# chaitjo/efficient-gnns

Measured on NVIDIA H100. Metric: edges aggregated/s (fwd+bwd), 3-layer GCN student + logit-KD, ARXIV-shape, higher is better.
Workload: dtype f32

## Files before the change

efficient-gnns_b200/csrc/dense_rows.cu:

```cuda
#include "common.cuh"
#include "philox.cuh"

namespace b200gnn {

constexpr int ROWS_THREADS = 256;

struct RowMap {
  int nvec, rows_per_iter, cv, rg;
  bool active;
};
__device__ __forceinline__ RowMap make_row_map(int K) {
  RowMap m;
  m.nvec = K >> 2;
  m.rows_per_iter = ROWS_THREADS / m.nvec;
  m.rg = threadIdx.x / m.nvec;
  m.cv = threadIdx.x - m.rg * m.nvec;
  m.active = m.rg < m.rows_per_iter;
  return m;
}

__device__ __forceinline__ float4 ld4(const float* p) { return *reinterpret_cast<const float4*>(p); }
__device__ __forceinline__ float4 ld4s(const float* p) { return __ldcs(reinterpret_cast<const float4*>(p)); }
__device__ __forceinline__ void st4(float* p, const float4& v) { *reinterpret_cast<float4*>(p) = v; }

__device__ __forceinline__ void reduce_store_2xK(const RowMap& m, int K, float4 a, float4 b, float* smem ,
                                                 float* out) {
  for (int i = threadIdx.x; i < 2 * K; i += ROWS_THREADS) smem[i] = 0.f;
  __syncthreads();
  for (int g = 0; g < m.rows_per_iter; ++g) {
    if (m.active && m.rg == g) {
      float* s = smem + 4 * m.cv;
      float* q = smem + K + 4 * m.cv;
      s[0] += a.x; s[1] += a.y; s[2] += a.z; s[3] += a.w;
      q[0] += b.x; q[1] += b.y; q[2] += b.z; q[3] += b.w;
    }
    __syncthreads();
  }
  for (int i = threadIdx.x; i < 2 * K; i += ROWS_THREADS) out[i] = smem[i];
}

__global__ void __launch_bounds__(ROWS_THREADS) col_stats4_kernel(const float* __restrict__ Y, int64_t n_rows, int K,
                                                                  float* __restrict__ partial, int slots) {
  extern __shared__ float smem[];
  const RowMap m = make_row_map(K);
  const int64_t per = (n_rows + slots - 1) / slots;
  const int64_t r0 = (int64_t)blockIdx.x * per, r1 = min(n_rows, r0 + per);
  float4 s = make_float4(0, 0, 0, 0), q = s;
  if (m.active)
    for (int64_t r = r0 + m.rg; r < r1; r += m.rows_per_iter) {
      const float4 y = ld4(Y + (size_t)r * K + 4 * m.cv);
      vstat(s, q, y);
    }
  reduce_store_2xK(m, K, s, q, smem, partial + (size_t)blockIdx.x * 2 * K);
}

constexpr int FIN_COLS = 4, FIN_GROUPS = 64;
__device__ __forceinline__ bool finalize_reduce(const float* __restrict__ partial, int slots, int K, bool second,
                                                double& s_out, double& q_out, int& k_out) {
  __shared__ double sh[2][FIN_GROUPS][FIN_COLS];
  const int c = threadIdx.x % FIN_COLS, g = threadIdx.x / FIN_COLS;
  const int k = blockIdx.x * FIN_COLS + c;
  double s = 0.0, q = 0.0;
  if (k < K)
    for (int j = g; j < slots; j += FIN_GROUPS) {
      s += (double)partial[(size_t)j * 2 * K + k];
      if (second) q += (double)partial[(size_t)j * 2 * K + K + k];
    }
  sh[0][g][c] = s; sh[1][g][c] = q;
  __syncthreads();
  if (g == 0 && k < K) {
    s = 0.0; q = 0.0;
    for (int j = 0; j < FIN_GROUPS; ++j) { s += sh[0][j][c]; q += sh[1][j][c]; }
    s_out = s; q_out = q; k_out = k;
    return true;
  }
  return false;
}

__global__ void __launch_bounds__(256) bn_finalize_kernel(const float* __restrict__ partial, int slots, int K,
                                                          int64_t n, const float* __restrict__ gamma,
                                                          const float* __restrict__ beta, float eps, float momentum,
                                                          float* running_mean, float* running_var, float* mean_out,
                                                          float* invstd_out, float* scale_out, float* shift_out) {
  double s, q; int k;
  if (finalize_reduce(partial, slots, K, true, s, q, k)) {
    const double mean = s / (double)n;
    double var = q / (double)n - mean * mean;
    if (var < 0.0) var = 0.0;
    const float invstd = (float)(1.0 / sqrt(var + (double)eps));
    const float sc = gamma[k] * invstd;
    mean_out[k] = (float)mean;
    invstd_out[k] = invstd;
    scale_out[k] = sc;
    shift_out[k] = beta[k] - (float)mean * sc;
    if (running_mean) {
      const double unbiased = n > 1 ? var * (double)n / (double)(n - 1) : var;
      running_mean[k] = (1.f - momentum) * running_mean[k] + momentum * (float)mean;
      running_var[k] = (1.f - momentum) * running_var[k] + momentum * (float)unbiased;
    }
  }
}

__device__ __forceinline__ float4 affine_relu4(float4 y, const float* __restrict__ scale, const float* __restrict__ shift,
                                               int cv, int relu) {
  if (scale) {
    const float4 sc = ld4(scale + 4 * cv), sh = ld4(shift + 4 * cv);
    y.x = fmaf(y.x, sc.x, sh.x); y.y = fmaf(y.y, sc.y, sh.y);
    y.z = fmaf(y.z, sc.z, sh.z); y.w = fmaf(y.w, sc.w, sh.w);
  }
  if (relu) { y.x = fmaxf(y.x, 0.f); y.y = fmaxf(y.y, 0.f); y.z = fmaxf(y.z, 0.f); y.w = fmaxf(y.w, 0.f); }
  return y;
}

template <bool P16>
__global__ void __launch_bounds__(256) affine_relu_dropout_kernel(const float* __restrict__ Y, float* __restrict__ out,
                                                                  int64_t n_vec, int nvec_row,
                                                                  const float* __restrict__ scale,
                                                                  const float* __restrict__ shift, int relu, float p,
                                                                  uint32_t thr16, uint64_t seed, uint64_t offset,
                                                                  const int32_t* __restrict__ step_dev,
// ... 249 lines not shown
    int K, float inv_keep, float* __restrict__ dY, float* __restrict__ colsum_partial, int slots) {
  extern __shared__ float smem[];
  const RowMap m = make_row_map(K);
  const int64_t per = (n_rows + slots - 1) / slots;
  const int64_t r0 = (int64_t)blockIdx.x * per, r1 = min(n_rows, r0 + per);
  float4 s = make_float4(0, 0, 0, 0), q = s;
  if (m.active) {
    const float4 mu = ld4(mean + 4 * m.cv), is = ld4(invstd + 4 * m.cv);
    const float4 c1 = ld4(coef + 4 * m.cv), c2 = ld4(coef + K + 4 * m.cv), c3 = ld4(coef + 2 * K + 4 * m.cv);
    for (int64_t r = r0 + m.rg; r < r1; r += m.rows_per_iter) {
      const size_t o = (size_t)r * K + 4 * m.cv;
      float4 g = ld4s(dOut + o);
      const float4 y = ld4s(Y + o);
      if (!DZ) {
        const float4 x = ld4s(Xout + o);
        g.x = x.x > 0.f ? g.x * inv_keep : 0.f; g.y = x.y > 0.f ? g.y * inv_keep : 0.f;
        g.z = x.z > 0.f ? g.z * inv_keep : 0.f; g.w = x.w > 0.f ? g.w * inv_keep : 0.f;
      }
      float4 d;
      d.x = c1.x * (g.x - c2.x - (y.x - mu.x) * is.x * c3.x);
      d.y = c1.y * (g.y - c2.y - (y.y - mu.y) * is.y * c3.y);
      d.z = c1.z * (g.z - c2.z - (y.z - mu.z) * is.z * c3.z);
      d.w = c1.w * (g.w - c2.w - (y.w - mu.w) * is.w * c3.w);
      st4(dY + o, d);
      s.x += d.x; s.y += d.y; s.z += d.z; s.w += d.w;
    }
  }
  if (colsum_partial) reduce_store_2xK(m, K, s, q, smem, colsum_partial + (size_t)blockIdx.x * 2 * K);
}

__global__ void __launch_bounds__(256) partial_reduce_kernel(const float* __restrict__ partial, int slots, int K2,
                                                             float* __restrict__ out) {
  __shared__ double sh[FIN_GROUPS][FIN_COLS];
  const int c = threadIdx.x % FIN_COLS, g = threadIdx.x / FIN_COLS;
  const int k = blockIdx.x * FIN_COLS + c;
  double s = 0.0;
  if (k < K2)
    for (int j = g; j < slots; j += FIN_GROUPS) s += (double)partial[(size_t)j * K2 + k];
  sh[g][c] = s;
  __syncthreads();
  if (g == 0 && k < K2) {
    s = 0.0;
    for (int j = 0; j < FIN_GROUPS; ++j) s += sh[j][c];
    out[k] = (float)s;
  }
}

__global__ void __launch_bounds__(256) colsum_finalize_kernel(const float* __restrict__ partial, int slots, int K,
                                                              float* __restrict__ out) {
  double s, q; int k;
  if (finalize_reduce(partial, slots, K, false, s, q, k)) out[k] = (float)s;
}

__global__ void __launch_bounds__(256) adam_kernel(float* __restrict__ p, const float* __restrict__ g,
                                                   float* __restrict__ m, float* __restrict__ v, int64_t n, float lr,
                                                   float b1, float b2, float eps, const int32_t* __restrict__ step) {
  const float t = (float)(*step + 1);
  const float bc1 = 1.f - powf(b1, t), bc2 = 1.f - powf(b2, t);
  const float step_size = lr / bc1, inv_sqrt_bc2 = rsqrtf(bc2);
  for (int64_t i = (int64_t)blockIdx.x * blockDim.x + threadIdx.x; i < n; i += (int64_t)gridDim.x * blockDim.x)
    adam_update(p[i], m[i], v[i], g[i], b1, b2, eps, step_size, inv_sqrt_bc2);
}
__global__ void adam_tick_kernel(int32_t* step) { *step += 1; }

__global__ void __launch_bounds__(256) rmsprop_kernel(float* __restrict__ p, const float* __restrict__ g, float* __restrict__ sq,
                                                      int64_t n, double lr, int warmup, float alpha, float one_minus_alpha,
                                                      float eps, float wd, const int32_t* __restrict__ step) {
  const int e = *step + 1;
  const float neg_lr = -(float)(warmup > 0 ? lr * (double)(e < warmup ? e : warmup) / (double)warmup : lr);
  for (int64_t i = (int64_t)blockIdx.x * blockDim.x + threadIdx.x; i < n; i += (int64_t)gridDim.x * blockDim.x) {
    const float pi = p[i];
    float gi = g[i];
    if (wd != 0.f) gi = __fadd_rn(gi, __fmul_rn(wd, pi));
    const float s = __fadd_rn(__fmul_rn(sq[i], alpha), __fmul_rn(__fmul_rn(one_minus_alpha, gi), gi));
    sq[i] = s;
    p[i] = __fadd_rn(pi, __fdiv_rn(__fmul_rn(neg_lr, gi), __fadd_rn(__fsqrt_rn(s), eps)));
  }
}

static inline int grid_for(int64_t n_items, int per_cta, int cap = 132 * 8) {
  int64_t g = (n_items + per_cta - 1) / per_cta;
  if (g > cap) g = cap;
  if (g < 1) g = 1;
  return (int)g;
}

}

using namespace b200gnn;

static bool rows_ok(int64_t n_rows, int64_t K) { return n_rows >= 0 && K > 0 && K % 4 == 0 && K <= 1024; }

extern "C" int64_t b200gnn_rows_slots(int64_t n_rows) {
  int64_t s = (n_rows + 255) / 256;
  if (s > 132 * 4) s = 132 * 4;
  return s < 1 ? 1 : s;
}

extern "C" int b200gnn_col_stats_f32(const float* Y, int64_t n_rows, int64_t K, float* partial, int64_t slots,
                                     void* stream) {
  if (!rows_ok(n_rows, K) || !Y || !partial || slots < 1 || !aligned_to(Y, 16)) return B200GNN_ERR_BAD_ARG;
  col_stats4_kernel<<<(int)slots, ROWS_THREADS, 2 * K * sizeof(float), (cudaStream_t)stream>>>(Y, n_rows, (int)K, partial,
                                                                                             (int)slots);
  return check_launch();
}

extern "C" int b200gnn_bn_finalize_f32(const float* partial, int64_t slots, int64_t K, int64_t n_rows,
                                       const float* gamma, const float* beta, float eps, float momentum,
                                       float* running_mean, float* running_var, float* mean_out, float* invstd_out,
                                       float* scale_out, float* shift_out, void* stream) {
  if (!partial || slots < 1 || K <= 0 || n_rows <= 0 || !gamma || !beta || !mean_out || !invstd_out || !scale_out ||
      !shift_out || ((running_mean == nullptr) != (running_var == nullptr)))
    return B200GNN_ERR_BAD_ARG;
  bn_finalize_kernel<<<(int)((K + FIN_COLS - 1) / FIN_COLS), 256, 0, (cudaStream_t)stream>>>(
// ... 182 lines not shown
  const size_t smem = 2 * K * sizeof(float);
  int rc;
  bn_bwd_finalize_kernel<<<(int)((K + FIN_COLS - 1) / FIN_COLS), 256, 0, st>>>(sums, (int)sum_slots, (int)K, n_norm, gamma,
                                                                              invstd, dgamma, dbeta, coef);
  if ((rc = check_launch())) return rc;
  if (Xout)
    bn_act_bwd_apply_kernel<false><<<(int)slots, ROWS_THREADS, smem, st>>>(dOut, Xout, Y, mean, invstd, coef, n_rows, (int)K,
                                                                          inv_keep, dY, dbias ? partial : nullptr, (int)slots);
  else
    bn_act_bwd_apply_kernel<true><<<(int)slots, ROWS_THREADS, smem, st>>>(dOut, nullptr, Y, mean, invstd, coef, n_rows, (int)K,
                                                                         inv_keep, dY, dbias ? partial : nullptr, (int)slots);
  if ((rc = check_launch())) return rc;
  if (dbias) {
    colsum_finalize_kernel<<<(int)((K + FIN_COLS - 1) / FIN_COLS), 256, 0, st>>>(partial, (int)slots, (int)K, dbias);
    if ((rc = check_launch())) return rc;
  }
  return B200GNN_OK;
}

extern "C" int b200gnn_bn_act_bwd_f32(const float* dOut, const float* Xout, const float* Y, const float* mean,
                                      const float* invstd, const float* gamma, int64_t n_rows, int64_t K, float p,
                                      float* dY, float* dgamma, float* dbeta, float* dbias, float* partial,
                                      int64_t slots, float* coef, void* stream) {
  int rc = b200gnn_bn_act_bwd_reduce_f32(dOut, Xout, Y, mean, invstd, n_rows, K, p, partial, slots, stream);
  if (rc) return rc;
  return b200gnn_bn_act_bwd_apply_f32(dOut, Xout, Y, mean, invstd, gamma, partial, slots, n_rows, n_rows, K, p, dY,
                                      dgamma, dbeta, dbias, partial, slots, coef, stream);
}

extern "C" int b200gnn_partial_reduce_f32(const float* partial, int64_t slots, int64_t K2, float* out, void* stream) {
  if (!partial || !out || slots < 1 || K2 < 1) return B200GNN_ERR_BAD_ARG;
  partial_reduce_kernel<<<(int)((K2 + FIN_COLS - 1) / FIN_COLS), 256, 0, (cudaStream_t)stream>>>(partial, (int)slots, (int)K2,
                                                                                               out);
  return check_launch();
}

extern "C" int b200gnn_col_sum_f32(const float* Y, int64_t n_rows, int64_t K, float* out, float* partial,
                                   int64_t slots, void* stream) {
  if (!rows_ok(n_rows, K) || !Y || !out || !partial || slots < 1) return B200GNN_ERR_BAD_ARG;
  cudaStream_t st = (cudaStream_t)stream;
  int rc;
  col_stats4_kernel<<<(int)slots, ROWS_THREADS, 2 * K * sizeof(float), st>>>(Y, n_rows, (int)K, partial, (int)slots);
  if ((rc = check_launch())) return rc;
  colsum_finalize_kernel<<<(int)((K + FIN_COLS - 1) / FIN_COLS), 256, 0, st>>>(partial, (int)slots, (int)K, out);
  return check_launch();
}

extern "C" int b200gnn_adam_step_f32(float* params, const float* grads, float* exp_avg, float* exp_avg_sq, int64_t n,
                                     float lr, float beta1, float beta2, float eps, int32_t* step, void* stream) {
  if (!params || !grads || !exp_avg || !exp_avg_sq || !step || n < 0) return B200GNN_ERR_BAD_ARG;
  cudaStream_t st = (cudaStream_t)stream;
  int rc;
  if (n > 0) {
    adam_kernel<<<grid_for(n, 256), 256, 0, st>>>(params, grads, exp_avg, exp_avg_sq, n, lr, beta1, beta2, eps, step);
    if ((rc = check_launch())) return rc;
  }
  adam_tick_kernel<<<1, 1, 0, st>>>(step);
  return check_launch();
}

extern "C" int b200gnn_rmsprop_step_f32(float* params, const float* grads, float* square_avg, int64_t n, double lr,
                                        int64_t warmup, double alpha, double eps, double weight_decay, int32_t* step,
                                        void* stream) {
  if (!params || !grads || !square_avg || !step || n < 0 || !(lr >= 0.0) || !(alpha >= 0.0) || !(eps >= 0.0) ||
      !(weight_decay >= 0.0) || warmup < 0 || warmup > (1 << 30))
    return B200GNN_ERR_BAD_ARG;
  cudaStream_t st = (cudaStream_t)stream;
  int rc;
  if (n > 0) {
    rmsprop_kernel<<<grid_for(n, 256), 256, 0, st>>>(params, grads, square_avg, n, lr, (int)warmup, (float)alpha,
                                                     (float)(1.0 - alpha), (float)eps, (float)weight_decay, step);
    if ((rc = check_launch())) return rc;
  }
  adam_tick_kernel<<<1, 1, 0, st>>>(step);
  return check_launch();
}
```

efficient-gnns_b200/csrc/gemm_tf32x3.cu:

```cuda
#include <cuda.h>

#include "common.cuh"
#include "tc_common.cuh"

namespace b200gnn {
namespace gemm {
using namespace tc;

constexpr int BM = 128, BK = 32;
constexpr int THREADS = 384;
constexpr int CONSUMER_WARPS = 8;
constexpr int TILE_BYTES = BM * BK * 4;
constexpr int BAR_BYTES = 256;
constexpr int EPI_BYTES = CONSUMER_WARPS * 16 * 32 * 4;
constexpr int STAT_MAX_N = 256;
constexpr int STAT_BYTES = CONSUMER_WARPS * 2 * STAT_MAX_N * 4;
constexpr int XY_ROWS = 16;
constexpr int XY_SLOT_BYTES = 2 * XY_ROWS * 32 * 4;
constexpr int XY_BYTES = CONSUMER_WARPS * 2 * XY_SLOT_BYTES;
constexpr int XY_BAR_OFF = 128;
constexpr int BNBWD_TMA_MAX_K = 128;

template <int BN_T, int NSTAGE, int EXTRA = 0>
struct Cfg {
// ... 370 lines not shown
      } else {
        const int rr = lane & 15, cb = (lane >> 4) * 16, grow = m0 + q * 16 + rr;
        if (grow < p.M && col0 + cb < p.N) {
          for (int jx = 0; jx < 16; ++jx) {
            const int cc = cb + jx, col = col0 + cc;
            if (col >= p.N) break;
            const float v = tile_s[stg(rr, cc >> 2) + (cc & 3)] + (p.bias ? __ldg(p.bias + col) : 0.f);
            if (PEER && p.bcast) {
              for (int r = 0; r < p.n_peer; ++r) p.Cp[r][(size_t)(p.row_off + grow) * p.ldc + col] = v;
            } else if (!PEER) {
              float* dst = p.C + (size_t)(ROWIDX ? __ldg(p.row_idx + grow) : (int64_t)grow) * p.ldc + col;
              *dst = v + (p.accumulate ? *dst : 0.f);
            }
          }
        }
        __syncwarp();
      }
    }
  }
  if (COLSTAT) {
    __syncwarp();
    float* out = p.stat_partial + (size_t)(blockIdx.x * CONSUMER_WARPS + q) * 2 * p.N;
    for (int i = lane; i < 2 * p.N; i += 32) out[i] = stat[i];
  }
  if (PRB) {
#pragma unroll
    for (int d = 16; d > 0; d >>= 1) sg += __shfl_xor_sync(0xffffffffu, sg, d);
    if (lane == 0) p.slope_partial[blockIdx.x * CONSUMER_WARPS + q] = sg;
  }
}

__global__ void __launch_bounds__(32) slope_grad_finalize_kernel(const double* __restrict__ part, int n, float* __restrict__ out,
                                                                 int accumulate) {
  double a = 0.0;
  for (int i = threadIdx.x; i < n; i += 32) a += part[i];
#pragma unroll
  for (int d = 16; d > 0; d >>= 1) a += __shfl_xor_sync(0xffffffffu, a, d);
  if (threadIdx.x == 0) out[0] = accumulate ? out[0] + (float)a : (float)a;
}

__global__ void __launch_bounds__(256) split_tf32_kernel(const float* __restrict__ W, int64_t rows, int64_t cols,
                                                         int transpose, float* __restrict__ hi, float* __restrict__ lo) {
  const int64_t n = rows * cols;
  for (int64_t i = (int64_t)blockIdx.x * blockDim.x + threadIdx.x; i < n; i += (int64_t)gridDim.x * blockDim.x) {
    const int64_t r = i / cols, c = i - r * cols;
    uint32_t h, l;
    split1(__float_as_uint(W[i]), h, l);
    const int64_t o = transpose ? c * rows + r : i;
    hi[o] = __uint_as_float(h);
    lo[o] = __uint_as_float(l);
  }
}

static bool make_map(CUtensorMap* m, const float* base, int64_t rows, int64_t cols, int64_t ld, int box_rows, bool swizzle = true) {
  EncodeTiledFn fn = encode_fn();
  if (!fn) return false;
  cuuint64_t dims[2] = {(cuuint64_t)cols, (cuuint64_t)rows};
  cuuint64_t strides[1] = {(cuuint64_t)ld * 4};
  cuuint32_t box[2] = {(cuuint32_t)BK, (cuuint32_t)box_rows};
  cuuint32_t estr[2] = {1, 1};
  return fn(m, CU_TENSOR_MAP_DATA_TYPE_FLOAT32, 2, const_cast<float*>(base), dims, strides, box, estr,
            CU_TENSOR_MAP_INTERLEAVE_NONE, swizzle ? CU_TENSOR_MAP_SWIZZLE_128B : CU_TENSOR_MAP_SWIZZLE_NONE,
            CU_TENSOR_MAP_L2_PROMOTION_L2_256B, CU_TENSOR_MAP_FLOAT_OOB_FILL_NONE) == CUDA_SUCCESS;
}

template <class C, int STAT = 0, bool PEER = false, bool ACT = false, bool PRELU = false, bool ROWIDX = false>
static int launch(const float* A, int64_t lda, const float* B_hi, const float* B_lo, int64_t ldb, const Params& p,
                  cudaStream_t stream) {
  CUtensorMap tA, tBh, tBl, tX, tY;
  if (!make_map(&tA, A, p.M, p.K, lda, BM) || !make_map(&tBh, B_hi, p.N, p.K, ldb, C::BN) ||
      !make_map(&tBl, B_lo, p.N, p.K, ldb, C::BN))
    return B200GNN_ERR_UNSUPPORTED;
  tX = tA; tY = tA;
  if (STAT == 3 && ((!ACT && !make_map(&tX, p.bn_x, p.M, p.N, p.ldc, XY_ROWS, false)) ||
                    !make_map(&tY, p.bn_y, p.M, p.N, p.ldc, XY_ROWS, false)))
    return B200GNN_ERR_UNSUPPORTED;
  int dev = 0, sms = 132;
  cudaGetDevice(&dev);
  static bool attr_set[64] = {};
  if (dev >= 0 && dev < 64 && !attr_set[dev]) {
    cudaError_t e = cudaFuncSetAttribute(gemm_tf32x3_kernel<C, STAT, PEER, ACT, PRELU, ROWIDX>, cudaFuncAttributeMaxDynamicSharedMemorySize,
                                         C::SMEM_BYTES);
    if (e != cudaSuccess) { set_cuda_error(e); return B200GNN_ERR_CUDA; }
    attr_set[dev] = true;
  }
  const int tiles = ((p.M + BM - 1) / BM) * ((p.N + C::BN - 1) / C::BN);
  cudaDeviceGetAttribute(&sms, cudaDevAttrMultiProcessorCount, dev);
  const int grid = tiles < sms ? tiles : sms;
  gemm_tf32x3_kernel<C, STAT, PEER, ACT, PRELU, ROWIDX><<<grid, THREADS, C::SMEM_BYTES, stream>>>(tA, tBh, tBl, tX, tY, p);
  return check_launch();
}

}
}

using namespace b200gnn;

extern "C" int b200gnn_split_tf32_f32(const float* W, int64_t rows, int64_t cols, int transpose, float* hi, float* lo,
                                      void* stream) {
  if (!W || !hi || !lo || rows <= 0 || cols <= 0) return B200GNN_ERR_BAD_ARG;
  const int64_t n = rows * cols;
  int grid = (int)((n + 255) / 256);
  if (grid > 132 * 8) grid = 132 * 8;
  gemm::split_tf32_kernel<<<grid, 256, 0, (cudaStream_t)stream>>>(W, rows, cols, transpose, hi, lo);
  return check_launch();
}

static int g_bnbwd_variant = 0;
extern "C" void b200gnn_gemm_set_bnbwd_variant(int v) { g_bnbwd_variant = v; }

static int gemm_dispatch(const float* A, int64_t lda, const float* B_hi, const float* B_lo, int64_t ldb, float* C, int64_t ldc,
                         int64_t M, int64_t N, int64_t K, const float* bias, int accumulate, void* stream,
                         const gemm::Params* st = nullptr, const gemm::Params* act = nullptr,
                         const gemm::Params* prelu = nullptr) {
  if (!A || !B_hi || !B_lo || !C || M <= 0 || N <= 0 || K <= 0 || lda < K || ldb < K || ldc < N ||
      M >= INT32_MAX || N >= INT32_MAX || K >= INT32_MAX)
    return B200GNN_ERR_BAD_ARG;
  if (lda % 4 || ldb % 4 || !aligned_to(A, 16) || !aligned_to(B_hi, 16) || !aligned_to(B_lo, 16))
    return B200GNN_ERR_UNSUPPORTED;
  gemm::Params p{};
  p.C = C; p.bias = bias; p.ldc = ldc; p.M = (int32_t)M; p.N = (int32_t)N; p.K = (int32_t)K; p.accumulate = accumulate ? 1 : 0;
  p.n_peer = 0; p.kc = 0; p.row_off = 0; p.bcast = 0;
  if (act) {
    if (!act->act_scale || !act->act_shift || !act->act_bits || !aligned_to(act->act_scale, 16) || !aligned_to(act->act_shift, 16))
      return B200GNN_ERR_BAD_ARG;
    p.act_scale = act->act_scale; p.act_shift = act->act_shift; p.act_bits = act->act_bits; p.act_words = act->act_words;
    p.inv_keep = act->inv_keep;
  }
  if (prelu) {
    if (!prelu->act_slope || !prelu->act_bits) return B200GNN_ERR_BAD_ARG;
    p.act_slope = prelu->act_slope; p.act_bits = prelu->act_bits; p.act_words = prelu->act_words; p.inv_keep = prelu->inv_keep;
    if (prelu->stat_mode == 0) {
      if (N <= 48) return gemm::launch<gemm::Cfg<48, 6>, 0, false, false, true>(A, lda, B_hi, B_lo, ldb, p, (cudaStream_t)stream);
      return gemm::launch<gemm::Cfg<128, 4>, 0, false, false, true>(A, lda, B_hi, B_lo, ldb, p, (cudaStream_t)stream);
    }
    if (N % 32 || ldc % 4 || !aligned_to(C, 16) || !prelu->bn_y || !aligned_to(prelu->bn_y, 16) || !prelu->slope_partial)
      return B200GNN_ERR_UNSUPPORTED;
    p.stat_mode = 4; p.bn_y = prelu->bn_y; p.slope_partial = prelu->slope_partial;
    return gemm::launch<gemm::Cfg<128, 4>, 4>(A, lda, B_hi, B_lo, ldb, p, (cudaStream_t)stream);
  }
  if (act && !st) {
    if (K > (int64_t)gemm::STAT_BYTES / 8) return B200GNN_ERR_UNSUPPORTED;
    if (N <= 48) return gemm::launch<gemm::Cfg<48, 6>, 0, false, true>(A, lda, B_hi, B_lo, ldb, p, (cudaStream_t)stream);
    return gemm::launch<gemm::Cfg<128, 4>, 0, false, true>(A, lda, B_hi, B_lo, ldb, p, (cudaStream_t)stream);
  }
  if (st) {
    if (N % 32 || N > gemm::STAT_MAX_N || N <= 48 || ldc % 4 || !aligned_to(C, 16) || !st->stat_partial) return B200GNN_ERR_UNSUPPORTED;
    p.stat_mode = st->stat_mode; p.stat_partial = st->stat_partial; p.bn_x = st->bn_x; p.bn_y = st->bn_y;
    p.bn_mean = st->bn_mean; p.bn_invstd = st->bn_invstd; p.inv_keep = st->inv_keep;
    if (p.stat_mode == 1) return gemm::launch<gemm::Cfg<128, 4>, 1>(A, lda, B_hi, B_lo, ldb, p, (cudaStream_t)stream);
    const bool tma = N % 128 == 0 && (g_bnbwd_variant == 1 || (g_bnbwd_variant == 0 && K < gemm::BNBWD_TMA_MAX_K));
    if (act)
      return tma ? gemm::launch<gemm::Cfg<128, 2, gemm::XY_BYTES>, 3, false, true>(A, lda, B_hi, B_lo, ldb, p, (cudaStream_t)stream)
                 : gemm::launch<gemm::Cfg<128, 4>, 2, false, true>(A, lda, B_hi, B_lo, ldb, p, (cudaStream_t)stream);
    if (tma) return gemm::launch<gemm::Cfg<128, 2, gemm::XY_BYTES>, 3>(A, lda, B_hi, B_lo, ldb, p, (cudaStream_t)stream);
    return gemm::launch<gemm::Cfg<128, 4>, 2>(A, lda, B_hi, B_lo, ldb, p, (cudaStream_t)stream);
  }
  if (N <= 48) return gemm::launch<gemm::Cfg<48, 6>>(A, lda, B_hi, B_lo, ldb, p, (cudaStream_t)stream);
  return gemm::launch<gemm::Cfg<128, 4>>(A, lda, B_hi, B_lo, ldb, p, (cudaStream_t)stream);
}
// ... 148 lines not shown
```

efficient-gnns_b200/csrc/spmm.cu:

```cuda
#include <cuda.h>

#include "common.cuh"
#include "tc_common.cuh"

namespace b200gnn {

constexpr int SPMM_THREADS = 256;
constexpr int SPMM_WARPS = SPMM_THREADS / 32;
constexpr int SPMM_MAX_SLAB_FLOATS = 512;

struct SpmmParams {
  const int32_t* rowptr;
  const int32_t* col;
  const float* val;
  const float* X;
  float* Y;
  const float* bias;
  float* stat_partial;
  const int32_t* chunk_rowptr;
  const int32_t* hub_rows;
  const int32_t* hub_segptr;
  float* hub_ws;
  int64_t ldx, ldy;
  int32_t n_rows, K, nvec;
  int32_t hub_threshold, seg_len, n_hub, n_seg, n_chunks;
  int32_t mean, stream_store, main_grid;
  int32_t n_slabs, l2_hint;
  float* Yp[16];
  int32_t yoff[17];
  int32_t n_yp, ycol;
  int64_t ldyp;
};

__device__ __forceinline__ float4* y_row_v4(const SpmmParams& p, int row) {
  if (p.n_yp == 0) return reinterpret_cast<float4*>(p.Y) + (size_t)row * (size_t)(p.ldy / 4);
  int q = 0;
#pragma unroll 1
  while (q + 1 < p.n_yp && row >= p.yoff[q + 1]) ++q;
  return reinterpret_cast<float4*>(p.Yp[q] + (size_t)(row - p.yoff[q]) * (size_t)p.ldyp + p.ycol);
}

struct LaneMap {
  int lpr, groups, g, l;
  bool active;
};

__device__ __forceinline__ LaneMap make_lane_map(int nvec, int lane) {
  LaneMap m;
  if (nvec >= 32) {
    m.lpr = 32; m.groups = 1; m.g = 0; m.l = lane; m.active = true;
  } else {
    m.lpr = nvec; m.groups = 32 / nvec; m.g = lane / nvec; m.l = lane - m.g * nvec;
    m.active = m.g < m.groups;
  }
  return m;
}

template <typename V, int CH, bool HAS_VAL>
__device__ __forceinline__ void walk_edges(const int32_t* __restrict__ col, const float* __restrict__ val,
                                           const V* __restrict__ Xv, size_t ldxv, int beg, int end,
                                           int lane, const LaneMap& m, int slab_voff, int nvec, V (&acc)[CH]) {
  constexpr int U = 8 / CH;
  bool cvalid[CH];
#pragma unroll
  for (int j = 0; j < CH; ++j) cvalid[j] = m.active && (slab_voff + m.l + 32 * j < nvec);

  for (int base = beg; base < end; base += 32) {
    const int e = base + lane;
    int c = 0;
    float v = HAS_VAL ? 0.f : 1.f;
    if (e < end) {
      c = __ldg(col + e);
      if (HAS_VAL) v = __ldg(val + e);
    }
    const int cnt = min(32, end - base);
// ... 77 lines not shown
  const int row_lo = chunk < p.n_chunks ? __ldg(p.chunk_rowptr + chunk) : 0;
  const int row_hi = chunk < p.n_chunks ? __ldg(p.chunk_rowptr + chunk + 1) : 0;
  int end = row_lo < row_hi ? __ldg(p.rowptr + row_lo) : 0;
  for (int row = row_lo; row < row_hi; ++row) {
    const int beg = end;
    end = __ldg(p.rowptr + row + 1);
    const int deg = end - beg;
    if (deg > p.hub_threshold) continue;
    for (int slab = 0; slab < nslab; ++slab) {
      const int slab_voff = slab * slab_vecs;
      V acc[CH];
#pragma unroll
      for (int j = 0; j < CH; ++j) vzero(acc[j]);
      walk_edges<V, CH, HAS_VAL>(p.col, p.val, Xv, ldxv, beg, end, lane, m, slab_voff, p.nvec, acc);
      if (m.groups > 1) group_reduce(acc[0], m);
      if (m.g == 0 && m.active) {
#pragma unroll
        for (int j = 0; j < CH; ++j) {
          const int voff = slab_voff + m.l + 32 * j;
          if (voff < p.nvec) {
            V y = acc[j];
            if (p.mean) vdiv(y, (float)max(deg, 1));
            if (p.bias) vadd(y, load_bias<V>(p.bias, voff));
            V* dst = Yv + (size_t)row * ldyv + voff;
            if (p.stream_store) vstcs(dst, y); else *dst = y;
            if (do_stats) vstat(ssum[j], ssq[j], y);
          }
        }
      }
    }
  }

  if (do_stats) {
    float* ss = s_stat;
    float* sq = s_stat + p.K;
    for (int i = threadIdx.x; i < 2 * p.K; i += SPMM_THREADS) s_stat[i] = 0.f;
    __syncthreads();
    for (int w = 0; w < SPMM_WARPS; ++w) {
      if (warp == w && m.g == 0 && m.active) {
#pragma unroll
        for (int j = 0; j < CH; ++j) {
          const int voff = m.l + 32 * j;
          if (voff < p.nvec) smem_accum(ss, sq, voff, ssum[j], ssq[j]);
        }
      }
      __syncthreads();
    }
    float* out = p.stat_partial + (size_t)cta * 2 * p.K;
    for (int i = threadIdx.x; i < 2 * p.K; i += SPMM_THREADS) out[i] = s_stat[i];
  }
}

template <typename V, int CH, bool HAS_VAL>
__device__ __forceinline__ void spmm_hub_seg_cta(const SpmmParams& p, const int seg, float* s_buf, const int slab_lo = 0,
                                                 const int slab_hi = 1 << 30) {
  constexpr int W = VecTraits<V>::W;

  const int warp = threadIdx.x >> 5, lane = threadIdx.x & 31;
  const LaneMap m = make_lane_map(p.nvec, lane);
  const int slab_vecs = 32 * CH;
  const int nslab = (p.nvec <= 32) ? 1 : (p.nvec + slab_vecs - 1) / slab_vecs;
  const V* Xv = reinterpret_cast<const V*>(p.X);
  const size_t ldxv = (size_t)(p.ldx / W);

  int lo = 0, hi = p.n_hub;
  while (hi - lo > 1) {
    const int mid = (lo + hi) >> 1;
    if (__ldg(p.hub_segptr + mid) <= seg) lo = mid; else hi = mid;
  }
  const int h = lo;
  const int row = __ldg(p.hub_rows + h);
  const int s = seg - __ldg(p.hub_segptr + h);
  const int rbeg = __ldg(p.rowptr + row), rend = __ldg(p.rowptr + row + 1);
  const int sbeg = rbeg + s * p.seg_len;
  const int send = min(rend, sbeg + p.seg_len);
  int per = (send - sbeg + SPMM_WARPS - 1) / SPMM_WARPS;
  per = (per + 31) / 32 * 32;
  const int wbeg = min(send, sbeg + warp * per);
  const int wend = min(send, wbeg + per);

  float* ws = p.hub_ws + (size_t)seg * p.K;
  for (int slab = slab_lo; slab < min(nslab, slab_hi); ++slab) {
    const int slab_voff = slab * slab_vecs;
    V acc[CH];
#pragma unroll
    for (int j = 0; j < CH; ++j) vzero(acc[j]);
    walk_edges<V, CH, HAS_VAL>(p.col, p.val, Xv, ldxv, wbeg, wend, lane, m, slab_voff, p.nvec, acc);
    if (m.groups > 1) group_reduce(acc[0], m);

    for (int i = threadIdx.x; i < SPMM_MAX_SLAB_FLOATS; i += SPMM_THREADS) s_buf[i] = 0.f;
    __syncthreads();
    for (int w = 0; w < SPMM_WARPS; ++w) {
      if (warp == w && m.g == 0 && m.active) {
#pragma unroll
        for (int j = 0; j < CH; ++j) {
          const int voff = slab_voff + m.l + 32 * j;
          if (voff < p.nvec) smem_add1(s_buf, m.l + 32 * j, acc[j]);
        }
      }
      __syncthreads();
    }
    const int slab_f0 = slab_voff * W;
    const int slab_fn = min(slab_vecs * W, p.K - slab_f0);
    for (int i = threadIdx.x; i < slab_fn; i += SPMM_THREADS) ws[slab_f0 + i] = s_buf[i];
    __syncthreads();
  }
}

template <typename V, int CH, bool HAS_VAL, bool STATS>
__global__ void __launch_bounds__(SPMM_THREADS, 3) spmm_rows_kernel(const SpmmParams p) {
  __shared__ float s_mem[2 * SPMM_MAX_SLAB_FLOATS];
  if ((int)blockIdx.x < p.n_seg) spmm_hub_seg_cta<V, CH, HAS_VAL>(p, (int)blockIdx.x, s_mem);
  else spmm_chunk_cta<V, CH, HAS_VAL, STATS>(p, (int)blockIdx.x - p.n_seg, s_mem);
}


constexpr int PIPE_BYTES = 8192;
constexpr int PIPE_SMEM = SPMM_WARPS * PIPE_BYTES;

__device__ __forceinline__ void cp_async16(void* smem_dst, const void* gsrc) {
  asm volatile("cp.async.cg.shared.global [%0], [%1], 16;" ::"r"((uint32_t)__cvta_generic_to_shared(smem_dst)), "l"(gsrc)
               : "memory");
}
__device__ __forceinline__ void cp_async_commit() { asm volatile("cp.async.commit_group;" ::: "memory"); }
template <int N>
__device__ __forceinline__ void cp_async_wait() { asm volatile("cp.async.wait_group %0;" ::"n"(N) : "memory"); }

template <int CH, bool HAS_VAL, bool STATS>
__device__ __forceinline__ void spmm_chunk_cta_pipe(const SpmmParams& p, const int cta, float* s_stat, float4* ring_all) {
  constexpr int D = PIPE_BYTES / (CH * 512);
  constexpr int G = D >= 8 ? 4 : 2, NG = D / G;
  const int warp = threadIdx.x >> 5, lane = threadIdx.x & 31;
  float4* ring = ring_all + (size_t)warp * (PIPE_BYTES / 16);
  const float4* Xv = reinterpret_cast<const float4*>(p.X);
  float4* Yv = reinterpret_cast<float4*>(p.Y);
  const size_t ldxv = (size_t)(p.ldx / 4), ldyv = (size_t)(p.ldy / 4);

  float4 ssum[CH], ssq[CH];
#pragma unroll
  for (int j = 0; j < CH; ++j) { vzero(ssum[j]); vzero(ssq[j]); }

  const int chunk = cta * SPMM_WARPS + warp;
  const int row_lo = chunk < p.n_chunks ? __ldg(p.chunk_rowptr + chunk) : 0;
  const int row_hi = chunk < p.n_chunks ? __ldg(p.chunk_rowptr + chunk + 1) : 0;

  auto flush = [&](int row, int deg, float4 (&acc)[CH]) {
#pragma unroll
    for (int j = 0; j < CH; ++j) {
      const int voff = lane + 32 * j;
      float4 y = acc[j];
      if (p.mean) vdiv(y, (float)max(deg, 1));
      if (p.bias) vadd(y, load_bias<float4>(p.bias, voff));
      float4* dst = Yv + (size_t)row * ldyv + voff;
      if (p.stream_store) vstcs(dst, y); else *dst = y;
      if (STATS) vstat(ssum[j], ssq[j], y);
      vzero(acc[j]);
    }
  };

  int r = row_lo;
  while (r < row_hi) {
    int e_lo = __ldg(p.rowptr + r);
    {
      const int e_next = __ldg(p.rowptr + r + 1);
      if (e_next - e_lo > p.hub_threshold) { ++r; continue; }
// ... 59 lines not shown
      int done = 0;
      while (done < cnt) {
        const int room = rend - (e_lo + j0 + done);
        const int take = min(cnt - done, room);
        if (take == G) {
#pragma unroll
          for (int u = 0; u < G; ++u) {
            const float w = HAS_VAL ? __shfl_sync(FULL_MASK, vA, (j0 + u) & 31) : 1.f;
#pragma unroll
            for (int jj = 0; jj < CH; ++jj) vfma(acc[jj], w, sbase[u * (CH * 32) + 32 * jj]);
          }
        } else {
#pragma unroll 1
          for (int u = done; u < done + take; ++u) {
            const float w = HAS_VAL ? __shfl_sync(FULL_MASK, vA, (j0 + u) & 31) : 1.f;
#pragma unroll
            for (int jj = 0; jj < CH; ++jj) vfma(acc[jj], w, sbase[u * (CH * 32) + 32 * jj]);
          }
        }
        done += take;
        if (take == room) boundary();
      }
    };
#pragma unroll
    for (int g = 0; g < NG; ++g) issue_group(g * G, g * G);
#pragma unroll 1
    for (int j = 0, s0 = 0; j < n; j += G, s0 = (s0 + G) & (D - 1)) {
      cp_async_wait<NG - 1>();
      consume_group(j, s0);
      issue_group(j + D, s0);
    }
    cp_async_wait<0>();
  }

  if (STATS) {
    float* ss = s_stat;
    float* sq = s_stat + p.K;
    for (int i = threadIdx.x; i < 2 * p.K; i += SPMM_THREADS) s_stat[i] = 0.f;
    __syncthreads();
    for (int w = 0; w < SPMM_WARPS; ++w) {
      if (warp == w) {
#pragma unroll
        for (int j = 0; j < CH; ++j) smem_accum(ss, sq, lane + 32 * j, ssum[j], ssq[j]);
      }
      __syncthreads();
    }
    float* out = p.stat_partial + (size_t)cta * 2 * p.K;
    for (int i = threadIdx.x; i < 2 * p.K; i += SPMM_THREADS) out[i] = s_stat[i];
  }
}

template <int CH, bool HAS_VAL, bool STATS>
__global__ void __launch_bounds__(SPMM_THREADS, 3) spmm_rows_pipe_kernel(const SpmmParams p) {
  __shared__ float s_mem[2 * SPMM_MAX_SLAB_FLOATS];
  extern __shared__ float4 s_ring[];
  if ((int)blockIdx.x < p.n_seg) spmm_hub_seg_cta<float4, CH, HAS_VAL>(p, (int)blockIdx.x, s_mem);
  else spmm_chunk_cta_pipe<CH, HAS_VAL, STATS>(p, (int)blockIdx.x - p.n_seg, s_mem, s_ring);
}


constexpr int BULK_RING = 8192;
constexpr int BULK_MAX_GROUPS = 8;

__device__ __forceinline__ uint32_t smem_u32(const void* p) { return (uint32_t)__cvta_generic_to_shared(p); }
__device__ __forceinline__ void mbar_init(uint64_t* bar, int count) {
  asm volatile("mbarrier.init.shared::cta.b64 [%0], %1;" ::"r"(smem_u32(bar)), "r"(count) : "memory");
}
__device__ __forceinline__ void mbar_expect_tx(uint64_t* bar, uint32_t bytes) {
  asm volatile("mbarrier.arrive.expect_tx.shared::cta.b64 _, [%0], %1;" ::"r"(smem_u32(bar)), "r"(bytes) : "memory");
}
__device__ __forceinline__ void mbar_wait(uint64_t* bar, uint32_t parity) {
  asm volatile(
      "{\n\t.reg .pred p;\n\t"
      "WAIT_%=:\n\t"
      "mbarrier.try_wait.parity.shared::cta.b64 p, [%0], %1;\n\t"
      "@p bra DONE_%=;\n\t"
      "bra WAIT_%=;\n\t"
      "DONE_%=:\n\t}" ::"r"(smem_u32(bar)), "r"(parity)
      : "memory");
}
__device__ __forceinline__ void bulk_g2s(void* dst, const void* src, uint32_t bytes, uint64_t* bar) {
  asm volatile("cp.async.bulk.shared::cluster.global.mbarrier::complete_tx::bytes [%0], [%1], %2, [%3];" ::"r"(smem_u32(dst)),
               "l"(src), "r"(bytes), "r"(smem_u32(bar))
               : "memory");
}
__device__ __forceinline__ void bulk_g2s_hint(void* dst, const void* src, uint32_t bytes, uint64_t* bar, uint64_t pol) {
  asm volatile("cp.async.bulk.shared::cluster.global.mbarrier::complete_tx::bytes.L2::cache_hint [%0], [%1], %2, [%3], %4;" ::
                   "r"(smem_u32(dst)), "l"(src), "r"(bytes), "r"(smem_u32(bar)), "l"(pol)
               : "memory");
}

template <int CH, int G, bool HAS_VAL, bool STATS>
__device__ __forceinline__ void spmm_chunk_cta_bulk(const SpmmParams& p, const int cta, const int slab, float* s_stat,
                                                    float4* ring_all, uint64_t* bars_all) {
  constexpr int SLOT_V = CH * 32;
  constexpr int SLOT_B = SLOT_V * 16;
  constexpr int D = BULK_RING / SLOT_B;
  constexpr int NG = D / G;
  static_assert(NG >= 2 && NG <= BULK_MAX_GROUPS && (32 % G) == 0 && D <= 32, "ring geometry");
  const int warp = threadIdx.x >> 5, lane = threadIdx.x & 31;
  float4* ring = ring_all + (size_t)warp * (BULK_RING / 16);
  uint64_t* bars = bars_all + warp * BULK_MAX_GROUPS;
  if (lane < NG) mbar_init(bars + lane, 1);
  asm volatile("fence.mbarrier_init.release.cluster;" ::: "memory");
  asm volatile("fence.proxy.async.shared::cta;" ::: "memory");
  __syncwarp();
  uint64_t pol = 0;
  if (p.l2_hint) asm volatile("createpolicy.fractional.L2::evict_last.b64 %0, 1.0;" : "=l"(pol));

// ... 104 lines not shown
            const float w = HAS_VAL ? __shfl_sync(FULL_MASK, vA, (j0 + u) & 31) : 1.f;
#pragma unroll
            for (int jj = 0; jj < CH; ++jj) vfma(acc[jj], w, sbase[u * SLOT_V + 32 * jj]);
          }
        } else {
#pragma unroll 1
          for (int u = done; u < done + take; ++u) {
            const float w = HAS_VAL ? __shfl_sync(FULL_MASK, vA, (j0 + u) & 31) : 1.f;
#pragma unroll
            for (int jj = 0; jj < CH; ++jj) vfma(acc[jj], w, sbase[u * SLOT_V + 32 * jj]);
          }
        }
        done += take;
        if (take == room) boundary();
      }
    };
#pragma unroll
    for (int g = 0; g < NG; ++g) issue_group(g * G, g * G, g);
    int b = 0;
#pragma unroll 1
    for (int j = 0, s0 = 0; j < n; j += G) {
      mbar_wait(bars + b, (phases >> b) & 1u);
      phases ^= 1u << b;
      consume_group(j, s0);
      __syncwarp();
      issue_group(j + D, s0, b);
      s0 = (s0 + G) & (D - 1);
      b = (b + 1 == NG) ? 0 : b + 1;
    }
  }

  if (STATS) {
    constexpr int SW = SLOT_V * 4;
    float* ss = s_stat;
    float* sq = s_stat + SW;
    for (int i = threadIdx.x; i < 2 * SW; i += SPMM_THREADS) s_stat[i] = 0.f;
    __syncthreads();
    for (int w = 0; w < SPMM_WARPS; ++w) {
      if (warp == w) {
#pragma unroll
        for (int j = 0; j < CH; ++j) smem_accum(ss, sq, lane + 32 * j, ssum[j], ssq[j]);
      }
      __syncthreads();
    }
    float* out = p.stat_partial + (size_t)cta * 2 * p.K + slab * SW;
    for (int i = threadIdx.x; i < SW; i += SPMM_THREADS) { out[i] = ss[i]; out[p.K + i] = sq[i]; }
  }
}

constexpr int BULK_SMEM = SPMM_WARPS * BULK_RING + SPMM_WARPS * BULK_MAX_GROUPS * 8;

template <int CH, int G, bool HAS_VAL, bool STATS>
__global__ void __launch_bounds__(SPMM_THREADS, 3) spmm_rows_bulk_kernel(const SpmmParams p) {
  __shared__ float s_mem[2 * SPMM_MAX_SLAB_FLOATS];
  extern __shared__ __align__(128) unsigned char s_dyn[];
  const int per_slab = p.main_grid + p.n_seg;
  const int slab = (int)blockIdx.x / per_slab;
  const int b = (int)blockIdx.x - slab * per_slab;
  if (b < p.n_seg) spmm_hub_seg_cta<float4, CH, HAS_VAL>(p, b, s_mem, slab, slab + 1);
  else spmm_chunk_cta_bulk<CH, G, HAS_VAL, STATS>(p, b - p.n_seg, slab, s_mem, reinterpret_cast<float4*>(s_dyn),
                                                  reinterpret_cast<uint64_t*>(s_dyn + SPMM_WARPS * BULK_RING));
}


constexpr int SLAB_RING = 8192;
constexpr int SLAB_G = 8;
constexpr int SLAB_SMEM = SPMM_WARPS * SLAB_RING;

__device__ __forceinline__ void cp_async16_pol(void* smem_dst, const void* gsrc, uint64_t pol) {
  asm volatile("cp.async.cg.shared.global.L2::cache_hint [%0], [%1], 16, %2;" ::"r"(smem_u32(smem_dst)), "l"(gsrc), "l"(pol)
               : "memory");
}
__device__ __forceinline__ int32_t ldg_pol(const int32_t* p, uint64_t pol) {
  int32_t v;
  asm("ld.global.nc.L2::cache_hint.b32 %0, [%1], %2;" : "=r"(v) : "l"(p), "l"(pol));
  return v;
}
__device__ __forceinline__ float ldg_pol(const float* p, uint64_t pol) {
  float v;
  asm("ld.global.nc.L2::cache_hint.f32 %0, [%1], %2;" : "=f"(v) : "l"(p), "l"(pol));
  return v;
}

template <int SW> struct SlabLane;
template <> struct SlabLane<32> { using V = float; };
template <> struct SlabLane<64> { using V = float2; };

template <int SW, bool HAS_VAL, bool STATS>
__device__ __forceinline__ void spmm_chunk_cta_slab(const SpmmParams& p, const int cta, const int slab, float* s_stat,
                                                    float* ring_all) {
  using V = typename SlabLane<SW>::V;
  constexpr int LPR = SW / 4;
  constexpr int E = 32 / LPR;
  constexpr int D = SLAB_RING / (SW * 4);
  constexpr int G = SLAB_G, NG = D / G;
  static_assert(G % E == 0 && 32 % G == 0 && NG >= 2 && (D & (D - 1)) == 0, "ring geometry");
  const int warp = threadIdx.x >> 5, lane = threadIdx.x & 31;
  float* ring = ring_all + (size_t)warp * (SLAB_RING / 4);
  uint64_t pol_keep, pol_stream;
  asm volatile("createpolicy.fractional.L2::evict_last.b64 %0, 1.0;" : "=l"(pol_keep));
  asm volatile("createpolicy.fractional.L2::evict_first.b64 %0, 1.0;" : "=l"(pol_stream));

  const int f0 = slab * SW;
  const float* Xs = p.X + f0 + (lane % LPR) * 4;
  float* ring_dst = ring + (lane / LPR) * SW + (lane % LPR) * 4;
  const int vlane = slab * 32 + lane;

  V ssum, ssq, bias_l;
  vzero(ssum); vzero(ssq); vzero(bias_l);
  if (p.bias) bias_l = load_bias<V>(p.bias, vlane);

  const int chunk = cta * SPMM_WARPS + warp;
// ... 87 lines not shown
      if (HAS_VAL && j0 > 0 && (j0 & 31) == 0) { vA = vN; vN = val_win(j0 + 32); }
      const V* sbase = reinterpret_cast<const V*>(ring + slot0 * SW) + lane;
      const int cnt = min(G, n - j0);
      int done = 0;
      while (done < cnt) {
        const int room = rend - (e_lo + j0 + done);
        const int take = min(cnt - done, room);
        if (take == G) {
#pragma unroll
          for (int u = 0; u < G; ++u) {
            const float w = HAS_VAL ? __shfl_sync(FULL_MASK, vA, (j0 + u) & 31) : 1.f;
            vfma(acc, w, sbase[u * 32]);
          }
        } else {
#pragma unroll 1
          for (int u = done; u < done + take; ++u) {
            const float w = HAS_VAL ? __shfl_sync(FULL_MASK, vA, (j0 + u) & 31) : 1.f;
            vfma(acc, w, sbase[u * 32]);
          }
        }
        done += take;
        if (take == room) boundary();
      }
    };
#pragma unroll
    for (int g = 0; g < NG; ++g) issue_group(g * G, g * G);
#pragma unroll 1
    for (int j = 0, s0 = 0; j < n; j += G, s0 = (s0 + G) & (D - 1)) {
      cp_async_wait<NG - 1>();
      __syncwarp();
      consume_group(j, s0);
      __syncwarp();
      issue_group(j + D, s0);
    }
    cp_async_wait<0>();
  }

  if (STATS) {
    float* ss = s_stat;
    float* sq = s_stat + SW;
    for (int i = threadIdx.x; i < 2 * SW; i += SPMM_THREADS) s_stat[i] = 0.f;
    __syncthreads();
    for (int w = 0; w < SPMM_WARPS; ++w) {
      if (warp == w) smem_accum(ss, sq, lane, ssum, ssq);
      __syncthreads();
    }
    float* out = p.stat_partial + (size_t)cta * 2 * p.K + f0;
    for (int i = threadIdx.x; i < SW; i += SPMM_THREADS) { out[i] = ss[i]; out[p.K + i] = sq[i]; }
  }
}

template <int SW, bool HAS_VAL, bool STATS>
__global__ void __launch_bounds__(SPMM_THREADS, 3) spmm_rows_slab_kernel(const SpmmParams p) {
  __shared__ float s_mem[2 * SPMM_MAX_SLAB_FLOATS];
  extern __shared__ __align__(128) unsigned char s_dyn[];
  const int b = (int)blockIdx.x;
  if (b < p.n_seg) {
    spmm_hub_seg_cta<float4, 1, HAS_VAL>(p, b, s_mem);
    return;
  }
  const int slab = (b - p.n_seg) / p.main_grid;
  spmm_chunk_cta_slab<SW, HAS_VAL, STATS>(p, b - p.n_seg - slab * p.main_grid, slab, s_mem, reinterpret_cast<float*>(s_dyn));
}


template <bool HAS_VAL, int U>
__device__ __forceinline__ void spmm_chunk_cta_narrow(const SpmmParams& p, const int cta) {
  const int warp = threadIdx.x >> 5, lane = threadIdx.x & 31;
  const int lpr = p.nvec, groups = 32 / lpr;
  const int g = lane / lpr, l = lane - g * lpr;
  const bool active = g < groups;
  const float4* Xv = reinterpret_cast<const float4*>(p.X);
  float4* Yv = reinterpret_cast<float4*>(p.Y);
  const size_t ldxv = (size_t)(p.ldx / 4), ldyv = (size_t)(p.ldy / 4);
  const int chunk = cta * SPMM_WARPS + warp;
  if (chunk >= p.n_chunks || !active) return;
  const int row_lo = __ldg(p.chunk_rowptr + chunk), row_hi = __ldg(p.chunk_rowptr + chunk + 1);
  float4 bias4 = make_float4(0.f, 0.f, 0.f, 0.f);
  if (p.bias) bias4 = load_bias<float4>(p.bias, l);
  for (int row = row_lo + g; row < row_hi; row += groups) {
    const int beg = __ldg(p.rowptr + row), end = __ldg(p.rowptr + row + 1);
    const int deg = end - beg;
    if (deg > p.hub_threshold) continue;
    float4 acc = make_float4(0.f, 0.f, 0.f, 0.f);
    int e = beg;
    if (e + U <= end) {
      int c[U]; float w[U];
#pragma unroll
      for (int u = 0; u < U; ++u) { c[u] = __ldg(p.col + e + u); w[u] = HAS_VAL ? __ldg(p.val + e + u) : 1.f; }
      for (; e + U <= end; e += U) {
        float4 x[U];
#pragma unroll
        for (int u = 0; u < U; ++u) x[u] = vldg(Xv + (size_t)c[u] * ldxv + l);
        float wc[U];
#pragma unroll
        for (int u = 0; u < U; ++u) wc[u] = w[u];
        if (e + 2 * U <= end) {
#pragma unroll
          for (int u = 0; u < U; ++u) { c[u] = __ldg(p.col + e + U + u); w[u] = HAS_VAL ? __ldg(p.val + e + U + u) : 1.f; }
        }
#pragma unroll
        for (int u = 0; u < U; ++u) vfma(acc, wc[u], x[u]);
      }
    }
    if (U > 4 && e + 4 <= end) {
      int c[4]; float w[4]; float4 x[4];
#pragma unroll
      for (int u = 0; u < 4; ++u) { c[u] = __ldg(p.col + e + u); w[u] = HAS_VAL ? __ldg(p.val + e + u) : 1.f; }
#pragma unroll
      for (int u = 0; u < 4; ++u) x[u] = vldg(Xv + (size_t)c[u] * ldxv + l);
#pragma unroll
      for (int u = 0; u < 4; ++u) vfma(acc, w[u], x[u]);
      e += 4;
    }
    for (; e < end; ++e) {
      const int c = __ldg(p.col + e);
      const float w = HAS_VAL ? __ldg(p.val + e) : 1.f;
      vfma(acc, w, vldg(Xv + (size_t)c * ldxv + l));
    }
    if (p.mean) vdiv(acc, (float)max(deg, 1));
    if (p.bias) vadd(acc, bias4);
    if (p.n_yp) y_row_v4(p, row)[l] = acc; else Yv[(size_t)row * ldyv + l] = acc;
  }
}

template <bool HAS_VAL, int U>
__global__ void __launch_bounds__(SPMM_THREADS, 3) spmm_rows_narrow_kernel(const SpmmParams p) {
  __shared__ float s_mem[SPMM_MAX_SLAB_FLOATS];
  if ((int)blockIdx.x < p.n_seg) spmm_hub_seg_cta<float4, 1, HAS_VAL>(p, (int)blockIdx.x, s_mem);
  else spmm_chunk_cta_narrow<HAS_VAL, U>(p, (int)blockIdx.x - p.n_seg);
}

__global__ void __launch_bounds__(256) spmm_hub_finalize_kernel(const SpmmParams p) {
  __shared__ float4 sh[256];
  const int h = blockIdx.x;
  const int row = __ldg(p.hub_rows + h);
  const int s0 = __ldg(p.hub_segptr + h), s1 = __ldg(p.hub_segptr + h + 1);
  const int deg = __ldg(p.rowptr + row + 1) - __ldg(p.rowptr + row);
  float* stat = p.stat_partial ? p.stat_partial + (size_t)(p.main_grid + h) * 2 * p.K : nullptr;
  const int nvec = p.K >> 2;
  const auto al16 = [](const void* q) { return (reinterpret_cast<uintptr_t>(q) & 15) == 0; };
  if ((p.K & 3) == 0 && nvec <= 256 && (p.ldy & 3) == 0 && al16(p.Y) && al16(p.hub_ws) && (!stat || al16(stat))) {
    const int G = min(256 / nvec, 16);
    const int v = threadIdx.x % nvec, g = threadIdx.x / nvec;
    float4 acc = make_float4(0.f, 0.f, 0.f, 0.f);
    if (g < G)
      for (int s = s0 + g; s < s1; s += G) {
        const float4 x = *reinterpret_cast<const float4*>(p.hub_ws + (size_t)s * p.K + 4 * v);
        acc.x += x.x; acc.y += x.y; acc.z += x.z; acc.w += x.w;
      }
    sh[threadIdx.x] = acc;
    __syncthreads();
    if (g != 0) return;
    for (int j = 1; j < G; ++j) {
      const float4 x = sh[j * nvec + v];
      acc.x += x.x; acc.y += x.y; acc.z += x.z; acc.w += x.w;
    }
    if (p.mean) { const float d = (float)max(deg, 1); acc.x /= d; acc.y /= d; acc.z /= d; acc.w /= d; }
    if (p.bias) {
      acc.x += __ldg(p.bias + 4 * v); acc.y += __ldg(p.bias + 4 * v + 1);
      acc.z += __ldg(p.bias + 4 * v + 2); acc.w += __ldg(p.bias + 4 * v + 3);
    }
    if (p.n_yp) y_row_v4(p, row)[v] = acc; else *reinterpret_cast<float4*>(p.Y + (size_t)row * p.ldy + 4 * v) = acc;
    if (stat) {
      *reinterpret_cast<float4*>(stat + 4 * v) = acc;
      *reinterpret_cast<float4*>(stat + p.K + 4 * v) = make_float4(acc.x * acc.x, acc.y * acc.y, acc.z * acc.z, acc.w * acc.w);
    }
    return;
  }
  float* yrow = p.n_yp ? reinterpret_cast<float*>(y_row_v4(p, row)) : p.Y + (size_t)row * p.ldy;
  for (int k = threadIdx.x; k < p.K; k += blockDim.x) {
    float acc = 0.f;
    for (int s = s0; s < s1; ++s) acc += p.hub_ws[(size_t)s * p.K + k];
    if (p.mean) acc /= (float)max(deg, 1);
    if (p.bias) acc += __ldg(p.bias + k);
    yrow[k] = acc;
    if (stat) { stat[k] = acc; stat[p.K + k] = acc * acc; }
  }
}

__global__ void __launch_bounds__(256) col_stats_kernel(const float* __restrict__ Y, int64_t ldy, int64_t n_rows,
                                                        int K, float* __restrict__ partial, int slots) {
  const int slot = blockIdx.x;
  const int64_t per = (n_rows + slots - 1) / slots;
  const int64_t r0 = (int64_t)slot * per, r1 = min(n_rows, r0 + per);
  float* out = partial + (size_t)slot * 2 * K;
  for (int k = threadIdx.x; k < K; k += blockDim.x) {
    float s = 0.f, q = 0.f;
    for (int64_t r = r0; r < r1; ++r) {
      const float y = Y[(size_t)r * ldy + k];
      s += y; q = fmaf(y, y, q);
    }
    out[k] = s; out[K + k] = q;
  }
}

template <typename V, int CH>
static int launch_spmm(const SpmmParams& p, cudaStream_t st) {
  int rc;
  const bool stats = p.stat_partial != nullptr;
  const int grid = p.main_grid + p.n_seg;
  if (p.val) {
    if (stats) spmm_rows_kernel<V, CH, true, true><<<grid, SPMM_THREADS, 0, st>>>(p);
    else spmm_rows_kernel<V, CH, true, false><<<grid, SPMM_THREADS, 0, st>>>(p);
  } else {
    if (stats) spmm_rows_kernel<V, CH, false, true><<<grid, SPMM_THREADS, 0, st>>>(p);
    else spmm_rows_kernel<V, CH, false, false><<<grid, SPMM_THREADS, 0, st>>>(p);
  }
  if ((rc = check_launch())) return rc;
  if (p.n_hub > 0) {
    spmm_hub_finalize_kernel<<<p.n_hub, 256, 0, st>>>(p);
    if ((rc = check_launch())) return rc;
  }
  return B200GNN_OK;
}

template <int CH>
static int launch_spmm_pipe(const SpmmParams& p, cudaStream_t st) {
  int rc;
  const bool stats = p.stat_partial != nullptr;
  const int grid = p.main_grid + p.n_seg;
  int dev = 0;
  cudaGetDevice(&dev);
  static bool attr_done_dev[64] = {};
  if (dev >= 0 && dev < 64 && !attr_done_dev[dev]) {
    cudaFuncSetAttribute(spmm_rows_pipe_kernel<CH, true, true>, cudaFuncAttributeMaxDynamicSharedMemorySize, PIPE_SMEM);
    cudaFuncSetAttribute(spmm_rows_pipe_kernel<CH, true, false>, cudaFuncAttributeMaxDynamicSharedMemorySize, PIPE_SMEM);
    cudaFuncSetAttribute(spmm_rows_pipe_kernel<CH, false, true>, cudaFuncAttributeMaxDynamicSharedMemorySize, PIPE_SMEM);
    cudaFuncSetAttribute(spmm_rows_pipe_kernel<CH, false, false>, cudaFuncAttributeMaxDynamicSharedMemorySize, PIPE_SMEM);
    attr_done_dev[dev] = true;
  }
  if (p.val) {
    if (stats) spmm_rows_pipe_kernel<CH, true, true><<<grid, SPMM_THREADS, PIPE_SMEM, st>>>(p);
    else spmm_rows_pipe_kernel<CH, true, false><<<grid, SPMM_THREADS, PIPE_SMEM, st>>>(p);
  } else {
    if (stats) spmm_rows_pipe_kernel<CH, false, true><<<grid, SPMM_THREADS, PIPE_SMEM, st>>>(p);
    else spmm_rows_pipe_kernel<CH, false, false><<<grid, SPMM_THREADS, PIPE_SMEM, st>>>(p);
  }
  if ((rc = check_launch())) return rc;
  if (p.n_hub > 0) {
    spmm_hub_finalize_kernel<<<p.n_hub, 256, 0, st>>>(p);
    if ((rc = check_launch())) return rc;
  }
  return B200GNN_OK;
}

constexpr int BULK_SMEM_2CTA = 112 * 1024;

template <int CH, int G>
static int launch_spmm_bulk(const SpmmParams& p, cudaStream_t st, bool two_ctas) {
  int rc;
  const bool stats = p.stat_partial != nullptr;
  const int grid = (p.main_grid + p.n_seg) * p.n_slabs;
  const int smem = two_ctas ? BULK_SMEM_2CTA : BULK_SMEM;
  int dev = 0;
  cudaGetDevice(&dev);
  static bool attr_done[64] = {};
  if (dev >= 0 && dev < 64 && !attr_done[dev]) {
    cudaFuncSetAttribute(spmm_rows_bulk_kernel<CH, G, true, true>, cudaFuncAttributeMaxDynamicSharedMemorySize, BULK_SMEM_2CTA);
    cudaFuncSetAttribute(spmm_rows_bulk_kernel<CH, G, true, false>, cudaFuncAttributeMaxDynamicSharedMemorySize, BULK_SMEM_2CTA);
    cudaFuncSetAttribute(spmm_rows_bulk_kernel<CH, G, false, true>, cudaFuncAttributeMaxDynamicSharedMemorySize, BULK_SMEM_2CTA);
    cudaFuncSetAttribute(spmm_rows_bulk_kernel<CH, G, false, false>, cudaFuncAttributeMaxDynamicSharedMemorySize, BULK_SMEM_2CTA);
    attr_done[dev] = true;
  }
  if (p.val) {
    if (stats) spmm_rows_bulk_kernel<CH, G, true, true><<<grid, SPMM_THREADS, smem, st>>>(p);
    else spmm_rows_bulk_kernel<CH, G, true, false><<<grid, SPMM_THREADS, smem, st>>>(p);
  } else {
    if (stats) spmm_rows_bulk_kernel<CH, G, false, true><<<grid, SPMM_THREADS, smem, st>>>(p);
    else spmm_rows_bulk_kernel<CH, G, false, false><<<grid, SPMM_THREADS, smem, st>>>(p);
  }
  if ((rc = check_launch())) return rc;
  if (p.n_hub > 0) {
    spmm_hub_finalize_kernel<<<p.n_hub, 256, 0, st>>>(p);
    if ((rc = check_launch())) return rc;
  }
  return B200GNN_OK;
}

template <int SW>
static int launch_spmm_slab(const SpmmParams& p, cudaStream_t st) {
  int rc;
  const bool stats = p.stat_partial != nullptr;
  const int grid = p.n_seg + p.main_grid * p.n_slabs;
  int dev = 0;
  cudaGetDevice(&dev);
  static bool attr_done[64] = {};
  if (dev >= 0 && dev < 64 && !attr_done[dev]) {
    cudaFuncSetAttribute(spmm_rows_slab_kernel<SW, true, true>, cudaFuncAttributeMaxDynamicSharedMemorySize, SLAB_SMEM);
    cudaFuncSetAttribute(spmm_rows_slab_kernel<SW, true, false>, cudaFuncAttributeMaxDynamicSharedMemorySize, SLAB_SMEM);
    cudaFuncSetAttribute(spmm_rows_slab_kernel<SW, false, true>, cudaFuncAttributeMaxDynamicSharedMemorySize, SLAB_SMEM);
    cudaFuncSetAttribute(spmm_rows_slab_kernel<SW, false, false>, cudaFuncAttributeMaxDynamicSharedMemorySize, SLAB_SMEM);
    attr_done[dev] = true;
  }
  if (p.val) {
    if (stats) spmm_rows_slab_kernel<SW, true, true><<<grid, SPMM_THREADS, SLAB_SMEM, st>>>(p);
    else spmm_rows_slab_kernel<SW, true, false><<<grid, SPMM_THREADS, SLAB_SMEM, st>>>(p);
  } else {
    if (stats) spmm_rows_slab_kernel<SW, false, true><<<grid, SPMM_THREADS, SLAB_SMEM, st>>>(p);
    else spmm_rows_slab_kernel<SW, false, false><<<grid, SPMM_THREADS, SLAB_SMEM, st>>>(p);
  }
  if ((rc = check_launch())) return rc;
  if (p.n_hub > 0) {
    spmm_hub_finalize_kernel<<<p.n_hub, 256, 0, st>>>(p);
    if ((rc = check_launch())) return rc;
  }
  return B200GNN_OK;
}

template <typename V>
static int dispatch_ch(const SpmmParams& p, cudaStream_t st) {
  if (p.nvec <= 32) return launch_spmm<V, 1>(p, st);
  if (p.nvec <= 64) return launch_spmm<V, 2>(p, st);
  return launch_spmm<V, 4>(p, st);
}

__global__ void __launch_bounds__(1024) hub_count_kernel(const int32_t* __restrict__ rowptr, int64_t n_rows,
                                                         int32_t thr, int32_t seg_len, int32_t* __restrict__ out) {
  __shared__ int s_cnt[2];
  if (threadIdx.x < 2) s_cnt[threadIdx.x] = 0;
  __syncthreads();
  int nh = 0, ns = 0;
  for (int64_t r = threadIdx.x; r < n_rows; r += blockDim.x) {
    const int deg = rowptr[r + 1] - rowptr[r];
    if (deg > thr) { nh += 1; ns += (deg + seg_len - 1) / seg_len; }
  }
  atomicAdd(&s_cnt[0], nh);
  atomicAdd(&s_cnt[1], ns);
  __syncthreads();
  if (threadIdx.x < 2) out[threadIdx.x] = s_cnt[threadIdx.x];
}

__global__ void __launch_bounds__(1024) hub_fill_kernel(const int32_t* __restrict__ rowptr, int64_t n_rows,
                                                        int32_t thr, int32_t seg_len, int32_t* __restrict__ hub_rows,
                                                        int32_t* __restrict__ hub_segptr, int64_t n_hub) {
  __shared__ int s_wflag[32], s_wseg[32];
  __shared__ int s_base[2];
  const int lane = threadIdx.x & 31, warp = threadIdx.x >> 5;
  if (threadIdx.x == 0) { s_base[0] = 0; s_base[1] = 0; }
  __syncthreads();
  for (int64_t r0 = 0; r0 < n_rows; r0 += blockDim.x) {
    const int64_t r = r0 + threadIdx.x;
    int flag = 0, segs = 0;
    if (r < n_rows) {
      const int deg = rowptr[r + 1] - rowptr[r];
      if (deg > thr) { flag = 1; segs = (deg + seg_len - 1) / seg_len; }
    }
    int f = flag, s = segs;
    for (int d = 1; d < 32; d <<= 1) {
      const int of = __shfl_up_sync(FULL_MASK, f, d), os = __shfl_up_sync(FULL_MASK, s, d);
      if (lane >= d) { f += of; s += os; }
    }
    if (lane == 31) { s_wflag[warp] = f; s_wseg[warp] = s; }
    __syncthreads();
    if (warp == 0) {
      int wf = s_wflag[lane], wsg = s_wseg[lane];
// ... 36 lines not shown
}

}

using namespace b200gnn;

static int g_spmm_variant = 0;

struct ScatterArgs { int n; float* ptr[16]; int32_t off[17]; int64_t ld, col; };
static thread_local ScatterArgs g_scatter = {0, {}, {}, 0, 0};

static int bulk_auto_slab(int64_t K, int64_t n_src) {
  (void)n_src;
  return (K % 256 == 0) ? 256 : 128;
}
constexpr int64_t SLAB_L2_BUDGET = (int64_t)40 << 20;
constexpr int SLAB_SW = 64;
extern "C" void b200gnn_spmm_set_variant(int v) { g_spmm_variant = v; }

extern "C" int64_t b200gnn_csr_chunk_count(int64_t n_rows, int64_t nnz, int32_t chunk_nnz, int32_t row_cost) {
  if (n_rows < 0 || nnz < 0 || chunk_nnz <= 0 || row_cost <= 0) return B200GNN_ERR_BAD_ARG;
  const int64_t total = nnz + n_rows * (int64_t)row_cost;
  return total == 0 ? 0 : (total + chunk_nnz - 1) / chunk_nnz;
}

extern "C" int b200gnn_csr_chunk_plan(const int32_t* rowptr, int64_t n_rows, int64_t nnz, int32_t chunk_nnz,
                                      int32_t row_cost, int32_t* chunk_rowptr, void* stream) {
  const int64_t n_chunks = b200gnn_csr_chunk_count(n_rows, nnz, chunk_nnz, row_cost);
  if (n_chunks < 0 || !rowptr || !chunk_rowptr) return B200GNN_ERR_BAD_ARG;
  chunk_plan_kernel<<<(int)((n_chunks + 1 + 255) / 256), 256, 0, (cudaStream_t)stream>>>(rowptr, n_rows, chunk_nnz,
                                                                                        row_cost, chunk_rowptr, n_chunks);
  return check_launch();
}

extern "C" int b200gnn_csr_hub_count(const int32_t* rowptr, int64_t n_rows, int32_t hub_threshold, int32_t seg_len,
                                     int32_t* counts_out, void* stream) {
  if (!rowptr || !counts_out || n_rows < 0 || hub_threshold < 0 || seg_len <= 0) return B200GNN_ERR_BAD_ARG;
  hub_count_kernel<<<1, 1024, 0, (cudaStream_t)stream>>>(rowptr, n_rows, hub_threshold, seg_len, counts_out);
  return check_launch();
}

extern "C" int b200gnn_csr_hub_fill(const int32_t* rowptr, int64_t n_rows, int32_t hub_threshold, int32_t seg_len,
                                    int32_t* hub_rows, int32_t* hub_segptr, int64_t n_hub, void* stream) {
  if (!rowptr || !hub_segptr || n_rows < 0 || n_hub < 0 || hub_threshold < 0 || seg_len <= 0) return B200GNN_ERR_BAD_ARG;
  if (n_hub > 0 && !hub_rows) return B200GNN_ERR_BAD_ARG;
  hub_fill_kernel<<<1, 1024, 0, (cudaStream_t)stream>>>(rowptr, n_rows, hub_threshold, seg_len, hub_rows, hub_segptr, n_hub);
  return check_launch();
}

extern "C" int64_t b200gnn_spmm_stat_slots(int64_t n_chunks, int64_t n_hub) {
  return (n_chunks + SPMM_WARPS - 1) / SPMM_WARPS + n_hub;
}

extern "C" int b200gnn_spmm_csr_f32(const int32_t* rowptr, const int32_t* col, const float* val, const float* X,
                                    int64_t ldx, float* Y, int64_t ldy, int64_t n_rows, int64_t n_src, int64_t K,
                                    int reduce, const float* bias, float* stat_partial,
                                    const int32_t* chunk_rowptr, int64_t n_chunks, int32_t hub_threshold,
                                    int32_t seg_len, const int32_t* hub_rows, const int32_t* hub_segptr,
                                    int64_t n_hub, int64_t n_seg, float* hub_workspace, void* stream) {
  if (n_rows < 0 || n_src < 0 || K <= 0 || n_rows >= INT32_MAX || n_src >= INT32_MAX || K > (1 << 20))
    return B200GNN_ERR_BAD_ARG;
  if (reduce != B200GNN_REDUCE_SUM && reduce != B200GNN_REDUCE_MEAN) return B200GNN_ERR_BAD_ARG;
  if (n_rows == 0) return B200GNN_OK;
  if (!rowptr || !Y || ldy < K || !chunk_rowptr || n_chunks <= 0 || n_chunks >= INT32_MAX) return B200GNN_ERR_BAD_ARG;
  if (n_src > 0 && (!X || ldx < K)) return B200GNN_ERR_BAD_ARG;
  if (n_hub < 0 || n_seg < 0 || hub_threshold < 0) return B200GNN_ERR_BAD_ARG;
  if (n_hub > 0 && (!hub_rows || !hub_segptr || !hub_workspace || seg_len <= 0 || n_seg < n_hub))
    return B200GNN_ERR_BAD_ARG;
  cudaStream_t st = (cudaStream_t)stream;

  SpmmParams p;
  p.rowptr = rowptr; p.col = col; p.val = val; p.X = X; p.Y = Y; p.bias = bias;
  p.stat_partial = stat_partial;
  p.chunk_rowptr = chunk_rowptr; p.n_chunks = (int32_t)n_chunks;
  p.hub_rows = hub_rows; p.hub_segptr = hub_segptr; p.hub_ws = hub_workspace;
  p.ldx = ldx; p.ldy = ldy;
  p.n_rows = (int32_t)n_rows; p.K = (int32_t)K;
  p.hub_threshold = hub_threshold; p.seg_len = seg_len; p.n_hub = (int32_t)n_hub;
  p.n_seg = n_hub > 0 ? (int32_t)n_seg : 0;
  p.mean = reduce == B200GNN_REDUCE_MEAN;
  p.stream_store = (n_rows * K * 4 > (int64_t)64 << 20) ? 1 : 0;
  p.main_grid = (int32_t)((n_chunks + SPMM_WARPS - 1) / SPMM_WARPS);

  int W = 1;
  if (K % 4 == 0 && ldx % 4 == 0 && ldy % 4 == 0 && aligned_to(X, 16) && aligned_to(Y, 16)) W = 4;
  else if (K % 2 == 0 && ldx % 2 == 0 && ldy % 2 == 0 && aligned_to(X, 8) && aligned_to(Y, 8)) W = 2;
  p.nvec = (int32_t)(K / W);
  p.n_slabs = 1; p.l2_hint = 0;
  p.n_yp = 0; p.ycol = 0; p.ldyp = 0;
  if (g_scatter.n > 0) {
    if (W != 4 || K % 4 || g_scatter.ld % 4 || g_scatter.col % 4) return B200GNN_ERR_UNSUPPORTED;
    const int sfam = g_spmm_variant & 15;
    const bool to_bulk = K % 128 == 0 && K <= 4096 && (sfam == 0 || (sfam >= 3 && sfam <= 7));
    const bool to_narrow = p.nvec <= 16 && !stat_partial && sfam != 1 && sfam != 2;
    if (!to_bulk && !to_narrow) return B200GNN_ERR_UNSUPPORTED;
    p.n_yp = g_scatter.n; p.ycol = (int32_t)g_scatter.col; p.ldyp = g_scatter.ld;
    for (int q = 0; q < g_scatter.n; ++q) { p.Yp[q] = g_scatter.ptr[q]; p.yoff[q] = g_scatter.off[q]; }
    p.yoff[g_scatter.n] = g_scatter.off[g_scatter.n];
  }

  if (g_spmm_variant == 0 && W == 4 && p.n_yp == 0 && (K == 128 || K == 256) && n_src * K * 4 > SLAB_L2_BUDGET) {
    p.n_slabs = (int32_t)(K / SLAB_SW);
    return launch_spmm_slab<SLAB_SW>(p, st);
  }

  const int fam = g_spmm_variant & 15;
  const bool alt_g = (g_spmm_variant & 32) != 0;
  int bulk_sw = 0;
  if (W == 4 && K % 128 == 0 && K <= 4096) {
    if (fam == 3) bulk_sw = (K % 256 == 0) ? 256 : 128;
    else if (fam == 4) bulk_sw = 128;
    else if (fam == 5) bulk_sw = (K % 256 == 0) ? 256 : 128;
    else if (fam == 6 || fam == 7) bulk_sw = 128;
    else if (fam == 0) bulk_sw = bulk_auto_slab(K, n_src);
  }
  int rc;
  float* fused_stats = stat_partial;
  bool single_slab = true;
  if (bulk_sw) {
    p.n_slabs = (int32_t)(K / bulk_sw);
    p.l2_hint = (g_spmm_variant & 16) ? 1 : 0;
    if (fam == 6) return launch_spmm_bulk<1, 8>(p, st, false);
    if (fam == 7) return launch_spmm_bulk<1, 4>(p, st, false);
    const bool two = (g_spmm_variant & 64) != 0;
    if (bulk_sw == 128) rc = alt_g ? launch_spmm_bulk<1, 2>(p, st, two) : launch_spmm_bulk<1, 4>(p, st, two);
    else rc = alt_g ? launch_spmm_bulk<2, 2>(p, st, two) : launch_spmm_bulk<2, 4>(p, st, two);
    return rc;
  }

  const int ch = p.nvec <= 32 ? 1 : (p.nvec <= 64 ? 2 : 4);
  single_slab = p.nvec <= 32 * ch;
  if (!single_slab) p.stat_partial = nullptr;

  const bool pipe_ok = (W == 4) && fam == 2 && (p.nvec == 32 || p.nvec == 64 || p.nvec == 128);
  const bool narrow_ok = (W == 4) && p.nvec <= 16 && !p.stat_partial && fam != 1;
  if (narrow_ok) {
    rc = B200GNN_OK;
    const int grid = p.main_grid + p.n_seg;
    const bool deep = (g_spmm_variant & 128) != 0;
    if (p.val) { if (deep) spmm_rows_narrow_kernel<true, 8><<<grid, SPMM_THREADS, 0, st>>>(p); else spmm_rows_narrow_kernel<true, 4><<<grid, SPMM_THREADS, 0, st>>>(p); }
    else { if (deep) spmm_rows_narrow_kernel<false, 8><<<grid, SPMM_THREADS, 0, st>>>(p); else spmm_rows_narrow_kernel<false, 4><<<grid, SPMM_THREADS, 0, st>>>(p); }
    if ((rc = check_launch())) return rc;
    if (p.n_hub > 0) {
      spmm_hub_finalize_kernel<<<p.n_hub, 256, 0, st>>>(p);
      if ((rc = check_launch())) return rc;
    }
  }
  else if (pipe_ok && p.nvec == 32) rc = launch_spmm_pipe<1>(p, st);
  else if (pipe_ok && p.nvec == 64) rc = launch_spmm_pipe<2>(p, st);
  else if (pipe_ok && p.nvec == 128) rc = launch_spmm_pipe<4>(p, st);
  else if (W == 4) rc = dispatch_ch<float4>(p, st);
  else if (W == 2) rc = dispatch_ch<float2>(p, st);
  else rc = dispatch_ch<float>(p, st);
  if (rc) return rc;

  if (fused_stats && !single_slab) {
    const int slots = (int)b200gnn_spmm_stat_slots(n_chunks, n_hub);
    col_stats_kernel<<<slots, 256, 0, st>>>(Y, ldy, n_rows, (int)K, fused_stats, slots);
    if ((rc = check_launch())) return rc;
  }
  return B200GNN_OK;
}

extern "C" int b200gnn_spmm_csr_scatter_f32(const int32_t* rowptr, const int32_t* col, const float* val, const float* X,
                                            int64_t ldx, float* const* Y_ptrs, const int32_t* row_off, int32_t world,
                                            int64_t ldy_dst, int64_t col_dst, int64_t n_rows, int64_t n_src, int64_t K, int reduce,
                                            const float* bias, const int32_t* chunk_rowptr, int64_t n_chunks,
                                            int32_t hub_threshold, int32_t seg_len, const int32_t* hub_rows,
                                            const int32_t* hub_segptr, int64_t n_hub, int64_t n_seg, float* hub_workspace,
                                            void* stream) {
  if (!Y_ptrs || !row_off || world <= 0 || world > 16 || ldy_dst < K || col_dst < 0 || row_off[0] != 0 || row_off[world] != n_rows)
    return B200GNN_ERR_BAD_ARG;
  g_scatter.n = world; g_scatter.ld = ldy_dst; g_scatter.col = col_dst;
  for (int q = 0; q < world; ++q) {
    if (!Y_ptrs[q] || !aligned_to(Y_ptrs[q], 16) || row_off[q + 1] < row_off[q]) { g_scatter.n = 0; return B200GNN_ERR_BAD_ARG; }
    g_scatter.ptr[q] = Y_ptrs[q]; g_scatter.off[q] = row_off[q];
  }
  g_scatter.off[world] = row_off[world];
  const int rc = b200gnn_spmm_csr_f32(rowptr, col, val, X, ldx, Y_ptrs[0], K, n_rows, n_src, K, reduce, bias, nullptr, chunk_rowptr,
                                      n_chunks, hub_threshold, seg_len, hub_rows, hub_segptr, n_hub, n_seg, hub_workspace, stream);
  g_scatter.n = 0;
  return rc;
}
```

efficient-gnns_b200/engine.py:

```python
from __future__ import annotations

import math
from typing import Dict, List, Optional

import torch

from . import lib, ops
from .sparse import CsrGraph, SparseTensor
from .trainer import FlatParams, FullBatchStudent, one_objective


def gcn_norm(adj: SparseTensor) -> SparseTensor:
    if not adj.has_value():
        adj = adj.fill_value(1.0)
    adj = adj.fill_diag(1.0)
    deg = adj.sum(dim=1)
    dis = deg.pow(-0.5)
    dis.masked_fill_(dis == float("inf"), 0.0)
    row, col, val = adj.coo()
    return adj.set_value(dis[row] * val * dis[col])


def _is_symmetric(adj: SparseTensor) -> bool:
    st = adj.storage
# ... 7 lines not shown


class GCNStudentTrainer(FullBatchStudent):

    def __init__(self, adj: SparseTensor, dims: List[int], dropout: float = 0.5, lr: float = 0.01, seed: int = 0,
                 alpha: float = 0.9, kd_T: float = 4.0, bn_eps: float = 1e-5, bn_momentum: float = 0.1,
                 aggregate_first: Optional[bool] = None, tensor_core_gemm: bool = True, overlap_wgrad: bool = True,
                 fuse_row_passes: bool = True, fuse_activations: bool = True, _prebuilt_graph: Optional[CsrGraph] = None, _rows_alloc: Optional[int] = None,
                 gcrd=None, lsp=None, gsp=None):
        self.objective = one_objective(gcrd, lsp, gsp)
        assert adj.is_cuda(), "the engine runs on a CUDA device"
        self.device = adj.device
        self.dims, self.L = list(dims), len(dims) - 1
        self.p, self.lr, self.alpha, self.kd_T = float(dropout), float(lr), float(alpha), float(kd_T)
        self.bn_eps, self.bn_momentum = bn_eps, bn_momentum
        self.seed = int(seed)
        self.tc_gemm = bool(tensor_core_gemm) and all(d % 4 == 0 for d in dims)
        for d in dims[1:]:
            assert d % 4 == 0 and d <= 1024, "layer widths must be multiples of 4 (128-bit rows)"
        self.N = adj.size(0)
        self.agg_first = (dims[0] < dims[1] and dims[0] % 4 == 0) if aggregate_first is None else bool(aggregate_first)
        if self.L < 2:
            self.agg_first = False

        if _prebuilt_graph is not None:
            self.G = self.Gt = _prebuilt_graph
            self.N = _prebuilt_graph.n_rows
        else:
            norm = gcn_norm(adj)
            self.G: CsrGraph = norm.storage.engine_csr()
            self.Gt: CsrGraph = self.G if _is_symmetric(norm) else norm.storage.engine_csc("value")
        self.nnz = self.G.nnz

        shapes = []
        for l in range(self.L):
            shapes += [(dims[l], dims[l + 1]), (dims[l + 1],)]
            if l < self.L - 1:
                shapes += [(dims[l + 1],), (dims[l + 1],)]
        dev = self.device
        self.store = FlatParams(shapes, dev).attach(self)
        self.W, self.b, self.gamma, self.beta = [], [], [], []
        self.gW, self.gb, self.ggamma, self.gbeta = [], [], [], []
        views = iter(self.store.views)
        for l in range(self.L):
            (w, gw), (b, gb) = next(views), next(views)
            self.W.append(w); self.gW.append(gw); self.b.append(b); self.gb.append(gb)
            if l < self.L - 1:
                (g, gg), (be, gbe) = next(views), next(views)
                self.gamma.append(g); self.ggamma.append(gg); self.beta.append(be); self.gbeta.append(gbe)
        self.Wt_split = [(torch.empty(dims[l + 1], dims[l], device=dev), torch.empty(dims[l + 1], dims[l], device=dev))
                         for l in range(self.L)]
        self.W_split = [(torch.empty(dims[l], dims[l + 1], device=dev), torch.empty(dims[l], dims[l + 1], device=dev))
                        for l in range(self.L)]
        wg = [ops.wgrad_supported(dims[l], dims[l + 1]) for l in range(self.L)]
        self.wgrad_ws = (torch.empty(max(ops.wgrad_workspace_floats(dims[l], dims[l + 1]) for l in range(self.L) if wg[l]), device=dev)
                         if self.tc_gemm and any(wg) else None)
        self.running_mean = [torch.zeros(d, device=dev) for d in dims[1:-1]]
        self.running_var = [torch.ones(d, device=dev) for d in dims[1:-1]]
        self.reset_parameters(seed)

        N = self.N
        rows_alloc = N if _rows_alloc is None else _rows_alloc
        self._blocks = []

        def buf(k):
            blk = torch.zeros(rows_alloc, k, device=dev)
            self._blocks.append(blk)
            return blk[:N]
        self.H = [buf(dims[l + 1]) for l in range(self.L)]
        self.Y = [buf(dims[l + 1]) for l in range(self.L)]
        self._A = [buf(dims[l + 1]) for l in range(self.L - 1)]
        self.dY = [buf(dims[l + 1]) for l in range(self.L)]
        self.dH = [buf(dims[l + 1]) for l in range(self.L)]
        self.dA = [buf(dims[l + 1]) for l in range(self.L - 1)]
        self.AX = buf(dims[0]) if self.agg_first else None
        slots_spmm = ops.stat_slots(self.G)
        self.stat_part = [torch.empty(slots_spmm, 2, dims[l + 1], device=dev) for l in range(self.L - 1)]
        self.bn = [torch.empty(4, dims[l + 1], device=dev) for l in range(self.L - 1)]
        self.rs = ops.rows_slots(N)
        self.fuse_rows = bool(fuse_row_passes) and self.tc_gemm
        self._gemm_part = {k: torch.empty(ops.gemm_stat_slots(N, k), 2, k, device=dev)
                           for k in set(dims[1:-1]) if self.fuse_rows and ops.gemm_stats_supported(k)}
        hid = dims[1:-1]
        self.fuse_act = (bool(fuse_activations) and self.fuse_rows and self.L >= 2 and len(set(hid)) == 1
                         and ops.gemm_stats_supported(hid[0]) and hid[0] <= 2048
                         and all(ops.wgrad_supported(dims[l], dims[l + 1]) for l in range(1, self.L)))
        self.keep_bits = (torch.zeros(self.L - 1, N, (hid[0] + 31) // 32, dtype=torch.int32, device=dev)
                          if self.fuse_act else None)
        self._act_stale = False
        self._fwd_fused = False
        self._ev_bits = torch.cuda.Event()
        self.kd_part = torch.empty(2 * int(lib.load().b200gnn_kd_partials(N)), device=dev)
        self.overlap_wgrad = overlap_wgrad
        self._side = torch.cuda.Stream(device=dev) if overlap_wgrad else None
        self._ev_fork, self._ev_join = torch.cuda.Event(), torch.cuda.Event()
        self._static: Dict[str, torch.Tensor] = {}
        for k in set(dims[1:]):
            self._part(k); self._coef(k)
        if self.objective is not None:
            self.objective.bind(self)

    def reset_parameters(self, seed: int = 0):
        g = torch.Generator().manual_seed(seed)
        for l in range(self.L):
            fan_in, fan_out = self.dims[l], self.dims[l + 1]
            a = math.sqrt(6.0 / (fan_in + fan_out))
            self.W[l].copy_((torch.rand(fan_in, fan_out, generator=g) * 2 - 1) * a)
            self.b[l].zero_()
        for l in range(self.L - 1):
            self.gamma[l].fill_(1.0); self.beta[l].zero_()
            self.running_mean[l].zero_(); self.running_var[l].fill_(1.0)
        self.exp_avg.zero_(); self.exp_avg_sq.zero_(); self.step_count.zero_()

    def state_dict(self) -> Dict[str, torch.Tensor]:
        sd = {}
        for l in range(self.L):
            sd[f"convs.{l}.weight"] = self.W[l].detach().clone()
            sd[f"convs.{l}.bias"] = self.b[l].detach().clone()
        for l in range(self.L - 1):
            sd[f"bns.{l}.weight"] = self.gamma[l].detach().clone()
            sd[f"bns.{l}.bias"] = self.beta[l].detach().clone()
            sd[f"bns.{l}.running_mean"] = self.running_mean[l].clone()
            sd[f"bns.{l}.running_var"] = self.running_var[l].clone()
        return sd

    def load_state_dict(self, sd: Dict[str, torch.Tensor]):
        for l in range(self.L):
            self.W[l].copy_(sd[f"convs.{l}.weight"]); self.b[l].copy_(sd[f"convs.{l}.bias"])
        for l in range(self.L - 1):
            self.gamma[l].copy_(sd[f"bns.{l}.weight"]); self.beta[l].copy_(sd[f"bns.{l}.bias"])
            if f"bns.{l}.running_mean" in sd:
                self.running_mean[l].copy_(sd[f"bns.{l}.running_mean"]); self.running_var[l].copy_(sd[f"bns.{l}.running_var"])

    @property
    def A(self) -> List[torch.Tensor]:
        if self._act_stale:
            self._act_stale = False
            for l in range(self.L - 1):
                ops.affine_relu_bits(self.Y[l], self.keep_bits[l], self.bn[l][2], self.bn[l][3], self.p, out=self._A[l])
        return self._A

    def _act(self, l: int):
        return self.Y[l], self.bn[l][2], self.bn[l][3], self.keep_bits[l]

    def activation_pattern(self, l: int) -> torch.Tensor:
        return self.A[l] > 0

    def out_feat(self) -> torch.Tensor:
        return self.A[-1]

    def forward(self, x: torch.Tensor, training: bool = True) -> torch.Tensor:
        fused = training and self.fuse_act
        self._act_stale = False
        if fused:
            if self._side is not None:
                self._ev_fork.record(torch.cuda.current_stream())
                self._side.wait_event(self._ev_fork)
                with torch.cuda.stream(self._side):
                    ops.dropout_bits(self.keep_bits, self.p, self.seed, 0, step_dev=self.step_count, step_mul=self.L)
                self._ev_bits.record(self._side)
            else:
                ops.dropout_bits(self.keep_bits, self.p, self.seed, 0, step_dev=self.step_count, step_mul=self.L)
        A = self._A
        inp = x
        for l in range(self.L):
            last = l == self.L - 1
            if l == 0 and self.agg_first:
                ops.spmm_csr(self.G, x, "sum", out=self.AX)
                if training:
                    gp = self._gemm_part.get(self.dims[1])
                    if gp is not None:
                        hi, lo = ops.split_tf32(self.W[0], transpose=True, hi=self.Wt_split[0][0], lo=self.Wt_split[0][1])
                        ops.gemm_tf32x3_stats(self.AX, hi, lo, self.b[0], self.Y[0], gp)
                        part = gp
                    else:
                        self._linear(0, self.AX, self.Y[0], bias=self.b[0])
                        part = ops.col_stats(self.Y[0], partial=self._part(self.dims[1]))
                    ops.bn_finalize(part, self.N, self.gamma[0], self.beta[0], self.bn_eps,
                                    self.bn_momentum, self.running_mean[0], self.running_var[0], out=self.bn[0])
                    if not fused:
                        ops.affine_relu_dropout(self.Y[0], self.bn[0][2], self.bn[0][3], True, self.p, self.seed, 0,
                                                out=A[0], step_dev=self.step_count, step_mul=self.L)
                else:
                    self._linear(0, self.AX, self.Y[0], bias=self.b[0])
                    scale = self.gamma[0] * torch.rsqrt(self.running_var[0] + self.bn_eps)
                    shift = self.beta[0] - self.running_mean[0] * scale
                    ops.affine_relu_dropout(self.Y[0], scale, shift, True, 0.0, out=A[0])
                inp = A[0]
                continue
            if fused and l > 0:
                if l == 1 and self._side is not None:
                    torch.cuda.current_stream().wait_event(self._ev_bits)
                self._linear(l, None, self.H[l], act=self._act(l - 1))
            else:
                self._linear(l, inp, self.H[l])
            if last:
                ops.spmm_csr(self.G, self.H[l], "sum", bias=self.b[l], out=self.Y[l])
            elif training:
                ops.spmm_csr(self.G, self.H[l], "sum", bias=self.b[l], out=self.Y[l], stat_partial=self.stat_part[l])
                ops.bn_finalize(self.stat_part[l], self.N, self.gamma[l], self.beta[l], self.bn_eps, self.bn_momentum,
                                self.running_mean[l], self.running_var[l], out=self.bn[l])
                if not fused:
                    ops.affine_relu_dropout(self.Y[l], self.bn[l][2], self.bn[l][3], True, self.p, self.seed, l,
                                            out=A[l], step_dev=self.step_count, step_mul=self.L)
                inp = A[l]
            else:
                ops.spmm_csr(self.G, self.H[l], "sum", bias=self.b[l], out=self.Y[l])
                scale = self.gamma[l] * torch.rsqrt(self.running_var[l] + self.bn_eps)
                shift = self.beta[l] - self.running_mean[l] * scale
                ops.affine_relu_dropout(self.Y[l], scale, shift, True, 0.0, out=A[l])
                inp = A[l]
        self._act_stale = self._fwd_fused = fused
        return self.Y[-1]

    def backward(self, x: torch.Tensor, d_out_feat: Optional[torch.Tensor] = None):
        fused = self._fwd_fused
        for l in range(self.L - 1, -1, -1):
            act = self._act(l - 1) if fused and l > 0 else None
            inp = x if l == 0 else (None if act else self._A[l - 1])
            if l == self.L - 1:
                ops.col_sum(self.dY[l], out=self.gb[l], partial=self._part(self.dims[l + 1]))
            if l == 0 and self.agg_first:
                self._wgrad_async(0, self.AX, self.dY[0])
                continue
            ops.spmm_csr(self.Gt, self.dY[l], "sum", out=self.dH[l])
            d_prev = self.dA[l - 1] if l > 0 else None
            gp = self._gemm_part.get(self.dims[l]) if l > 0 else None
            if l > 0:
                acc = d_out_feat is not None and l == self.L - 1
                if acc:
                    d_prev = d_out_feat
                if gp is not None:
                    hi, lo = ops.split_tf32(self.W[l], transpose=False, hi=self.W_split[l][0], lo=self.W_split[l][1])
                    if act:
                        ops.gemm_tf32x3_bnbwd_bits(self.dH[l], hi, lo, d_prev, act[3], self.Y[l - 1], self.bn[l - 1][0],
                                                   self.bn[l - 1][1], act[1], act[2], self.p, gp, accumulate=acc)
                    else:
                        ops.gemm_tf32x3_bnbwd(self.dH[l], hi, lo, d_prev, self._A[l - 1], self.Y[l - 1], self.bn[l - 1][0],
                                              self.bn[l - 1][1], self.p, gp, accumulate=acc)
                else:
                    self._linear_dgrad(l, self.dH[l], d_prev, accumulate=acc)
            self._wgrad_async(l, inp, self.dH[l], act=act)
            if l > 0:
                k = self.dims[l]
                part = self._part(k)
                if gp is not None:
                    ops.bn_act_bwd_apply(d_prev, None, self.Y[l - 1], self.bn[l - 1][0], self.bn[l - 1][1], self.gamma[l - 1],
                                         gp, self.N, self.p, self.dY[l - 1], self.ggamma[l - 1], self.gbeta[l - 1],
                                         self.gb[l - 1], part, self._coef(k))
                else:
                    ops.bn_act_bwd(d_prev, self._A[l - 1], self.Y[l - 1], self.bn[l - 1][0], self.bn[l - 1][1],
                                   self.gamma[l - 1], self.p, d_y=self.dY[l - 1], d_gamma=self.ggamma[l - 1],
                                   d_beta=self.gbeta[l - 1], d_bias=self.gb[l - 1], partial=part, coef=self._coef(k))
        self._wgrad_join()

    def _wgrad_async(self, l: int, inp: Optional[torch.Tensor], d_out: torch.Tensor, act=None):
        if self._side is None:
            return self._linear_wgrad(l, inp, d_out, act)
        self._ev_fork.record(torch.cuda.current_stream())
        self._side.wait_event(self._ev_fork)
        with torch.cuda.stream(self._side):
            self._linear_wgrad(l, inp, d_out, act)

    def _wgrad_join(self):
        if self._side is not None:
            self._ev_join.record(self._side)
            torch.cuda.current_stream().wait_event(self._ev_join)

    def _linear(self, l: int, inp: Optional[torch.Tensor], out: torch.Tensor, bias: Optional[torch.Tensor] = None, act=None):
        if act is not None:
            hi, lo = ops.split_tf32(self.W[l], transpose=True, hi=self.Wt_split[l][0], lo=self.Wt_split[l][1])
            ops.gemm_tf32x3_act(*act, self.p, hi, lo, bias=bias, out=out)
        elif self.tc_gemm:
            hi, lo = ops.split_tf32(self.W[l], transpose=True, hi=self.Wt_split[l][0], lo=self.Wt_split[l][1])
            ops.gemm_tf32x3(inp, hi, lo, bias=bias, out=out)
        elif bias is not None:
            torch.addmm(bias, inp, self.W[l], out=out)
        else:
            torch.mm(inp, self.W[l], out=out)

    def _linear_dgrad(self, l: int, d_out: torch.Tensor, d_inp: torch.Tensor, accumulate: bool = False):
        if self.tc_gemm:
            hi, lo = ops.split_tf32(self.W[l], transpose=False, hi=self.W_split[l][0], lo=self.W_split[l][1])
            ops.gemm_tf32x3(d_out, hi, lo, out=d_inp, accumulate=accumulate)
        elif accumulate:
            d_inp.addmm_(d_out, self.W[l].t())
        else:
            torch.mm(d_out, self.W[l].t(), out=d_inp)

    def _linear_wgrad(self, l: int, inp: Optional[torch.Tensor], d_out: torch.Tensor, act=None):
        if act is not None:
            ops.gemm_wgrad_tf32x3_act(*act, self.p, d_out, out=self.gW[l], workspace=self.wgrad_ws)
        elif self.tc_gemm and ops.wgrad_supported(self.dims[l], self.dims[l + 1]):
            ops.gemm_wgrad_tf32x3(inp, d_out, out=self.gW[l], workspace=self.wgrad_ws)
        else:
            torch.mm(inp.t(), d_out, out=self.gW[l])

    def replay(self, key: int = 0) -> torch.Tensor:
        super().replay(key)
        self._act_stale = self.fuse_act
        return self.loss_out

    def aggregations_per_step(self) -> Dict[int, int]:
        out: Dict[int, int] = {}
        for l in range(self.L):
            if l == 0 and self.agg_first:
                out[self.dims[0]] = out.get(self.dims[0], 0) + 1
            else:
                out[self.dims[l + 1]] = out.get(self.dims[l + 1], 0) + 2
        return out

    def spmm_algorithmic_bytes(self) -> Dict[int, int]:
        return {k: 2 * self.N * k * 4 + self.nnz * 8 + (self.N + 1) * 4 for k in set(self.dims)}
```

efficient-gnns_b200/lib.py:

```python
from __future__ import annotations

import ctypes as C
import os
from pathlib import Path

import torch

PKG_DIR = Path(__file__).resolve().parent
LIB_PATH = PKG_DIR / "libb200gnn.so"

OK = 0
REDUCE_SUM = 0
REDUCE_MEAN = 1
LSP_MAX_F = 512

_i32p = C.c_void_p
_f32p = C.c_void_p
_ptr = C.c_void_p
_i64 = C.c_int64
_i32 = C.c_int32
_int = C.c_int
_f32 = C.c_float
_f64 = C.c_double
_u64 = C.c_uint64

SIGNATURES = {
    "b200gnn_abi_version": (_int, []),
    "b200gnn_error_string": (C.c_char_p, [_int]),
    "b200gnn_last_cuda_error": (C.c_char_p, []),
    "b200gnn_launch_count": (_i64, []),
    "b200gnn_reset_launch_count": (None, []),
    "b200gnn_csr_chunk_count": (_i64, [_i64, _i64, _i32, _i32]),
    "b200gnn_csr_chunk_plan": (_int, [_i32p, _i64, _i64, _i32, _i32, _i32p, _ptr]),
    "b200gnn_csr_hub_count": (_int, [_i32p, _i64, _i32, _i32, _i32p, _ptr]),
    "b200gnn_csr_hub_fill": (_int, [_i32p, _i64, _i32, _i32, _i32p, _i32p, _i64, _ptr]),
    "b200gnn_spmm_stat_slots": (_i64, [_i64, _i64]),
    "b200gnn_spmm_set_variant": (None, [_int]),
    "b200gnn_spmm_csr_f32": (_int, [_i32p, _i32p, _f32p, _f32p, _i64, _f32p, _i64, _i64, _i64, _i64, _int,
                                    _f32p, _f32p, _i32p, _i64, _i32, _i32, _i32p, _i32p, _i64, _i64, _f32p, _ptr]),
    "b200gnn_spmm_csr_scatter_f32": (_int, [_i32p, _i32p, _f32p, _f32p, _i64, _ptr, _ptr, _i32, _i64, _i64, _i64, _i64, _i64, _int,
                                            _f32p, _i32p, _i64, _i32, _i32, _i32p, _i32p, _i64, _i64, _f32p, _ptr]),
    "b200gnn_rows_slots": (_i64, [_i64]),
    "b200gnn_col_stats_f32": (_int, [_f32p, _i64, _i64, _f32p, _i64, _ptr]),
    "b200gnn_col_sum_f32": (_int, [_f32p, _i64, _i64, _f32p, _f32p, _i64, _ptr]),
    "b200gnn_bn_finalize_f32": (_int, [_f32p, _i64, _i64, _i64, _f32p, _f32p, _f32, _f32, _f32p, _f32p,
                                       _f32p, _f32p, _f32p, _f32p, _ptr]),
    "b200gnn_affine_relu_dropout_f32": (_int, [_f32p, _f32p, _i64, _i64, _f32p, _f32p, _int, _f32, _u64, _u64,
                                               _i32p, _u64, _u64, _ptr]),
    "b200gnn_affine_relu_dropout_mapped_f32": (_int, [_f32p, _f32p, _i64, _i64, _f32p, _f32p, _int, _f32, _u64, _u64,
                                                      _i32p, _u64, _i32p, _u64, _i64, _i64, _ptr]),
    "b200gnn_affine_relu_dropout_scatter_f32": (_int, [_f32p, _f32p, _i64, _i64, _f32p, _f32p, _int, _f32, _u64, _u64,
                                                       _i32p, _u64, _i32p, _u64, _i64, _i64, _ptr, _ptr, _i32, _i64, _ptr]),
    "b200gnn_dropout_mask_u8": (_int, [_ptr, _i64, _i64, _f32, _u64, _u64, _ptr]),
    "b200gnn_dropout_mask_step_u8": (_int, [_ptr, _i64, _i64, _f32, _u64, _u64, _i32p, _u64, _ptr]),
    "b200gnn_dropout_bits_u32": (_int, [_ptr, _i64, _i64, _i64, _f32, _u64, _u64, _i32p, _u64, _ptr]),
    "b200gnn_affine_relu_bits_f32": (_int, [_f32p, _ptr, _f32p, _f32p, _f32, _f32p, _i64, _i64, _ptr]),
    "b200gnn_gather_rows_act_f32": (_int, [_f32p, _i64, _ptr, _i64, _i64, _ptr, _f32p, _f32p, _f32, _f32p, _ptr]),
    "b200gnn_relu_dropout_bwd_f32": (_int, [_f32p, _f32p, _f32p, _i64, _i64, _f32, _ptr]),
    "b200gnn_bn_act_bwd_f32": (_int, [_f32p, _f32p, _f32p, _f32p, _f32p, _f32p, _i64, _i64, _f32, _f32p, _f32p,
                                      _f32p, _f32p, _f32p, _i64, _f32p, _ptr]),
    "b200gnn_bn_act_bwd_reduce_f32": (_int, [_f32p, _f32p, _f32p, _f32p, _f32p, _i64, _i64, _f32, _f32p, _i64, _ptr]),
    "b200gnn_bn_act_bwd_apply_f32": (_int, [_f32p, _f32p, _f32p, _f32p, _f32p, _f32p, _f32p, _i64, _i64, _i64, _i64, _f32,
                                            _f32p, _f32p, _f32p, _f32p, _f32p, _i64, _f32p, _ptr]),
    "b200gnn_partial_reduce_f32": (_int, [_f32p, _i64, _i64, _f32p, _ptr]),
    "b200gnn_adam_step_f32": (_int, [_f32p, _f32p, _f32p, _f32p, _i64, _f32, _f32, _f32, _f32, _i32p, _ptr]),
    "b200gnn_rmsprop_step_f32": (_int, [_f32p, _f32p, _f32p, _i64, _f64, _i64, _f64, _f64, _f64, _i32p, _ptr]),
    "b200gnn_teacher_slots": (_i64, [_i64]),
    "b200gnn_label_inputs_f32": (_int, [_f32p, _i64, _i64, _i64, _i64, _i32p, _ptr, _int, _f32, _u64, _u64, _i32p, _u64, _ptr,
                                        _int, _ptr, _i32p, _ptr]),
    "b200gnn_label_softmax_f32": (_int, [_f32p, _i64, _i64, _i64, _ptr, _int, _f32p, _i64, _ptr]),
    "b200gnn_logce_fwd_bwd_f32": (_int, [_f32p, _i64, _i64, _ptr, _i64, _ptr, _ptr, _i32p, _i64, _f32p, _i64, _f32p, _f32p,
                                         _ptr, _ptr]),
    "b200gnn_split_eval_f32": (_int, [_f32p, _i64, _i64, _ptr, _i64, _i64, _i64, _ptr, _f32p, _f32p, _ptr, _ptr]),
    "b200gnn_snapshot_if_better_f32": (_int, [_f32p, _f32p, _f32p, _f32p, _i64, _f32p, _f32p, _i64, _f32p, _f32p, _i64, _ptr]),
    "b200gnn_kd_partials": (_i64, [_i64]),
    "b200gnn_kd_loss_fwd_bwd_f32": (_int, [_f32p, _i64, _ptr, _i64, _ptr, _f32p, _i64, _i64, _f32, _f32, _i64, _f32p,
                                           _i64, _f32p, _f32p, _ptr]),
    "b200gnn_split_tf32_f32": (_int, [_f32p, _i64, _i64, _int, _f32p, _f32p, _ptr]),
    "b200gnn_gemm_tf32x3_f32": (_int, [_f32p, _i64, _f32p, _f32p, _i64, _f32p, _i64, _i64, _i64, _i64, _f32p, _ptr]),
    "b200gnn_random_walk_i64": (_int, [_i32p, _i32p, _i64, _ptr, _i64, _i32, _u64, _u64, _ptr, _ptr]),
    "b200gnn_saint_subgraph_count_i64": (_int, [_i32p, _i32p, _ptr, _i64, _i32p, _ptr, _ptr]),
    "b200gnn_saint_subgraph_fill_i64": (_int, [_i32p, _i32p, _ptr, _ptr, _i64, _i32p, _ptr, _ptr, _ptr, _ptr, _ptr]),
    "b200gnn_gemm_stat_slots": (_i64, [_i64, _i64]),
    "b200gnn_gemm_set_bnbwd_variant": (None, [_int]),
    "b200gnn_gemm_tf32x3_stats_f32": (_int, [_f32p, _i64, _f32p, _f32p, _i64, _f32p, _i64, _i64, _i64, _i64, _f32p, _int, _f32p, _i64,
                                             _ptr]),
    "b200gnn_gemm_tf32x3_bnbwd_f32": (_int, [_f32p, _i64, _f32p, _f32p, _i64, _f32p, _i64, _i64, _i64, _i64, _int,
                                             _f32p, _f32p, _f32p, _f32p, _f32, _f32p, _i64, _ptr]),
    "b200gnn_gemm_tf32x3_bnbwd_bits_f32": (_int, [_f32p, _i64, _f32p, _f32p, _i64, _f32p, _i64, _i64, _i64, _i64, _int,
                                                  _ptr, _f32p, _f32p, _f32p, _f32p, _f32p, _f32, _f32p, _i64, _ptr]),
    "b200gnn_gemm_tf32x3_act_f32": (_int, [_f32p, _i64, _f32p, _f32p, _i64, _f32p, _i64, _i64, _i64, _i64, _f32p,
                                           _f32p, _f32p, _ptr, _f32, _ptr]),
    "b200gnn_gemm_tf32x3_acc_f32": (_int, [_f32p, _i64, _f32p, _f32p, _i64, _f32p, _i64, _i64, _i64, _i64, _ptr]),
    "b200gnn_gemm_tf32x3_rowidx_f32": (_int, [_f32p, _i64, _f32p, _f32p, _i64, _f32p, _i64, _i64, _i64, _i64, _ptr, _ptr]),
    "b200gnn_gemm_tf32x3_scatter_f32": (_int, [_f32p, _i64, _f32p, _f32p, _i64, _ptr, _i32, _i64, _i64, _i64, _i64, _f32p, _ptr]),
    "b200gnn_gemm_tf32x3_bcast_f32": (_int, [_f32p, _i64, _f32p, _f32p, _i64, _ptr, _i32, _i64, _i64, _i64, _i64, _i64, _f32p, _ptr]),
    "b200gnn_wgrad_workspace_floats": (_i64, [_i64, _i64]),
    "b200gnn_gemm_wgrad_tf32x3_f32": (_int, [_f32p, _i64, _f32p, _i64, _f32p, _i64, _i64, _i64, _f32p, _ptr]),
    "b200gnn_gemm_wgrad_tf32x3_act_f32": (_int, [_f32p, _i64, _f32p, _i64, _f32p, _i64, _i64, _i64, _f32p, _f32p, _ptr, _f32,
                                                 _f32p, _ptr]),
    "b200gnn_gemm_tf32x3_prelu_f32": (_int, [_f32p, _i64, _f32p, _f32p, _i64, _f32p, _i64, _i64, _i64, _i64, _f32p,
                                             _f32p, _ptr, _f32, _ptr]),
    "b200gnn_gemm_tf32x3_prelu_bwd_f32": (_int, [_f32p, _i64, _f32p, _f32p, _i64, _f32p, _i64, _i64, _i64, _i64, _int,
                                                 _f32p, _ptr, _f32p, _f32, _f32p, _int, _ptr, _i64, _ptr]),
    "b200gnn_gemm_wgrad_tf32x3_prelu_f32": (_int, [_f32p, _i64, _f32p, _i64, _f32p, _i64, _i64, _i64, _f32p, _ptr, _i64, _f32,
                                                   _f32p, _ptr]),
    "b200gnn_prelu_bits_f32": (_int, [_f32p, _i64, _ptr, _i64, _f32p, _f32, _f32p, _i64, _i64, _i64, _ptr]),
    "b200gnn_sign_gather_f32": (_int, [_ptr, _i32, _i64, _i64, _ptr, _i64, _f32, _u64, _u64, _i32p, _u64, _f32p, _ptr, _ptr,
                                       _f32p, _i64, _i64, _f32p, _ptr]),
    "b200gnn_col_sum_ld_slots": (_i64, [_i64]),
    "b200gnn_col_sum_ld_f32": (_int, [_f32p, _i64, _i64, _i64, _f32p, _f32p, _i64, _ptr]),
    "b200gnn_row_normalize_fwd_f32": (_int, [_f32p, _i64, _i64, _f32, _f32, _f32p, _f32p, _ptr]),
    "b200gnn_row_normalize_bwd_f32": (_int, [_f32p, _f32p, _f32p, _i64, _i64, _f32, _f32, _f32p, _int, _ptr]),
    "b200gnn_reduce_slots": (_i64, [_i64]),
    "b200gnn_mse_fwd_bwd_f32": (_int, [_f32p, _f32p, _i64, _f32, _f32p, _f32p, _f32p, _ptr]),
    "b200gnn_bce_logits_fwd_bwd_f32": (_int, [_f32p, _f32p, _int, _i64, _f32, _f32p, _f32p, _f32p, _ptr]),
    "b200gnn_row_sqnorm_f32": (_int, [_f32p, _i64, _i64, _f32p, _ptr]),
    "b200gnn_row_sqnorm_bwd_f32": (_int, [_f32p, _f32p, _i64, _i64, _f32p, _ptr]),
    "b200gnn_nce_rows_f32": (_int, [_f32p, _i64, _f32p, _f32p, _ptr]),
    "b200gnn_nce_rows_chunk_f32": (_int, [_f32p, _i64, _i64, _i64, _i64, _f32p, _ptr]),
    "b200gnn_nce_finish_f32": (_int, [_f32p, _i64, _f32p, _ptr]),
    "b200gnn_gcrd_sample_workspace_bytes": (_i64, [_i64]),
    "b200gnn_gcrd_sample_i32": (_int, [_i64, _u64, _u64, _i32p, _i32p, _ptr, _ptr]),
    "b200gnn_gcrd_operands_f32": (_int, [_i32p, _i64, _i64, _f32p, _f32p, _f32p, _f32p, _f32, _f32, _f32p, _f32p, _f32p, _f32p,
                                         _ptr]),
    "b200gnn_gcrd_bwd_slots": (_i64, []),
    "b200gnn_gcrd_backward_f32": (_int, [_i32p, _i64, _i64, _f32p, _f32p, _f32p, _f32p, _f32p, _f32p, _f32, _f32, _f32p, _f32p,
                                         _f32p, _f32p, _f32, _f32p, _f32p, _f32p, _f32p, _f32p, _f32p, _ptr]),
    "b200gnn_transpose_f32": (_int, [_f32p, _i64, _i64, _f32p, _ptr]),
    "b200gnn_gsp_pair_f32": (_int, [_f32p, _f32p, _f32p, _f32p, _i64, _int, _f32p, _f32p, _f32p, _ptr]),
    "b200gnn_gsp_pair_chunk_f32": (_int, [_f32p, _f32p, _i64, _i64, _i64, _i64, _f32p, _f32p, _int, _f32p, _f32p, _f32p, _ptr]),
# ... 121 lines not shown
```

efficient-gnns_b200/ops.py:

```python
from __future__ import annotations

from typing import Optional, Tuple

import torch

from . import lib
from .sparse import CsrGraph, SparseTensor

_REDUCE = {"sum": lib.REDUCE_SUM, "add": lib.REDUCE_SUM, "mean": lib.REDUCE_MEAN}


def set_spmm_variant(variant: int) -> None:
    lib.load().b200gnn_spmm_set_variant(int(variant))


def stat_slots(g: CsrGraph) -> int:
    return int(lib.load().b200gnn_spmm_stat_slots(g.n_chunks, g.n_hub))


def spmm_csr(g: CsrGraph, x: torch.Tensor, reduce: str = "sum", bias: Optional[torch.Tensor] = None,
             out: Optional[torch.Tensor] = None, stat_partial: Optional[torch.Tensor] = None) -> torch.Tensor:
    if reduce not in _REDUCE:
        raise ValueError(f"reduce={reduce!r}: the engine implements sum/add/mean (what the reference path uses)")
    if x.dim() != 2:
        raise lib.B200GnnError("spmm: dense operand must be [n_src, K]")
    if x.shape[0] < g.n_cols:
        raise lib.B200GnnError(
            f"spmm: dense operand has {x.shape[0]} rows, matrix has {g.n_cols} columns")
    K = x.shape[1]
    if out is None:
        out = torch.empty(g.n_rows, K, dtype=torch.float32, device=x.device)
    if g.n_rows == 0 or K == 0:
        return out
    L = lib.load()
    ws = g.hub_workspace(K)
    rc = L.b200gnn_spmm_csr_f32(
        lib.dptr(g.rowptr, torch.int32, "rowptr"), lib.dptr(g.col, torch.int32, "col"),
        lib.dptr(g.val, torch.float32, "val"), lib.dptr(x, torch.float32, "x"), x.stride(0),
        lib.dptr(out, torch.float32, "out"), out.stride(0), g.n_rows, g.n_cols, K, _REDUCE[reduce],
        lib.dptr(bias, torch.float32, "bias"), lib.dptr(stat_partial, torch.float32, "stat_partial"),
        g.chunk_rowptr.data_ptr(), g.n_chunks, g.hub_threshold, g.seg_len,
        g.hub_rows.data_ptr() if g.n_hub else None, g.hub_segptr.data_ptr() if g.n_hub else None,
        g.n_hub, g.n_seg, None if ws is None else ws.data_ptr(), lib.stream_ptr())
    lib.check(rc, "spmm_csr_f32")
    return out


def _host_ptr_array(ptrs):
    import ctypes as C
    return (C.c_void_p * len(ptrs))(*[C.c_void_p(int(p)) for p in ptrs])


def _host_i32_array(vals):
    import ctypes as C
    return (C.c_int32 * len(vals))(*[int(v) for v in vals])


def spmm_csr_scatter(g: CsrGraph, x: torch.Tensor, dst_ptrs, row_off, ld_dst: int, col_dst: int, reduce: str = "sum",
                     bias: Optional[torch.Tensor] = None) -> None:
    K = x.shape[1]
    L = lib.load()
    ws = g.hub_workspace(K)
    rc = L.b200gnn_spmm_csr_scatter_f32(
        lib.dptr(g.rowptr, torch.int32, "rowptr"), lib.dptr(g.col, torch.int32, "col"), lib.dptr(g.val, torch.float32, "val"),
        lib.dptr(x, torch.float32, "x"), x.stride(0), _host_ptr_array(dst_ptrs), _host_i32_array(row_off), len(dst_ptrs),
        int(ld_dst), int(col_dst), g.n_rows, g.n_cols, K, _REDUCE[reduce], lib.dptr(bias, torch.float32, "bias"),
        g.chunk_rowptr.data_ptr(), g.n_chunks, g.hub_threshold, g.seg_len,
        g.hub_rows.data_ptr() if g.n_hub else None, g.hub_segptr.data_ptr() if g.n_hub else None,
        g.n_hub, g.n_seg, None if ws is None else ws.data_ptr(), lib.stream_ptr())
    lib.check(rc, "spmm_csr_scatter_f32")


class _SpMM(torch.autograd.Function):

    @staticmethod
    def forward(ctx, x, adj: SparseTensor, reduce: str):
        st = adj.storage
        g = st.engine_csr() if st.value() is not None else st.engine_csr_unweighted()
        ctx.adj, ctx.reduce = adj, reduce
        return spmm_csr(g, x.contiguous(), reduce)

    @staticmethod
    def backward(ctx, grad_out):
        st = ctx.adj.storage
        if ctx.reduce == "mean":
            gt = st.engine_csc("mean" if st.value() is None else "mean_value")
        else:
            gt = st.engine_csc("value")
        return spmm_csr(gt, grad_out.contiguous(), "sum"), None, None


def matmul(adj: SparseTensor, x: torch.Tensor, reduce: str = "sum") -> torch.Tensor:
    if reduce not in _REDUCE:
        raise ValueError(f"reduce={reduce!r} not implemented (reference path uses add/mean)")
    v = adj.storage.value()
    if v is not None and v.requires_grad:
        raise NotImplementedError("gradients w.r.t. sparse values are never taken on the reference path")
# ... 125 lines not shown
        n, K, None if bits is None else _bits(bits, x.shape[0], K), _f32(scale, "scale"), _f32(shift, "shift"), float(p),
        _f32(out, "out"), lib.stream_ptr()), "gather_rows_act_f32")
    return out


def lsp_student(feat: torch.Tensor, src: torch.Tensor, dst: torch.Tensor, rowptr: torch.Tensor, sim_t: torch.Tensor, kernel: int,
                pos_dst: torch.Tensor, pos_src: torch.Tensor, comb_rowptr: torch.Tensor, diag_pos: torch.Tensor,
                sim_s: torch.Tensor, scratch: torch.Tensor, val: torch.Tensor, selfc: torch.Tensor, loss: torch.Tensor,
                partial: torch.Tensor) -> None:
    E, n_seg, n_nodes = src.numel(), rowptr.numel() - 1, comb_rowptr.numel() - 1
    assert dst.numel() == E and sim_t.numel() == E and sim_s.numel() == E and scratch.numel() >= 2 * E
    assert pos_dst.numel() == E and pos_src.numel() == E and diag_pos.numel() == n_nodes and feat.shape[0] >= n_nodes
    assert val.numel() == selfc.numel() == 2 * E + n_nodes and partial.numel() >= int(lib.load().b200gnn_lsp_partials(n_seg))
    i32 = lambda t, name: lib.dptr(t, torch.int32, name)
    lib.check(lib.load().b200gnn_lsp_student_f32(
        _f32(feat, "feat"), feat.shape[1], i32(src, "src"), i32(dst, "dst"), i32(rowptr, "rowptr"), n_seg, E,
        _f32(sim_t, "sim_t"), int(kernel), i32(pos_dst, "pos_dst"), i32(pos_src, "pos_src"), i32(comb_rowptr, "comb_rowptr"),
        i32(diag_pos, "diag_pos"), n_nodes, _f32(sim_s, "sim_s"), _f32(scratch, "scratch"), _f32(val, "val"),
        _f32(selfc, "selfc"), _f32(loss, "loss"), _f32(partial, "partial"), lib.stream_ptr()), "lsp_student_f32")


def scatter_rows_scaled(src: torch.Tensor, idx: torch.Tensor, scale: float, out: torch.Tensor,
                        loss_aux: Optional[torch.Tensor] = None, loss_total: Optional[torch.Tensor] = None) -> torch.Tensor:
    n, K = src.shape
    assert idx.numel() == n and out.dim() == 2 and out.shape[1] == K and out.stride(1) == 1
    if out.dtype != torch.float32 or not out.is_cuda:
        raise lib.B200GnnError("scatter_rows_scaled: out must be a float32 CUDA tensor")
    lib.check(lib.load().b200gnn_scatter_rows_scaled_f32(
        _f32(src, "src"), lib.dptr(idx, torch.int64, "idx"), n, K, float(scale), out.data_ptr(), out.stride(0),
        _f32(loss_aux, "loss_aux"), _f32(loss_total, "loss_total"), lib.stream_ptr()), "scatter_rows_scaled_f32")
    return out


def bn_act_bwd(d_out, x_out, y, mean, invstd, gamma, p: float, d_y=None, d_gamma=None, d_beta=None, d_bias=None,
               partial=None, coef=None, want_dbias: bool = True):
    n, K = y.shape
    dev = y.device
    slots = rows_slots(n)
    d_y = torch.empty_like(y) if d_y is None else d_y
    d_gamma = torch.empty(K, device=dev) if d_gamma is None else d_gamma
    d_beta = torch.empty(K, device=dev) if d_beta is None else d_beta
    if want_dbias and d_bias is None:
        d_bias = torch.empty(K, device=dev)
    partial = torch.empty(slots, 2, K, device=dev) if partial is None else partial
    coef = torch.empty(3, K, device=dev) if coef is None else coef
    lib.check(lib.load().b200gnn_bn_act_bwd_f32(
        _f32(d_out, "d_out"), _f32(x_out, "x_out"), _f32(y, "y"), _f32(mean, "mean"), _f32(invstd, "invstd"),
        _f32(gamma, "gamma"), n, K, p, _f32(d_y, "d_y"), _f32(d_gamma, "d_gamma"), _f32(d_beta, "d_beta"),
        _f32(d_bias, "d_bias") if want_dbias else None, _f32(partial, "partial"), slots, _f32(coef, "coef"),
        lib.stream_ptr()), "bn_act_bwd_f32")
    return d_y, d_gamma, d_beta, d_bias


def adam_step(params, grads, exp_avg, exp_avg_sq, step: torch.Tensor, lr: float, betas=(0.9, 0.999), eps: float = 1e-8):
    lib.check(lib.load().b200gnn_adam_step_f32(
        _f32(params, "params"), _f32(grads, "grads"), _f32(exp_avg, "exp_avg"), _f32(exp_avg_sq, "exp_avg_sq"),
        params.numel(), lr, betas[0], betas[1], eps, lib.dptr(step, torch.int32, "step"), lib.stream_ptr()),
        "adam_step_f32")


def kd_loss_fwd_bwd(logits, labels, train_idx, teacher_logits=None, alpha: float = 0.9, T: float = 4.0,
                    d_logits=None, loss_out=None, partial=None, n_norm: int = 0):
    N, C = logits.shape
    n_train = train_idx.numel() if train_idx is not None else N
    L = lib.load()
    if d_logits is None:
        d_logits = torch.zeros_like(logits)
    if loss_out is None:
        loss_out = torch.empty(3, dtype=torch.float32, device=logits.device)
    if partial is None:
        partial = torch.empty(2 * int(L.b200gnn_kd_partials(max(n_train, 1))), dtype=torch.float32, device=logits.device)
    lib.check(L.b200gnn_kd_loss_fwd_bwd_f32(
        _f32(logits, "logits"), logits.stride(0), lib.dptr(train_idx, torch.int64, "train_idx"), n_train,
        lib.dptr(labels, torch.int64, "labels"), _f32(teacher_logits, "teacher_logits"),
        teacher_logits.stride(0) if teacher_logits is not None else 0, C, alpha, T, n_norm, _f32(d_logits, "d_logits"),
        d_logits.stride(0), _f32(loss_out, "loss_out"), _f32(partial, "partial"), lib.stream_ptr()), "kd_loss_fwd_bwd_f32")
    return loss_out, d_logits


def split_tf32(w: torch.Tensor, transpose: bool = False, hi: Optional[torch.Tensor] = None,
               lo: Optional[torch.Tensor] = None) -> Tuple[torch.Tensor, torch.Tensor]:
    rows, cols = w.shape
    shape = (cols, rows) if transpose else (rows, cols)
    hi = torch.empty(shape, dtype=torch.float32, device=w.device) if hi is None else hi
    lo = torch.empty(shape, dtype=torch.float32, device=w.device) if lo is None else lo
    lib.check(lib.load().b200gnn_split_tf32_f32(_f32(w, "w"), rows, cols, int(transpose), _f32(hi, "hi"), _f32(lo, "lo"),
                                                lib.stream_ptr()), "split_tf32_f32")
    return hi, lo


def gemm_tf32x3(a: torch.Tensor, b_hi: torch.Tensor, b_lo: torch.Tensor, bias: Optional[torch.Tensor] = None,
                out: Optional[torch.Tensor] = None, accumulate: bool = False) -> torch.Tensor:
    M, K = a.shape
    N = b_hi.shape[0]
    assert b_hi.shape == b_lo.shape and b_hi.shape[1] == K
    if out is None:
        assert not accumulate
        out = torch.empty(M, N, dtype=torch.float32, device=a.device)
    L = lib.load()
    if accumulate:
        assert bias is None
        lib.check(L.b200gnn_gemm_tf32x3_acc_f32(_f32(a, "a"), a.stride(0), _f32(b_hi, "b_hi"), _f32(b_lo, "b_lo"),
                                                b_hi.stride(0), _f32(out, "out"), out.stride(0), M, N, K, lib.stream_ptr()),
                  "gemm_tf32x3_acc_f32")
        return out
    lib.check(L.b200gnn_gemm_tf32x3_f32(_f32(a, "a"), a.stride(0), _f32(b_hi, "b_hi"), _f32(b_lo, "b_lo"),
                                        b_hi.stride(0), _f32(out, "out"), out.stride(0), M, N, K,
                                        _f32(bias, "bias"), lib.stream_ptr()), "gemm_tf32x3_f32")
    return out


def gemm_stat_slots(m: int, n: int) -> int:
    return int(lib.load().b200gnn_gemm_stat_slots(m, n))


def gemm_stats_supported(n: int) -> bool:
    return n % 32 == 0 and 48 < n <= 256


def gemm_tf32x3_stats(a: torch.Tensor, b_hi: torch.Tensor, b_lo: torch.Tensor, bias: Optional[torch.Tensor], out: torch.Tensor,
                      partial: torch.Tensor, accumulate: bool = False) -> torch.Tensor:
    M, K = a.shape
    N = b_hi.shape[0]
    lib.check(lib.load().b200gnn_gemm_tf32x3_stats_f32(_f32(a, "a"), a.stride(0), _f32(b_hi, "b_hi"), _f32(b_lo, "b_lo"),
                                                       b_hi.stride(0), _f32(out, "out"), out.stride(0), M, N, K, _f32(bias, "bias"),
                                                       int(accumulate), _f32(partial, "partial"), partial.shape[0], lib.stream_ptr()),
              "gemm_tf32x3_stats_f32")
    return out


def gemm_tf32x3_bnbwd(a: torch.Tensor, b_hi: torch.Tensor, b_lo: torch.Tensor, out: torch.Tensor, x_out: torch.Tensor,
                      y: torch.Tensor, mean: torch.Tensor, invstd: torch.Tensor, p: float, partial: torch.Tensor,
                      accumulate: bool = False) -> torch.Tensor:
    M, K = a.shape
    N = b_hi.shape[0]
    assert out.shape == x_out.shape == y.shape and out.stride(0) == x_out.stride(0) == y.stride(0)
    lib.check(lib.load().b200gnn_gemm_tf32x3_bnbwd_f32(_f32(a, "a"), a.stride(0), _f32(b_hi, "b_hi"), _f32(b_lo, "b_lo"),
                                                       b_hi.stride(0), _f32(out, "out"), out.stride(0), M, N, K, int(accumulate),
                                                       _f32(x_out, "x_out"), _f32(y, "y"), _f32(mean, "mean"),
                                                       _f32(invstd, "invstd"), float(p), _f32(partial, "partial"),
                                                       partial.shape[0], lib.stream_ptr()), "gemm_tf32x3_bnbwd_f32")
# ... 537 lines not shown
```

efficient-gnns_b200/sparse.py:

```python
from __future__ import annotations

from dataclasses import dataclass, field, replace
from typing import Optional, Tuple

import torch

from . import lib

HUB_THRESHOLD = 256
HUB_SEG_LEN = 256
CHUNK_NNZ = 128
CHUNK_ROW_COST = 4


def _narrow_i32(t: torch.Tensor, what: str) -> torch.Tensor:
    if t.numel() and int(t.max()) >= 2 ** 31 - 1:
        raise lib.B200GnnError(f"{what}: index >= 2^31-1 cannot be narrowed to the engine's int32")
    return t.to(torch.int32).contiguous()


@dataclass
class CsrGraph:
    rowptr: torch.Tensor
    col: torch.Tensor
# ... 6 lines not shown
    row_cost: int = 0
    chunk_rowptr: Optional[torch.Tensor] = None
    n_chunks: int = 0
    hub_rows: Optional[torch.Tensor] = None
    hub_segptr: Optional[torch.Tensor] = None
    n_hub: int = 0
    n_seg: int = 0
    _ws: dict = field(default_factory=dict)

    @property
    def nnz(self) -> int:
        return int(self.col.numel())

    @property
    def device(self):
        return self.rowptr.device

    def build_plan(self, hub_threshold: Optional[int] = None, seg_len: Optional[int] = None,
                   chunk_nnz: Optional[int] = None, row_cost: Optional[int] = None) -> "CsrGraph":
        self.hub_threshold = HUB_THRESHOLD if hub_threshold is None else hub_threshold
        self.seg_len = HUB_SEG_LEN if seg_len is None else seg_len
        self.chunk_nnz = CHUNK_NNZ if chunk_nnz is None else chunk_nnz
        self.row_cost = CHUNK_ROW_COST if row_cost is None else row_cost
        self._ws.clear()
        L = lib.load()
        st = lib.stream_ptr()
        self.n_chunks = int(L.b200gnn_csr_chunk_count(self.n_rows, self.nnz, self.chunk_nnz, self.row_cost))
        self.chunk_rowptr = torch.zeros(self.n_chunks + 1, dtype=torch.int32, device=self.device)
        if self.n_rows > 0:
            lib.check(L.b200gnn_csr_chunk_plan(lib.dptr(self.rowptr, torch.int32, "rowptr"), self.n_rows, self.nnz,
                                               self.chunk_nnz, self.row_cost, self.chunk_rowptr.data_ptr(), st),
                      "csr_chunk_plan")
        counts = torch.zeros(2, dtype=torch.int32, device=self.device)
        lib.check(L.b200gnn_csr_hub_count(lib.dptr(self.rowptr, torch.int32, "rowptr"), self.n_rows,
                                          self.hub_threshold, self.seg_len, counts.data_ptr(), st), "csr_hub_count")
        n_hub, n_seg = (int(v) for v in counts.tolist())
        self.hub_segptr = torch.zeros(n_hub + 1, dtype=torch.int32, device=self.device)
        self.hub_rows = torch.zeros(max(n_hub, 1), dtype=torch.int32, device=self.device)
        lib.check(L.b200gnn_csr_hub_fill(self.rowptr.data_ptr(), self.n_rows, self.hub_threshold, self.seg_len,
                                         self.hub_rows.data_ptr(), self.hub_segptr.data_ptr(), n_hub, st),
                  "csr_hub_fill")
        self.n_hub, self.n_seg = n_hub, n_seg
        return self

    def hub_workspace(self, K: int) -> Optional[torch.Tensor]:
        if self.n_seg == 0:
            return None
        ws = self._ws.get(K)
        if ws is None:
            ws = torch.empty(self.n_seg * K, dtype=torch.float32, device=self.device)
            self._ws[K] = ws
        return ws


def csr_graph_from(rowptr64: torch.Tensor, col64: torch.Tensor, val: Optional[torch.Tensor],
                   n_rows: int, n_cols: int) -> CsrGraph:
    if not rowptr64.is_cuda:
        raise lib.B200GnnError("engine graphs live on a CUDA device; there is no CPU fallback")
    g = CsrGraph(_narrow_i32(rowptr64, "rowptr"), _narrow_i32(col64, "col"),
                 None if val is None else val.to(torch.float32).contiguous(), n_rows, n_cols)
    return g.build_plan()


def ind2ptr(ind: torch.Tensor, size: int) -> torch.Tensor:
    counts = torch.bincount(ind, minlength=size) if ind.numel() else torch.zeros(size, dtype=torch.long, device=ind.device)
    ptr = torch.zeros(size + 1, dtype=torch.long, device=ind.device)
    torch.cumsum(counts, 0, out=ptr[1:])
    return ptr


def ptr2ind(ptr: torch.Tensor, nnz: int) -> torch.Tensor:
    counts = ptr[1:] - ptr[:-1]
    return torch.repeat_interleave(torch.arange(counts.numel(), device=ptr.device), counts, output_size=nnz)


def _on_engine_device(*ts) -> bool:
    return all(t is not None and t.is_cuda for t in ts)


def device_argsort(major: torch.Tensor, minor: torch.Tensor, major_size: int, minor_size: int) -> torch.Tensor:
    n = int(major.numel())
    if n == 0 or not _on_engine_device(major, minor) or n >= 2 ** 31 - 1 or float(major_size) * float(minor_size) >= 1.8e19:
        return torch.argsort(major * minor_size + minor, stable=True)
    L = lib.load()
    ws = torch.empty(int(L.b200gnn_graph_sort_workspace_bytes(n)), dtype=torch.uint8, device=major.device)
    perm = torch.empty(n, dtype=torch.int32, device=major.device)
    ma, mi = major.contiguous(), minor.contiguous()
    lib.check(L.b200gnn_graph_argsort_i64(ma.data_ptr(), mi.data_ptr(), n, int(major_size), int(minor_size), perm.data_ptr(),
                                          ws.data_ptr(), lib.stream_ptr()), "graph_argsort_i64")
    return perm.long()


def device_coalesce(row: torch.Tensor, col: torch.Tensor, n_rows: int, n_cols: int):
    n = int(row.numel())
    L = lib.load()
    dev = row.device
    ws = torch.empty(int(L.b200gnn_graph_sort_workspace_bytes(n)), dtype=torch.uint8, device=dev)
    out_row, out_col = torch.empty(n, dtype=torch.long, device=dev), torch.empty(n, dtype=torch.long, device=dev)
    src = torch.empty(n, dtype=torch.int32, device=dev)
    rowptr = torch.empty(n_rows + 1, dtype=torch.long, device=dev)
    nnz = torch.zeros(1, dtype=torch.long, device=dev)
    r, c = row.contiguous(), col.contiguous()
    lib.check(L.b200gnn_graph_coalesce_i64(r.data_ptr(), c.data_ptr(), n, int(n_rows), int(n_cols), out_row.data_ptr(),
                                           out_col.data_ptr(), src.data_ptr(), rowptr.data_ptr(), nnz.data_ptr(), ws.data_ptr(),
                                           lib.stream_ptr()), "graph_coalesce_i64")
    k = int(nnz.item())
# ... 212 lines not shown
```

efficient-gnns_b200/trainer.py:

```python
from __future__ import annotations

import contextlib
import math
from typing import Callable, Optional, Sequence, Tuple

import torch

from . import lib, ops


class FlatParams:

    def __init__(self, shapes: Sequence[Tuple[int, ...]], device):
        sizes = [math.prod(s) for s in shapes]
        n = sum(sizes)
        self.n_par_pad = (n + 3) // 4 * 4
        self.params = torch.zeros(n, device=device)
        self._grads_buf = torch.zeros(self.n_par_pad + 4, device=device)
        self.grads = self._grads_buf[:n]
        self.loss_out = self._grads_buf[self.n_par_pad:self.n_par_pad + 3]
        self.exp_avg = torch.zeros(n, device=device)
        self.exp_avg_sq = torch.zeros(n, device=device)
        self.step_count = torch.zeros(1, dtype=torch.int32, device=device)
        self.views = []
        off = 0
        for k, s in zip(sizes, shapes):
            self.views.append((self.params[off:off + k].view(s), self.grads[off:off + k].view(s)))
            off += k

    def attach(self, owner) -> "FlatParams":
        for k in ("params", "grads", "_grads_buf", "n_par_pad", "loss_out", "exp_avg", "exp_avg_sq", "step_count"):
            setattr(owner, k, getattr(self, k))
        return self

    @staticmethod
    def offset(view: torch.Tensor) -> int:
        return view.storage_offset()

    def like(self, buf: torch.Tensor, view: torch.Tensor) -> torch.Tensor:
        o = self.offset(view)
        return buf[o:o + view.numel()].view(view.shape)

    def adam(self, lr: float):
        ops.adam_step(self.params, self.grads, self.exp_avg, self.exp_avg_sq, self.step_count, lr)

    @contextlib.contextmanager
    def preserved(self):
        state = (self.params, self.exp_avg, self.exp_avg_sq, self.step_count)
        saved = [t.clone() for t in state]
        yield
        for t, v in zip(state, saved):
            t.copy_(v)


def aux_grad(out_feat: torch.Tensor, aux: Callable, beta: float):
    feat = out_feat.detach().requires_grad_(True)
    with torch.enable_grad():
        loss_aux = aux(feat)
        (loss_aux * beta).backward()
    d_feat = feat.grad if feat.grad is not None else torch.zeros_like(feat)
    return d_feat.contiguous(), loss_aux.detach()


def capture_graph(step: Callable[[], None], warmup: int) -> torch.cuda.CUDAGraph:
    s = torch.cuda.Stream()
    s.wait_stream(torch.cuda.current_stream())
    with torch.cuda.stream(s):
        for _ in range(warmup):
            step()
    torch.cuda.current_stream().wait_stream(s)
    torch.cuda.synchronize()
    g = torch.cuda.CUDAGraph()
    with torch.cuda.graph(g):
        step()
    return g


def one_objective(gcrd=None, lsp=None, gsp=None):
    if gcrd is not None and lsp is not None:
        raise ValueError("gcrd= and lsp= are two auxiliary losses; pass one")
    if gsp is not None and (gcrd is not None or lsp is not None):
        raise ValueError("gsp= and the gcrd= / lsp= objective are two auxiliary losses; pass one")
    return next((o for o in (gcrd, lsp, gsp) if o is not None), None)


class FullBatchStudent:

    objective = None
    _graph = None

    def dropout_offset(self, layer: int, step: int) -> int:
        return layer + step * self.L

    def _part(self, k: int) -> torch.Tensor:
        key = f"part{k}"
        if key not in self._static:
            self._static[key] = torch.empty(self.rs, 2, k, device=self.device)
# ... 54 lines not shown
```

include/b200gnn.h:

```cpp
#ifndef B200GNN_H_
#define B200GNN_H_

#include <stdint.h>

#ifdef __cplusplus
extern "C" {
#endif

#define B200GNN_OK 0
#define B200GNN_ERR_BAD_ARG (-1)
#define B200GNN_ERR_UNSUPPORTED (-2)
#define B200GNN_ERR_CUDA (-3)

#define B200GNN_REDUCE_SUM 0
#define B200GNN_REDUCE_MEAN 1

#define B200GNN_ABI_VERSION 2

int b200gnn_abi_version(void);
const char* b200gnn_error_string(int code);
const char* b200gnn_last_cuda_error(void);
int64_t b200gnn_launch_count(void);
void b200gnn_reset_launch_count(void);

int64_t b200gnn_csr_chunk_count(int64_t n_rows, int64_t nnz, int32_t chunk_nnz,
                                int32_t row_cost);
int b200gnn_csr_chunk_plan(const int32_t* rowptr, int64_t n_rows, int64_t nnz,
                           int32_t chunk_nnz, int32_t row_cost,
                           int32_t* chunk_rowptr, void* stream);

int b200gnn_csr_hub_count(const int32_t* rowptr, int64_t n_rows,
                          int32_t hub_threshold, int32_t seg_len,
                          int32_t* counts_out, void* stream);
int b200gnn_csr_hub_fill(const int32_t* rowptr, int64_t n_rows,
                         int32_t hub_threshold, int32_t seg_len,
                         int32_t* hub_rows, int32_t* hub_segptr,
                         int64_t n_hub, void* stream);

int64_t b200gnn_spmm_stat_slots(int64_t n_chunks, int64_t n_hub);
void b200gnn_spmm_set_variant(int variant);
int b200gnn_spmm_csr_f32(const int32_t* rowptr, const int32_t* col,
                         const float* val, const float* X, int64_t ldx,
                         float* Y, int64_t ldy, int64_t n_rows, int64_t n_src,
                         int64_t K, int reduce, const float* bias,
                         float* stat_partial, const int32_t* chunk_rowptr,
                         int64_t n_chunks, int32_t hub_threshold,
                         int32_t seg_len, const int32_t* hub_rows,
                         const int32_t* hub_segptr, int64_t n_hub,
                         int64_t n_seg, float* hub_workspace, void* stream);
int b200gnn_spmm_csr_scatter_f32(const int32_t* rowptr, const int32_t* col, const float* val, const float* X,
                                 int64_t ldx, float* const* Y_ptrs, const int32_t* row_off, int32_t world,
                                 int64_t ldy_dst, int64_t col_dst, int64_t n_rows, int64_t n_src, int64_t K,
                                 int reduce, const float* bias, const int32_t* chunk_rowptr, int64_t n_chunks,
                                 int32_t hub_threshold, int32_t seg_len, const int32_t* hub_rows,
                                 const int32_t* hub_segptr, int64_t n_hub, int64_t n_seg,
                                 float* hub_workspace, void* stream);

int64_t b200gnn_rows_slots(int64_t n_rows);
int b200gnn_col_stats_f32(const float* Y, int64_t n_rows, int64_t K,
                          float* partial, int64_t slots, void* stream);
int b200gnn_col_sum_f32(const float* Y, int64_t n_rows, int64_t K, float* out,
                        float* partial, int64_t slots, void* stream);
int b200gnn_bn_finalize_f32(const float* partial, int64_t slots, int64_t K,
                            int64_t n_rows, const float* gamma,
                            const float* beta, float eps, float momentum,
                            float* running_mean, float* running_var,
                            float* mean_out, float* invstd_out,
                            float* scale_out, float* shift_out, void* stream);
int b200gnn_affine_relu_dropout_f32(const float* Y, float* out, int64_t n_rows,
                                    int64_t K, const float* scale,
                                    const float* shift, int relu, float p,
                                    uint64_t seed, uint64_t offset,
                                    const int32_t* step_dev, uint64_t step_mul,
                                    uint64_t row_offset, void* stream);
int b200gnn_affine_relu_dropout_mapped_f32(const float* Y, float* out, int64_t n_rows, int64_t K,
                                           const float* scale, const float* shift, int relu, float p,
                                           uint64_t seed, uint64_t offset, const int32_t* step_dev,
                                           uint64_t step_mul, const int32_t* rowmap, uint64_t row_offset,
                                           int64_t K_global, int64_t col_offset, void* stream);
int b200gnn_affine_relu_dropout_scatter_f32(const float* Y, float* out, int64_t n_rows, int64_t K,
                                            const float* scale, const float* shift, int relu, float p,
                                            uint64_t seed, uint64_t offset, const int32_t* step_dev,
                                            uint64_t step_mul, const int32_t* rowmap, uint64_t row_offset,
                                            int64_t K_global, int64_t col_offset, float* const* dst_ptrs,
                                            const int32_t* row_off, int32_t world, int64_t ld_dst, void* stream);
int b200gnn_dropout_mask_u8(uint8_t* mask, int64_t n_rows, int64_t K, float p,
                            uint64_t seed, uint64_t offset, void* stream);
int b200gnn_dropout_mask_step_u8(uint8_t* mask, int64_t n_rows, int64_t K, float p, uint64_t seed, uint64_t offset,
                                 const int32_t* step_dev, uint64_t step_mul, void* stream);
int b200gnn_dropout_bits_u32(uint32_t* bits, int64_t n_layers, int64_t n_rows, int64_t K, float p, uint64_t seed,
                             uint64_t offset, const int32_t* step_dev, uint64_t step_mul, void* stream);
int b200gnn_affine_relu_bits_f32(const float* Y, const uint32_t* bits, const float* scale, const float* shift,
                                 float p, float* out, int64_t n_rows, int64_t K, void* stream);
int b200gnn_gather_rows_act_f32(const float* X, int64_t ldx, const int64_t* idx, int64_t n_idx, int64_t K,
                                const uint32_t* bits, const float* scale, const float* shift, float p, float* out,
                                void* stream);
int b200gnn_relu_dropout_bwd_f32(const float* dOut, const float* Xout, float* dY,
                                 int64_t n_rows, int64_t K, float p, void* stream);
int b200gnn_bn_act_bwd_f32(const float* dOut, const float* Xout, const float* Y,
                           const float* mean, const float* invstd,
                           const float* gamma, int64_t n_rows, int64_t K,
                           float p, float* dY, float* dgamma, float* dbeta,
                           float* dbias, float* partial, int64_t slots,
                           float* coef, void* stream);
int b200gnn_bn_act_bwd_reduce_f32(const float* dOut, const float* Xout,
                                  const float* Y, const float* mean,
                                  const float* invstd, int64_t n_rows,
                                  int64_t K, float p, float* partial,
                                  int64_t slots, void* stream);
int b200gnn_bn_act_bwd_apply_f32(const float* dOut, const float* Xout,
                                 const float* Y, const float* mean,
                                 const float* invstd, const float* gamma,
                                 const float* sums, int64_t sum_slots,
                                 int64_t n_norm, int64_t n_rows, int64_t K,
                                 float p, float* dY, float* dgamma,
                                 float* dbeta, float* dbias, float* partial,
                                 int64_t slots, float* coef, void* stream);
int b200gnn_partial_reduce_f32(const float* partial, int64_t slots, int64_t K2,
                               float* out, void* stream);
int b200gnn_adam_step_f32(float* params, const float* grads, float* exp_avg,
                          float* exp_avg_sq, int64_t n, float lr, float beta1,
                          float beta2, float eps, int32_t* step, void* stream);
int b200gnn_rmsprop_step_f32(float* params, const float* grads, float* square_avg, int64_t n, double lr, int64_t warmup,
                             double alpha, double eps, double weight_decay, int32_t* step, void* stream);

int64_t b200gnn_teacher_slots(int64_t n_items);
int b200gnn_label_inputs_f32(float* X, int64_t ldx, int64_t col0, int64_t C, int64_t n_rows, const int32_t* row_pos,
                             const int64_t* labels, int eval, float mask_rate, uint64_t seed, uint64_t offset,
                             const int32_t* step_dev, uint64_t step_mul, const uint8_t* mask_in, int use_labels, uint8_t* role,
                             int32_t* cnt_part, void* stream);
int b200gnn_label_softmax_f32(const float* logits, int64_t ld, int64_t C, int64_t n_rows, const uint8_t* role, int role_mask,
                              float* out, int64_t ldo, void* stream);
int b200gnn_logce_fwd_bwd_f32(const float* logits, int64_t ld, int64_t C, const int64_t* train_idx, int64_t n_train,
                              const int64_t* labels, const uint8_t* role, const int32_t* cnt_part, int64_t n_cnt,
                              float* dlogits, int64_t ldd, float* loss_out, float* acc_out, double* partial, void* stream);
int b200gnn_split_eval_f32(const float* logits, int64_t ld, int64_t C, const int64_t* idx, int64_t n0, int64_t n1, int64_t n2,
                           const int64_t* labels, float* loss_out, float* acc_out, double* partial, void* stream);
int b200gnn_snapshot_if_better_f32(const float* cand, float* best, const float* src0, float* dst0, int64_t n0,
                                   const float* src1, float* dst1, int64_t n1, const float* src2, float* dst2, int64_t n2,
                                   void* stream);

int64_t b200gnn_kd_partials(int64_t n_train);
int b200gnn_kd_loss_fwd_bwd_f32(const float* logits, int64_t ld,
                                const int64_t* train_idx, int64_t n_train,
                                const int64_t* labels,
                                const float* teacher_logits, int64_t ldt,
                                int64_t C, float alpha, float T,
                                int64_t n_norm, float* dlogits, int64_t ldd,
                                float* loss_out, float* partial, void* stream);

int b200gnn_split_tf32_f32(const float* W, int64_t rows, int64_t cols,
                           int transpose, float* hi, float* lo, void* stream);
int b200gnn_gemm_tf32x3_f32(const float* A, int64_t lda, const float* B_hi,
                            const float* B_lo, int64_t ldb, float* C,
                            int64_t ldc, int64_t M, int64_t N, int64_t K,
                            const float* bias, void* stream);
int b200gnn_gemm_tf32x3_acc_f32(const float* A, int64_t lda, const float* B_hi, const float* B_lo,
                                int64_t ldb, float* C, int64_t ldc, int64_t M, int64_t N, int64_t K,
                                void* stream);
int b200gnn_gemm_tf32x3_rowidx_f32(const float* A, int64_t lda, const float* B_hi, const float* B_lo,
                                   int64_t ldb, float* C, int64_t ldc, int64_t M, int64_t N, int64_t K,
                                   const int64_t* row_idx, void* stream);
int64_t b200gnn_gemm_stat_slots(int64_t M, int64_t N);
void b200gnn_gemm_set_bnbwd_variant(int v);
int b200gnn_gemm_tf32x3_stats_f32(const float* A, int64_t lda, const float* B_hi, const float* B_lo, int64_t ldb,
                                  float* C, int64_t ldc, int64_t M, int64_t N, int64_t K, const float* bias,
                                  int accumulate, float* partial, int64_t slots, void* stream);
int b200gnn_gemm_tf32x3_bnbwd_f32(const float* A, int64_t lda, const float* B_hi, const float* B_lo, int64_t ldb,
                                  float* C, int64_t ldc, int64_t M, int64_t N, int64_t K, int accumulate,
                                  const float* Xout, const float* Y, const float* mean, const float* invstd, float p_drop,
                                  float* partial, int64_t slots, void* stream);
int b200gnn_gemm_tf32x3_bnbwd_bits_f32(const float* A, int64_t lda, const float* B_hi, const float* B_lo, int64_t ldb,
                                       float* C, int64_t ldc, int64_t M, int64_t N, int64_t K, int accumulate,
                                       const uint32_t* bits, const float* Y, const float* mean, const float* invstd,
                                       const float* scale, const float* shift, float p_drop, float* partial,
                                       int64_t slots, void* stream);
int b200gnn_gemm_tf32x3_act_f32(const float* Y, int64_t lda, const float* B_hi, const float* B_lo, int64_t ldb,
                                float* C, int64_t ldc, int64_t M, int64_t N, int64_t K, const float* bias,
                                const float* scale, const float* shift, const uint32_t* bits, float p_drop,
                                void* stream);
int b200gnn_gemm_tf32x3_scatter_f32(const float* A, int64_t lda, const float* B_hi, const float* B_lo,
                                    int64_t ldb, float* const* C_ptrs, int32_t world, int64_t row_off,
                                    int64_t M, int64_t N, int64_t K, const float* bias, void* stream);
int b200gnn_gemm_tf32x3_bcast_f32(const float* A, int64_t lda, const float* B_hi, const float* B_lo,
                                  int64_t ldb, float* const* C_ptrs, int32_t world, int64_t row_off, int64_t ldc,
                                  int64_t M, int64_t N, int64_t K, const float* bias, void* stream);

int64_t b200gnn_wgrad_workspace_floats(int64_t Kin, int64_t Nout);
int b200gnn_gemm_wgrad_tf32x3_f32(const float* X, int64_t ldx, const float* G,
                                  int64_t ldg, float* dW, int64_t Nn,
                                  int64_t Kin, int64_t Nout, float* workspace,
                                  void* stream);
int b200gnn_gemm_wgrad_tf32x3_act_f32(const float* Y, int64_t ldx, const float* G, int64_t ldg, float* dW,
                                      int64_t Nn, int64_t Kin, int64_t Nout, const float* scale, const float* shift,
                                      const uint32_t* bits, float p_drop, float* workspace, void* stream);

int b200gnn_gemm_tf32x3_prelu_f32(const float* Z, int64_t lda, const float* B_hi, const float* B_lo, int64_t ldb,
                                  float* C, int64_t ldc, int64_t M, int64_t N, int64_t K, const float* bias,
                                  const float* slope, const uint32_t* bits, float p_drop, void* stream);
int b200gnn_gemm_tf32x3_prelu_bwd_f32(const float* A, int64_t lda, const float* B_hi, const float* B_lo, int64_t ldb,
                                      float* C, int64_t ldc, int64_t M, int64_t N, int64_t K, int accumulate,
                                      const float* Z, const uint32_t* bits, const float* slope, float p_drop,
                                      float* slope_grad, int slope_accumulate, double* partial, int64_t slots,
                                      void* stream);
int b200gnn_gemm_wgrad_tf32x3_prelu_f32(const float* Z, int64_t ldz, const float* G, int64_t ldg, float* dW,
// ... 205 lines not shown
```

Baseline: 3.986 billion.

## Fuse hub finalize and Adam tick via tickets, batch TF32 splits, unroll finalize loads

```diff
diff --git a/efficient-gnns_b200/csrc/dense_rows.cu b/efficient-gnns_b200/csrc/dense_rows.cu
--- a/efficient-gnns_b200/csrc/dense_rows.cu
+++ b/efficient-gnns_b200/csrc/dense_rows.cu
@@ -54,18 +54,34 @@
   reduce_store_2xK(m, K, s, q, smem, partial + (size_t)blockIdx.x * 2 * K);
 }
 
-constexpr int FIN_COLS = 4, FIN_GROUPS = 64;
+constexpr int FIN_COLS = 4, FIN_GROUPS = 64, FIN_BATCH = 16;
 __device__ __forceinline__ bool finalize_reduce(const float* __restrict__ partial, int slots, int K, bool second,
                                                 double& s_out, double& q_out, int& k_out) {
   __shared__ double sh[2][FIN_GROUPS][FIN_COLS];
   const int c = threadIdx.x % FIN_COLS, g = threadIdx.x / FIN_COLS;
   const int k = blockIdx.x * FIN_COLS + c;
   double s = 0.0, q = 0.0;
-  if (k < K)
-    for (int j = g; j < slots; j += FIN_GROUPS) {
+  if (k < K) {
+    int j = g;
+    for (; j + (FIN_BATCH - 1) * FIN_GROUPS < slots; j += FIN_BATCH * FIN_GROUPS) {
+      float a[FIN_BATCH], b[FIN_BATCH];
+#pragma unroll
+      for (int u = 0; u < FIN_BATCH; ++u) {
+        const size_t o = (size_t)(j + u * FIN_GROUPS) * 2 * K + k;
+        a[u] = partial[o];
+        b[u] = second ? partial[o + K] : 0.f;
+      }
+#pragma unroll
+      for (int u = 0; u < FIN_BATCH; ++u) {
+        s += (double)a[u];
+        if (second) q += (double)b[u];
+      }
+    }
+    for (; j < slots; j += FIN_GROUPS) {
       s += (double)partial[(size_t)j * 2 * K + k];
       if (second) q += (double)partial[(size_t)j * 2 * K + K + k];
     }
+  }
   sh[0][g][c] = s; sh[1][g][c] = q;
   __syncthreads();
   if (g == 0 && k < K) {
@@ -421,14 +437,25 @@
   if (finalize_reduce(partial, slots, K, false, s, q, k)) out[k] = (float)s;
 }
 
+template <bool TICK>
 __global__ void __launch_bounds__(256) adam_kernel(float* __restrict__ p, const float* __restrict__ g,
                                                    float* __restrict__ m, float* __restrict__ v, int64_t n, float lr,
-                                                   float b1, float b2, float eps, const int32_t* __restrict__ step) {
+                                                   float b1, float b2, float eps, int32_t* step, int32_t* ticket) {
   const float t = (float)(*step + 1);
   const float bc1 = 1.f - powf(b1, t), bc2 = 1.f - powf(b2, t);
   const float step_size = lr / bc1, inv_sqrt_bc2 = rsqrtf(bc2);
   for (int64_t i = (int64_t)blockIdx.x * blockDim.x + threadIdx.x; i < n; i += (int64_t)gridDim.x * blockDim.x)
     adam_update(p[i], m[i], v[i], g[i], b1, b2, eps, step_size, inv_sqrt_bc2);
+  if (TICK) {
+    __syncthreads();
+    if (threadIdx.x == 0) {
+      __threadfence();
+      if (atomicAdd(ticket, 1) == (int)gridDim.x - 1) {
+        *ticket = 0;
+        *step += 1;
+      }
+    }
+  }
 }
 __global__ void adam_tick_kernel(int32_t* step) { *step += 1; }
 
@@ -717,10 +744,24 @@
   cudaStream_t st = (cudaStream_t)stream;
   int rc;
   if (n > 0) {
-    adam_kernel<<<grid_for(n, 256), 256, 0, st>>>(params, grads, exp_avg, exp_avg_sq, n, lr, beta1, beta2, eps, step);
+    adam_kernel<false><<<grid_for(n, 256), 256, 0, st>>>(params, grads, exp_avg, exp_avg_sq, n, lr, beta1, beta2, eps, step,
+                                                        nullptr);
     if ((rc = check_launch())) return rc;
   }
   adam_tick_kernel<<<1, 1, 0, st>>>(step);
+  return check_launch();
+}
+
+extern "C" int b200gnn_adam_step_ticket_f32(float* params, const float* grads, float* exp_avg, float* exp_avg_sq,
+                                            int64_t n, float lr, float beta1, float beta2, float eps, int32_t* step,
+                                            int32_t* ticket, void* stream) {
+  if (!params || !grads || !exp_avg || !exp_avg_sq || !step || !ticket || n < 0) return B200GNN_ERR_BAD_ARG;
+  cudaStream_t st = (cudaStream_t)stream;
+  if (n > 0)
+    adam_kernel<true><<<grid_for(n, 256), 256, 0, st>>>(params, grads, exp_avg, exp_avg_sq, n, lr, beta1, beta2, eps, step,
+                                                       ticket);
+  else
+    adam_tick_kernel<<<1, 1, 0, st>>>(step);
   return check_launch();
 }
 
diff --git a/efficient-gnns_b200/csrc/gemm_tf32x3.cu b/efficient-gnns_b200/csrc/gemm_tf32x3.cu
--- a/efficient-gnns_b200/csrc/gemm_tf32x3.cu
+++ b/efficient-gnns_b200/csrc/gemm_tf32x3.cu
@@ -446,6 +446,32 @@
   }
 }
 
+constexpr int SPLIT_BATCH_MAX = 16;
+struct SplitBatch {
+  const float* W[SPLIT_BATCH_MAX];
+  float* hi[SPLIT_BATCH_MAX];
+  float* lo[SPLIT_BATCH_MAX];
+  int64_t rows[SPLIT_BATCH_MAX], cols[SPLIT_BATCH_MAX];
+  int transpose[SPLIT_BATCH_MAX];
+};
+
+__global__ void __launch_bounds__(256) split_tf32_batch_kernel(const SplitBatch b) {
+  const int j = blockIdx.y;
+  const float* __restrict__ W = b.W[j];
+  float* __restrict__ hi = b.hi[j];
+  float* __restrict__ lo = b.lo[j];
+  const int64_t rows = b.rows[j], cols = b.cols[j], n = rows * cols;
+  const int transpose = b.transpose[j];
+  for (int64_t i = (int64_t)blockIdx.x * blockDim.x + threadIdx.x; i < n; i += (int64_t)gridDim.x * blockDim.x) {
+    const int64_t r = i / cols, c = i - r * cols;
+    uint32_t h, l;
+    split1(__float_as_uint(W[i]), h, l);
+    const int64_t o = transpose ? c * rows + r : i;
+    hi[o] = __uint_as_float(h);
+    lo[o] = __uint_as_float(l);
+  }
+}
+
 static bool make_map(CUtensorMap* m, const float* base, int64_t rows, int64_t cols, int64_t ld, int box_rows, bool swizzle = true) {
   EncodeTiledFn fn = encode_fn();
   if (!fn) return false;
@@ -500,6 +526,24 @@
   return check_launch();
 }
 
+extern "C" int b200gnn_split_tf32_batch_f32(const float* const* W, const int64_t* rows, const int64_t* cols,
+                                            const int32_t* transpose, float* const* hi, float* const* lo, int32_t n,
+                                            void* stream) {
+  if (!W || !rows || !cols || !transpose || !hi || !lo || n <= 0 || n > gemm::SPLIT_BATCH_MAX) return B200GNN_ERR_BAD_ARG;
+  gemm::SplitBatch b;
+  int64_t grid = 1;
+  for (int j = 0; j < n; ++j) {
+    if (!W[j] || !hi[j] || !lo[j] || rows[j] <= 0 || cols[j] <= 0) return B200GNN_ERR_BAD_ARG;
+    b.W[j] = W[j]; b.hi[j] = hi[j]; b.lo[j] = lo[j];
+    b.rows[j] = rows[j]; b.cols[j] = cols[j]; b.transpose[j] = transpose[j];
+    const int64_t g = (rows[j] * cols[j] + 255) / 256;
+    if (g > grid) grid = g;
+  }
+  if (grid > 132 * 8) grid = 132 * 8;
+  gemm::split_tf32_batch_kernel<<<dim3((unsigned)grid, (unsigned)n), 256, 0, (cudaStream_t)stream>>>(b);
+  return check_launch();
+}
+
 static int g_bnbwd_variant = 0;
 extern "C" void b200gnn_gemm_set_bnbwd_variant(int v) { g_bnbwd_variant = v; }
 
diff --git a/efficient-gnns_b200/csrc/spmm.cu b/efficient-gnns_b200/csrc/spmm.cu
--- a/efficient-gnns_b200/csrc/spmm.cu
+++ b/efficient-gnns_b200/csrc/spmm.cu
@@ -21,6 +21,7 @@
   const int32_t* hub_rows;
   const int32_t* hub_segptr;
   float* hub_ws;
+  int32_t* hub_ticket;
   int64_t ldx, ldy;
   int32_t n_rows, K, nvec;
   int32_t hub_threshold, seg_len, n_hub, n_seg, n_chunks;
@@ -204,7 +205,7 @@
 }
 
 template <typename V, int CH, bool HAS_VAL>
-__device__ __forceinline__ void spmm_hub_seg_cta(const SpmmParams& p, const int seg, float* s_buf, const int slab_lo = 0,
+__device__ __forceinline__ int spmm_hub_seg_cta(const SpmmParams& p, const int seg, float* s_buf, const int slab_lo = 0,
                                                  const int slab_hi = 1 << 30) {
   constexpr int W = VecTraits<V>::W;
 
@@ -257,12 +258,82 @@
     for (int i = threadIdx.x; i < slab_fn; i += SPMM_THREADS) ws[slab_f0 + i] = s_buf[i];
     __syncthreads();
   }
+  return h;
+}
+
+__device__ __forceinline__ void spmm_hub_finalize_row(const SpmmParams& p, const int h, float4* sh) {
+  const int row = __ldg(p.hub_rows + h);
+  const int s0 = __ldg(p.hub_segptr + h), s1 = __ldg(p.hub_segptr + h + 1);
+  const int deg = __ldg(p.rowptr + row + 1) - __ldg(p.rowptr + row);
+  float* stat = p.stat_partial ? p.stat_partial + (size_t)(p.main_grid + h) * 2 * p.K : nullptr;
+  const int nvec = p.K >> 2;
+  const auto al16 = [](const void* q) { return (reinterpret_cast<uintptr_t>(q) & 15) == 0; };
+  if ((p.K & 3) == 0 && nvec <= 256 && (p.ldy & 3) == 0 && al16(p.Y) && al16(p.hub_ws) && (!stat || al16(stat))) {
+    const int G = min(256 / nvec, 16);
+    const int v = threadIdx.x % nvec, g = threadIdx.x / nvec;
+    float4 acc = make_float4(0.f, 0.f, 0.f, 0.f);
+    if (g < G)
+      for (int s = s0 + g; s < s1; s += G) {
+        const float4 x = __ldcg(reinterpret_cast<const float4*>(p.hub_ws + (size_t)s * p.K + 4 * v));
+        acc.x += x.x; acc.y += x.y; acc.z += x.z; acc.w += x.w;
+      }
+    sh[threadIdx.x] = acc;
+    __syncthreads();
+    if (g != 0) return;
+    for (int j = 1; j < G; ++j) {
+      const float4 x = sh[j * nvec + v];
+      acc.x += x.x; acc.y += x.y; acc.z += x.z; acc.w += x.w;
+    }
+    if (p.mean) { const float d = (float)max(deg, 1); acc.x /= d; acc.y /= d; acc.z /= d; acc.w /= d; }
+    if (p.bias) {
+      acc.x += __ldg(p.bias + 4 * v); acc.y += __ldg(p.bias + 4 * v + 1);
+      acc.z += __ldg(p.bias + 4 * v + 2); acc.w += __ldg(p.bias + 4 * v + 3);
+    }
+    if (p.n_yp) y_row_v4(p, row)[v] = acc; else *reinterpret_cast<float4*>(p.Y + (size_t)row * p.ldy + 4 * v) = acc;
+    if (stat) {
+      *reinterpret_cast<float4*>(stat + 4 * v) = acc;
+      *reinterpret_cast<float4*>(stat + p.K + 4 * v) = make_float4(acc.x * acc.x, acc.y * acc.y, acc.z * acc.z, acc.w * acc.w);
+    }
+    return;
+  }
+  float* yrow = p.n_yp ? reinterpret_cast<float*>(y_row_v4(p, row)) : p.Y + (size_t)row * p.ldy;
+  for (int k = threadIdx.x; k < p.K; k += blockDim.x) {
+    float acc = 0.f;
+    for (int s = s0; s < s1; ++s) acc += __ldcg(p.hub_ws + (size_t)s * p.K + k);
+    if (p.mean) acc /= (float)max(deg, 1);
+    if (p.bias) acc += __ldg(p.bias + k);
+    yrow[k] = acc;
+    if (stat) { stat[k] = acc; stat[p.K + k] = acc * acc; }
+  }
+}
+
+__global__ void __launch_bounds__(256) spmm_hub_finalize_kernel(const SpmmParams p) {
+  __shared__ float4 sh[256];
+  spmm_hub_finalize_row(p, blockIdx.x, sh);
+}
+
+template <typename V, int CH, bool HAS_VAL>
+__device__ __forceinline__ void spmm_hub_cta(const SpmmParams& p, const int seg, float* s_buf, const int parts = 1,
+                                             const int slab_lo = 0, const int slab_hi = 1 << 30) {
+  const int h = spmm_hub_seg_cta<V, CH, HAS_VAL>(p, seg, s_buf, slab_lo, slab_hi);
+  if (!p.hub_ticket) return;
+  __threadfence();
+  __syncthreads();
+  int last = 0;
+  if (threadIdx.x == 0) {
+    const int need = (__ldg(p.hub_segptr + h + 1) - __ldg(p.hub_segptr + h)) * parts;
+    last = atomicAdd(p.hub_ticket + h, 1) == need - 1;
+    if (last) p.hub_ticket[h] = 0;
+  }
+  if (!__syncthreads_or(last)) return;
+  __threadfence();
+  spmm_hub_finalize_row(p, h, reinterpret_cast<float4*>(s_buf));
 }
 
 template <typename V, int CH, bool HAS_VAL, bool STATS>
 __global__ void __launch_bounds__(SPMM_THREADS, 3) spmm_rows_kernel(const SpmmParams p) {
-  __shared__ float s_mem[2 * SPMM_MAX_SLAB_FLOATS];
-  if ((int)blockIdx.x < p.n_seg) spmm_hub_seg_cta<V, CH, HAS_VAL>(p, (int)blockIdx.x, s_mem);
+  __shared__ __align__(16) float s_mem[2 * SPMM_MAX_SLAB_FLOATS];
+  if ((int)blockIdx.x < p.n_seg) spmm_hub_cta<V, CH, HAS_VAL>(p, (int)blockIdx.x, s_mem);
   else spmm_chunk_cta<V, CH, HAS_VAL, STATS>(p, (int)blockIdx.x - p.n_seg, s_mem);
 }
 
@@ -428,9 +499,9 @@
 
 template <int CH, bool HAS_VAL, bool STATS>
 __global__ void __launch_bounds__(SPMM_THREADS, 3) spmm_rows_pipe_kernel(const SpmmParams p) {
-  __shared__ float s_mem[2 * SPMM_MAX_SLAB_FLOATS];
+  __shared__ __align__(16) float s_mem[2 * SPMM_MAX_SLAB_FLOATS];
   extern __shared__ float4 s_ring[];
-  if ((int)blockIdx.x < p.n_seg) spmm_hub_seg_cta<float4, CH, HAS_VAL>(p, (int)blockIdx.x, s_mem);
+  if ((int)blockIdx.x < p.n_seg) spmm_hub_cta<float4, CH, HAS_VAL>(p, (int)blockIdx.x, s_mem);
   else spmm_chunk_cta_pipe<CH, HAS_VAL, STATS>(p, (int)blockIdx.x - p.n_seg, s_mem, s_ring);
 }
 
@@ -641,12 +712,12 @@
 
 template <int CH, int G, bool HAS_VAL, bool STATS>
 __global__ void __launch_bounds__(SPMM_THREADS, 3) spmm_rows_bulk_kernel(const SpmmParams p) {
-  __shared__ float s_mem[2 * SPMM_MAX_SLAB_FLOATS];
+  __shared__ __align__(16) float s_mem[2 * SPMM_MAX_SLAB_FLOATS];
   extern __shared__ __align__(128) unsigned char s_dyn[];
   const int per_slab = p.main_grid + p.n_seg;
   const int slab = (int)blockIdx.x / per_slab;
   const int b = (int)blockIdx.x - slab * per_slab;
-  if (b < p.n_seg) spmm_hub_seg_cta<float4, CH, HAS_VAL>(p, b, s_mem, slab, slab + 1);
+  if (b < p.n_seg) spmm_hub_cta<float4, CH, HAS_VAL>(p, b, s_mem, p.n_slabs, slab, slab + 1);
   else spmm_chunk_cta_bulk<CH, G, HAS_VAL, STATS>(p, b - p.n_seg, slab, s_mem, reinterpret_cast<float4*>(s_dyn),
                                                   reinterpret_cast<uint64_t*>(s_dyn + SPMM_WARPS * BULK_RING));
 }
@@ -840,11 +911,11 @@
 
 template <int SW, bool HAS_VAL, bool STATS>
 __global__ void __launch_bounds__(SPMM_THREADS, 3) spmm_rows_slab_kernel(const SpmmParams p) {
-  __shared__ float s_mem[2 * SPMM_MAX_SLAB_FLOATS];
+  __shared__ __align__(16) float s_mem[2 * SPMM_MAX_SLAB_FLOATS];
   extern __shared__ __align__(128) unsigned char s_dyn[];
   const int b = (int)blockIdx.x;
   if (b < p.n_seg) {
-    spmm_hub_seg_cta<float4, 1, HAS_VAL>(p, b, s_mem);
+    spmm_hub_cta<float4, 1, HAS_VAL>(p, b, s_mem);
     return;
   }
   const int slab = (b - p.n_seg) / p.main_grid;
@@ -914,57 +985,9 @@
 
 template <bool HAS_VAL, int U>
 __global__ void __launch_bounds__(SPMM_THREADS, 3) spmm_rows_narrow_kernel(const SpmmParams p) {
-  __shared__ float s_mem[SPMM_MAX_SLAB_FLOATS];
-  if ((int)blockIdx.x < p.n_seg) spmm_hub_seg_cta<float4, 1, HAS_VAL>(p, (int)blockIdx.x, s_mem);
+  __shared__ __align__(16) float s_mem[2 * SPMM_MAX_SLAB_FLOATS];
+  if ((int)blockIdx.x < p.n_seg) spmm_hub_cta<float4, 1, HAS_VAL>(p, (int)blockIdx.x, s_mem);
   else spmm_chunk_cta_narrow<HAS_VAL, U>(p, (int)blockIdx.x - p.n_seg);
-}
-
-__global__ void __launch_bounds__(256) spmm_hub_finalize_kernel(const SpmmParams p) {
-  __shared__ float4 sh[256];
-  const int h = blockIdx.x;
-  const int row = __ldg(p.hub_rows + h);
-  const int s0 = __ldg(p.hub_segptr + h), s1 = __ldg(p.hub_segptr + h + 1);
-  const int deg = __ldg(p.rowptr + row + 1) - __ldg(p.rowptr + row);
-  float* stat = p.stat_partial ? p.stat_partial + (size_t)(p.main_grid + h) * 2 * p.K : nullptr;
-  const int nvec = p.K >> 2;
-  const auto al16 = [](const void* q) { return (reinterpret_cast<uintptr_t>(q) & 15) == 0; };
-  if ((p.K & 3) == 0 && nvec <= 256 && (p.ldy & 3) == 0 && al16(p.Y) && al16(p.hub_ws) && (!stat || al16(stat))) {
-    const int G = min(256 / nvec, 16);
-    const int v = threadIdx.x % nvec, g = threadIdx.x / nvec;
-    float4 acc = make_float4(0.f, 0.f, 0.f, 0.f);
-    if (g < G)
-      for (int s = s0 + g; s < s1; s += G) {
-        const float4 x = *reinterpret_cast<const float4*>(p.hub_ws + (size_t)s * p.K + 4 * v);
-        acc.x += x.x; acc.y += x.y; acc.z += x.z; acc.w += x.w;
-      }
-    sh[threadIdx.x] = acc;
-    __syncthreads();
-    if (g != 0) return;
-    for (int j = 1; j < G; ++j) {
-      const float4 x = sh[j * nvec + v];
-      acc.x += x.x; acc.y += x.y; acc.z += x.z; acc.w += x.w;
-    }
-    if (p.mean) { const float d = (float)max(deg, 1); acc.x /= d; acc.y /= d; acc.z /= d; acc.w /= d; }
-    if (p.bias) {
-      acc.x += __ldg(p.bias + 4 * v); acc.y += __ldg(p.bias + 4 * v + 1);
-      acc.z += __ldg(p.bias + 4 * v + 2); acc.w += __ldg(p.bias + 4 * v + 3);
-    }
-    if (p.n_yp) y_row_v4(p, row)[v] = acc; else *reinterpret_cast<float4*>(p.Y + (size_t)row * p.ldy + 4 * v) = acc;
-    if (stat) {
-      *reinterpret_cast<float4*>(stat + 4 * v) = acc;
-      *reinterpret_cast<float4*>(stat + p.K + 4 * v) = make_float4(acc.x * acc.x, acc.y * acc.y, acc.z * acc.z, acc.w * acc.w);
-    }
-    return;
-  }
-  float* yrow = p.n_yp ? reinterpret_cast<float*>(y_row_v4(p, row)) : p.Y + (size_t)row * p.ldy;
-  for (int k = threadIdx.x; k < p.K; k += blockDim.x) {
-    float acc = 0.f;
-    for (int s = s0; s < s1; ++s) acc += p.hub_ws[(size_t)s * p.K + k];
-    if (p.mean) acc /= (float)max(deg, 1);
-    if (p.bias) acc += __ldg(p.bias + k);
-    yrow[k] = acc;
-    if (stat) { stat[k] = acc; stat[p.K + k] = acc * acc; }
-  }
 }
 
 __global__ void __launch_bounds__(256) col_stats_kernel(const float* __restrict__ Y, int64_t ldy, int64_t n_rows,
@@ -996,7 +1019,7 @@
     else spmm_rows_kernel<V, CH, false, false><<<grid, SPMM_THREADS, 0, st>>>(p);
   }
   if ((rc = check_launch())) return rc;
-  if (p.n_hub > 0) {
+  if (p.n_hub > 0 && !p.hub_ticket) {
     spmm_hub_finalize_kernel<<<p.n_hub, 256, 0, st>>>(p);
     if ((rc = check_launch())) return rc;
   }
@@ -1026,7 +1049,7 @@
     else spmm_rows_pipe_kernel<CH, false, false><<<grid, SPMM_THREADS, PIPE_SMEM, st>>>(p);
   }
   if ((rc = check_launch())) return rc;
-  if (p.n_hub > 0) {
+  if (p.n_hub > 0 && !p.hub_ticket) {
     spmm_hub_finalize_kernel<<<p.n_hub, 256, 0, st>>>(p);
     if ((rc = check_launch())) return rc;
   }
@@ -1059,7 +1082,7 @@
     else spmm_rows_bulk_kernel<CH, G, false, false><<<grid, SPMM_THREADS, smem, st>>>(p);
   }
   if ((rc = check_launch())) return rc;
-  if (p.n_hub > 0) {
+  if (p.n_hub > 0 && !p.hub_ticket) {
     spmm_hub_finalize_kernel<<<p.n_hub, 256, 0, st>>>(p);
     if ((rc = check_launch())) return rc;
   }
@@ -1089,7 +1112,7 @@
     else spmm_rows_slab_kernel<SW, false, false><<<grid, SPMM_THREADS, SLAB_SMEM, st>>>(p);
   }
   if ((rc = check_launch())) return rc;
-  if (p.n_hub > 0) {
+  if (p.n_hub > 0 && !p.hub_ticket) {
     spmm_hub_finalize_kernel<<<p.n_hub, 256, 0, st>>>(p);
     if ((rc = check_launch())) return rc;
   }
@@ -1232,12 +1255,11 @@
   return (n_chunks + SPMM_WARPS - 1) / SPMM_WARPS + n_hub;
 }
 
-extern "C" int b200gnn_spmm_csr_f32(const int32_t* rowptr, const int32_t* col, const float* val, const float* X,
-                                    int64_t ldx, float* Y, int64_t ldy, int64_t n_rows, int64_t n_src, int64_t K,
-                                    int reduce, const float* bias, float* stat_partial,
-                                    const int32_t* chunk_rowptr, int64_t n_chunks, int32_t hub_threshold,
-                                    int32_t seg_len, const int32_t* hub_rows, const int32_t* hub_segptr,
-                                    int64_t n_hub, int64_t n_seg, float* hub_workspace, void* stream) {
+static int spmm_csr(const int32_t* rowptr, const int32_t* col, const float* val, const float* X, int64_t ldx, float* Y,
+                    int64_t ldy, int64_t n_rows, int64_t n_src, int64_t K, int reduce, const float* bias, float* stat_partial,
+                    const int32_t* chunk_rowptr, int64_t n_chunks, int32_t hub_threshold, int32_t seg_len,
+                    const int32_t* hub_rows, const int32_t* hub_segptr, int64_t n_hub, int64_t n_seg, float* hub_workspace,
+                    int32_t* hub_tickets, void* stream) {
   if (n_rows < 0 || n_src < 0 || K <= 0 || n_rows >= INT32_MAX || n_src >= INT32_MAX || K > (1 << 20))
     return B200GNN_ERR_BAD_ARG;
   if (reduce != B200GNN_REDUCE_SUM && reduce != B200GNN_REDUCE_MEAN) return B200GNN_ERR_BAD_ARG;
@@ -1254,6 +1276,7 @@
   p.stat_partial = stat_partial;
   p.chunk_rowptr = chunk_rowptr; p.n_chunks = (int32_t)n_chunks;
   p.hub_rows = hub_rows; p.hub_segptr = hub_segptr; p.hub_ws = hub_workspace;
+  p.hub_ticket = n_hub > 0 ? hub_tickets : nullptr;
   p.ldx = ldx; p.ldy = ldy;
   p.n_rows = (int32_t)n_rows; p.K = (int32_t)K;
   p.hub_threshold = hub_threshold; p.seg_len = seg_len; p.n_hub = (int32_t)n_hub;
@@ -1321,7 +1344,7 @@
     if (p.val) { if (deep) spmm_rows_narrow_kernel<true, 8><<<grid, SPMM_THREADS, 0, st>>>(p); else spmm_rows_narrow_kernel<true, 4><<<grid, SPMM_THREADS, 0, st>>>(p); }
     else { if (deep) spmm_rows_narrow_kernel<false, 8><<<grid, SPMM_THREADS, 0, st>>>(p); else spmm_rows_narrow_kernel<false, 4><<<grid, SPMM_THREADS, 0, st>>>(p); }
     if ((rc = check_launch())) return rc;
-    if (p.n_hub > 0) {
+    if (p.n_hub > 0 && !p.hub_ticket) {
       spmm_hub_finalize_kernel<<<p.n_hub, 256, 0, st>>>(p);
       if ((rc = check_launch())) return rc;
     }
@@ -1340,6 +1363,28 @@
     if ((rc = check_launch())) return rc;
   }
   return B200GNN_OK;
+}
+
+extern "C" int b200gnn_spmm_csr_f32(const int32_t* rowptr, const int32_t* col, const float* val, const float* X,
+                                    int64_t ldx, float* Y, int64_t ldy, int64_t n_rows, int64_t n_src, int64_t K,
+                                    int reduce, const float* bias, float* stat_partial,
+                                    const int32_t* chunk_rowptr, int64_t n_chunks, int32_t hub_threshold,
+                                    int32_t seg_len, const int32_t* hub_rows, const int32_t* hub_segptr,
+                                    int64_t n_hub, int64_t n_seg, float* hub_workspace, void* stream) {
+  return spmm_csr(rowptr, col, val, X, ldx, Y, ldy, n_rows, n_src, K, reduce, bias, stat_partial, chunk_rowptr, n_chunks,
+                  hub_threshold, seg_len, hub_rows, hub_segptr, n_hub, n_seg, hub_workspace, nullptr, stream);
+}
+
+extern "C" int b200gnn_spmm_csr_tickets_f32(const int32_t* rowptr, const int32_t* col, const float* val, const float* X,
+                                            int64_t ldx, float* Y, int64_t ldy, int64_t n_rows, int64_t n_src, int64_t K,
+                                            int reduce, const float* bias, float* stat_partial,
+                                            const int32_t* chunk_rowptr, int64_t n_chunks, int32_t hub_threshold,
+                                            int32_t seg_len, const int32_t* hub_rows, const int32_t* hub_segptr,
+                                            int64_t n_hub, int64_t n_seg, float* hub_workspace, int32_t* hub_tickets,
+                                            void* stream) {
+  if (n_hub > 0 && !hub_tickets) return B200GNN_ERR_BAD_ARG;
+  return spmm_csr(rowptr, col, val, X, ldx, Y, ldy, n_rows, n_src, K, reduce, bias, stat_partial, chunk_rowptr, n_chunks,
+                  hub_threshold, seg_len, hub_rows, hub_segptr, n_hub, n_seg, hub_workspace, hub_tickets, stream);
 }
 
 extern "C" int b200gnn_spmm_csr_scatter_f32(const int32_t* rowptr, const int32_t* col, const float* val, const float* X,
diff --git a/efficient-gnns_b200/engine.py b/efficient-gnns_b200/engine.py
--- a/efficient-gnns_b200/engine.py
+++ b/efficient-gnns_b200/engine.py
@@ -83,6 +83,7 @@
                          for l in range(self.L)]
         self.W_split = [(torch.empty(dims[l], dims[l + 1], device=dev), torch.empty(dims[l], dims[l + 1], device=dev))
                         for l in range(self.L)]
+        self._presplit = False
         wg = [ops.wgrad_supported(dims[l], dims[l + 1]) for l in range(self.L)]
         self.wgrad_ws = (torch.empty(max(ops.wgrad_workspace_floats(dims[l], dims[l + 1]) for l in range(self.L) if wg[l]), device=dev)
                          if self.tc_gemm and any(wg) else None)
@@ -183,6 +184,10 @@
     def forward(self, x: torch.Tensor, training: bool = True) -> torch.Tensor:
         fused = training and self.fuse_act
         self._act_stale = False
+        self._presplit = training and self.tc_gemm
+        if self._presplit:
+            ops.split_tf32_batch([(self.W[l], True, *self.Wt_split[l]) for l in range(self.L)] +
+                                 [(self.W[l], False, *self.W_split[l]) for l in range(1, self.L)])
         if fused:
             if self._side is not None:
                 self._ev_fork.record(torch.cuda.current_stream())
@@ -201,7 +206,7 @@
                 if training:
                     gp = self._gemm_part.get(self.dims[1])
                     if gp is not None:
-                        hi, lo = ops.split_tf32(self.W[0], transpose=True, hi=self.Wt_split[0][0], lo=self.Wt_split[0][1])
+                        hi, lo = self._wt_split(0)
                         ops.gemm_tf32x3_stats(self.AX, hi, lo, self.b[0], self.Y[0], gp)
                         part = gp
                     else:
@@ -262,7 +267,7 @@
                 if acc:
                     d_prev = d_out_feat
                 if gp is not None:
-                    hi, lo = ops.split_tf32(self.W[l], transpose=False, hi=self.W_split[l][0], lo=self.W_split[l][1])
+                    hi, lo = self._w_split(l)
                     if act:
                         ops.gemm_tf32x3_bnbwd_bits(self.dH[l], hi, lo, d_prev, act[3], self.Y[l - 1], self.bn[l - 1][0],
                                                    self.bn[l - 1][1], act[1], act[2], self.p, gp, accumulate=acc)
@@ -298,12 +303,22 @@
             self._ev_join.record(self._side)
             torch.cuda.current_stream().wait_event(self._ev_join)
 
+    def _wt_split(self, l: int):
+        if self._presplit:
+            return self.Wt_split[l]
+        return ops.split_tf32(self.W[l], transpose=True, hi=self.Wt_split[l][0], lo=self.Wt_split[l][1])
+
+    def _w_split(self, l: int):
+        if self._presplit:
+            return self.W_split[l]
+        return ops.split_tf32(self.W[l], transpose=False, hi=self.W_split[l][0], lo=self.W_split[l][1])
+
     def _linear(self, l: int, inp: Optional[torch.Tensor], out: torch.Tensor, bias: Optional[torch.Tensor] = None, act=None):
         if act is not None:
-            hi, lo = ops.split_tf32(self.W[l], transpose=True, hi=self.Wt_split[l][0], lo=self.Wt_split[l][1])
+            hi, lo = self._wt_split(l)
             ops.gemm_tf32x3_act(*act, self.p, hi, lo, bias=bias, out=out)
         elif self.tc_gemm:
-            hi, lo = ops.split_tf32(self.W[l], transpose=True, hi=self.Wt_split[l][0], lo=self.Wt_split[l][1])
+            hi, lo = self._wt_split(l)
             ops.gemm_tf32x3(inp, hi, lo, bias=bias, out=out)
         elif bias is not None:
             torch.addmm(bias, inp, self.W[l], out=out)
@@ -312,7 +327,7 @@
 
     def _linear_dgrad(self, l: int, d_out: torch.Tensor, d_inp: torch.Tensor, accumulate: bool = False):
         if self.tc_gemm:
-            hi, lo = ops.split_tf32(self.W[l], transpose=False, hi=self.W_split[l][0], lo=self.W_split[l][1])
+            hi, lo = self._w_split(l)
             ops.gemm_tf32x3(d_out, hi, lo, out=d_inp, accumulate=accumulate)
         elif accumulate:
             d_inp.addmm_(d_out, self.W[l].t())
diff --git a/efficient-gnns_b200/lib.py b/efficient-gnns_b200/lib.py
--- a/efficient-gnns_b200/lib.py
+++ b/efficient-gnns_b200/lib.py
@@ -38,6 +38,9 @@
     "b200gnn_spmm_set_variant": (None, [_int]),
     "b200gnn_spmm_csr_f32": (_int, [_i32p, _i32p, _f32p, _f32p, _i64, _f32p, _i64, _i64, _i64, _i64, _int,
                                     _f32p, _f32p, _i32p, _i64, _i32, _i32, _i32p, _i32p, _i64, _i64, _f32p, _ptr]),
+    "b200gnn_spmm_csr_tickets_f32": (_int, [_i32p, _i32p, _f32p, _f32p, _i64, _f32p, _i64, _i64, _i64, _i64, _int,
+                                            _f32p, _f32p, _i32p, _i64, _i32, _i32, _i32p, _i32p, _i64, _i64, _f32p, _i32p,
+                                            _ptr]),
     "b200gnn_spmm_csr_scatter_f32": (_int, [_i32p, _i32p, _f32p, _f32p, _i64, _ptr, _ptr, _i32, _i64, _i64, _i64, _i64, _i64, _int,
                                             _f32p, _i32p, _i64, _i32, _i32, _i32p, _i32p, _i64, _i64, _f32p, _ptr]),
     "b200gnn_rows_slots": (_i64, [_i64]),
@@ -64,6 +67,7 @@
                                             _f32p, _f32p, _f32p, _f32p, _f32p, _i64, _f32p, _ptr]),
     "b200gnn_partial_reduce_f32": (_int, [_f32p, _i64, _i64, _f32p, _ptr]),
     "b200gnn_adam_step_f32": (_int, [_f32p, _f32p, _f32p, _f32p, _i64, _f32, _f32, _f32, _f32, _i32p, _ptr]),
+    "b200gnn_adam_step_ticket_f32": (_int, [_f32p, _f32p, _f32p, _f32p, _i64, _f32, _f32, _f32, _f32, _i32p, _i32p, _ptr]),
     "b200gnn_rmsprop_step_f32": (_int, [_f32p, _f32p, _f32p, _i64, _f64, _i64, _f64, _f64, _f64, _i32p, _ptr]),
     "b200gnn_teacher_slots": (_i64, [_i64]),
     "b200gnn_label_inputs_f32": (_int, [_f32p, _i64, _i64, _i64, _i64, _i32p, _ptr, _int, _f32, _u64, _u64, _i32p, _u64, _ptr,
@@ -77,6 +81,7 @@
     "b200gnn_kd_loss_fwd_bwd_f32": (_int, [_f32p, _i64, _ptr, _i64, _ptr, _f32p, _i64, _i64, _f32, _f32, _i64, _f32p,
                                            _i64, _f32p, _f32p, _ptr]),
     "b200gnn_split_tf32_f32": (_int, [_f32p, _i64, _i64, _int, _f32p, _f32p, _ptr]),
+    "b200gnn_split_tf32_batch_f32": (_int, [_ptr, _ptr, _ptr, _ptr, _ptr, _ptr, _i32, _ptr]),
     "b200gnn_gemm_tf32x3_f32": (_int, [_f32p, _i64, _f32p, _f32p, _i64, _f32p, _i64, _i64, _i64, _i64, _f32p, _ptr]),
     "b200gnn_random_walk_i64": (_int, [_i32p, _i32p, _i64, _ptr, _i64, _i32, _u64, _u64, _ptr, _ptr]),
     "b200gnn_saint_subgraph_count_i64": (_int, [_i32p, _i32p, _ptr, _i64, _i32p, _ptr, _ptr]),
diff --git a/efficient-gnns_b200/ops.py b/efficient-gnns_b200/ops.py
--- a/efficient-gnns_b200/ops.py
+++ b/efficient-gnns_b200/ops.py
@@ -33,16 +33,17 @@
     if g.n_rows == 0 or K == 0:
         return out
     L = lib.load()
-    ws = g.hub_workspace(K)
-    rc = L.b200gnn_spmm_csr_f32(
+    ws, tickets = g.hub_workspace(K), g.hub_tickets(K)
+    rc = L.b200gnn_spmm_csr_tickets_f32(
         lib.dptr(g.rowptr, torch.int32, "rowptr"), lib.dptr(g.col, torch.int32, "col"),
         lib.dptr(g.val, torch.float32, "val"), lib.dptr(x, torch.float32, "x"), x.stride(0),
         lib.dptr(out, torch.float32, "out"), out.stride(0), g.n_rows, g.n_cols, K, _REDUCE[reduce],
         lib.dptr(bias, torch.float32, "bias"), lib.dptr(stat_partial, torch.float32, "stat_partial"),
         g.chunk_rowptr.data_ptr(), g.n_chunks, g.hub_threshold, g.seg_len,
         g.hub_rows.data_ptr() if g.n_hub else None, g.hub_segptr.data_ptr() if g.n_hub else None,
-        g.n_hub, g.n_seg, None if ws is None else ws.data_ptr(), lib.stream_ptr())
-    lib.check(rc, "spmm_csr_f32")
+        g.n_hub, g.n_seg, None if ws is None else ws.data_ptr(), None if tickets is None else tickets.data_ptr(),
+        lib.stream_ptr())
+    lib.check(rc, "spmm_csr_tickets_f32")
     return out
 
 
@@ -274,7 +275,14 @@
     return d_y, d_gamma, d_beta, d_bias
 
 
-def adam_step(params, grads, exp_avg, exp_avg_sq, step: torch.Tensor, lr: float, betas=(0.9, 0.999), eps: float = 1e-8):
+def adam_step(params, grads, exp_avg, exp_avg_sq, step: torch.Tensor, lr: float, betas=(0.9, 0.999), eps: float = 1e-8,
+              ticket: Optional[torch.Tensor] = None):
+    if ticket is not None:
+        lib.check(lib.load().b200gnn_adam_step_ticket_f32(
+            _f32(params, "params"), _f32(grads, "grads"), _f32(exp_avg, "exp_avg"), _f32(exp_avg_sq, "exp_avg_sq"),
+            params.numel(), lr, betas[0], betas[1], eps, lib.dptr(step, torch.int32, "step"),
+            lib.dptr(ticket, torch.int32, "ticket"), lib.stream_ptr()), "adam_step_ticket_f32")
+        return
     lib.check(lib.load().b200gnn_adam_step_f32(
         _f32(params, "params"), _f32(grads, "grads"), _f32(exp_avg, "exp_avg"), _f32(exp_avg_sq, "exp_avg_sq"),
         params.numel(), lr, betas[0], betas[1], eps, lib.dptr(step, torch.int32, "step"), lib.stream_ptr()),
@@ -309,6 +317,24 @@
     lib.check(lib.load().b200gnn_split_tf32_f32(_f32(w, "w"), rows, cols, int(transpose), _f32(hi, "hi"), _f32(lo, "lo"),
                                                 lib.stream_ptr()), "split_tf32_f32")
     return hi, lo
+
+
+def split_tf32_batch(items) -> None:
+    import ctypes as C
+    if len(items) > 16:
+        split_tf32_batch(items[:16])
+        return split_tf32_batch(items[16:])
+    n = len(items)
+    for w, t, hi, lo in items:
+        rows, cols = w.shape
+        assert hi.shape == lo.shape == ((cols, rows) if t else (rows, cols))
+    rows = (C.c_int64 * n)(*[w.shape[0] for w, _, _, _ in items])
+    cols = (C.c_int64 * n)(*[w.shape[1] for w, _, _, _ in items])
+    trans = _host_i32_array([int(t) for _, t, _, _ in items])
+    lib.check(lib.load().b200gnn_split_tf32_batch_f32(
+        _host_ptr_array([_f32(w, "w") for w, _, _, _ in items]), rows, cols, trans,
+        _host_ptr_array([_f32(hi, "hi") for _, _, hi, _ in items]), _host_ptr_array([_f32(lo, "lo") for _, _, _, lo in items]),
+        n, lib.stream_ptr()), "split_tf32_batch_f32")
 
 
 def gemm_tf32x3(a: torch.Tensor, b_hi: torch.Tensor, b_lo: torch.Tensor, bias: Optional[torch.Tensor] = None,
diff --git a/efficient-gnns_b200/sparse.py b/efficient-gnns_b200/sparse.py
--- a/efficient-gnns_b200/sparse.py
+++ b/efficient-gnns_b200/sparse.py
@@ -82,6 +82,15 @@
             self._ws[K] = ws
         return ws
 
+    def hub_tickets(self, K: int) -> Optional[torch.Tensor]:
+        if self.n_hub == 0:
+            return None
+        t = self._ws.get(("tickets", K))
+        if t is None:
+            t = torch.zeros(self.n_hub, dtype=torch.int32, device=self.device)
+            self._ws[("tickets", K)] = t
+        return t
+
 
 def csr_graph_from(rowptr64: torch.Tensor, col64: torch.Tensor, val: Optional[torch.Tensor],
                    n_rows: int, n_cols: int) -> CsrGraph:
diff --git a/efficient-gnns_b200/trainer.py b/efficient-gnns_b200/trainer.py
--- a/efficient-gnns_b200/trainer.py
+++ b/efficient-gnns_b200/trainer.py
@@ -21,7 +21,9 @@
         self.loss_out = self._grads_buf[self.n_par_pad:self.n_par_pad + 3]
         self.exp_avg = torch.zeros(n, device=device)
         self.exp_avg_sq = torch.zeros(n, device=device)
-        self.step_count = torch.zeros(1, dtype=torch.int32, device=device)
+        counters = torch.zeros(2, dtype=torch.int32, device=device)
+        self.step_count = counters[:1]
+        self._adam_ticket = counters[1:]
         self.views = []
         off = 0
         for k, s in zip(sizes, shapes):
@@ -42,7 +44,7 @@
         return buf[o:o + view.numel()].view(view.shape)
 
     def adam(self, lr: float):
-        ops.adam_step(self.params, self.grads, self.exp_avg, self.exp_avg_sq, self.step_count, lr)
+        ops.adam_step(self.params, self.grads, self.exp_avg, self.exp_avg_sq, self.step_count, lr, ticket=self._adam_ticket)
 
     @contextlib.contextmanager
     def preserved(self):
diff --git a/include/b200gnn.h b/include/b200gnn.h
--- a/include/b200gnn.h
+++ b/include/b200gnn.h
@@ -48,6 +48,16 @@
                          int32_t seg_len, const int32_t* hub_rows,
                          const int32_t* hub_segptr, int64_t n_hub,
                          int64_t n_seg, float* hub_workspace, void* stream);
+int b200gnn_spmm_csr_tickets_f32(const int32_t* rowptr, const int32_t* col,
+                                 const float* val, const float* X, int64_t ldx,
+                                 float* Y, int64_t ldy, int64_t n_rows, int64_t n_src,
+                                 int64_t K, int reduce, const float* bias,
+                                 float* stat_partial, const int32_t* chunk_rowptr,
+                                 int64_t n_chunks, int32_t hub_threshold,
+                                 int32_t seg_len, const int32_t* hub_rows,
+                                 const int32_t* hub_segptr, int64_t n_hub,
+                                 int64_t n_seg, float* hub_workspace,
+                                 int32_t* hub_tickets, void* stream);
 int b200gnn_spmm_csr_scatter_f32(const int32_t* rowptr, const int32_t* col, const float* val, const float* X,
                                  int64_t ldx, float* const* Y_ptrs, const int32_t* row_off, int32_t world,
                                  int64_t ldy_dst, int64_t col_dst, int64_t n_rows, int64_t n_src, int64_t K,
@@ -121,6 +131,10 @@
 int b200gnn_adam_step_f32(float* params, const float* grads, float* exp_avg,
                           float* exp_avg_sq, int64_t n, float lr, float beta1,
                           float beta2, float eps, int32_t* step, void* stream);
+int b200gnn_adam_step_ticket_f32(float* params, const float* grads, float* exp_avg,
+                                 float* exp_avg_sq, int64_t n, float lr, float beta1,
+                                 float beta2, float eps, int32_t* step, int32_t* ticket,
+                                 void* stream);
 int b200gnn_rmsprop_step_f32(float* params, const float* grads, float* square_avg, int64_t n, double lr, int64_t warmup,
                              double alpha, double eps, double weight_decay, int32_t* step, void* stream);
 
@@ -151,6 +165,10 @@
 
 int b200gnn_split_tf32_f32(const float* W, int64_t rows, int64_t cols,
                            int transpose, float* hi, float* lo, void* stream);
+int b200gnn_split_tf32_batch_f32(const float* const* W, const int64_t* rows,
+                                 const int64_t* cols, const int32_t* transpose,
+                                 float* const* hi, float* const* lo, int32_t n,
+                                 void* stream);
 int b200gnn_gemm_tf32x3_f32(const float* A, int64_t lda, const float* B_hi,
                             const float* B_lo, int64_t ldb, float* C,
                             int64_t ldc, int64_t M, int64_t N, int64_t K,
```

Measured after the change: 4.056 billion, median of 6. 1.02x the previous value.
